# ExaScience/elprep

Hardware: AMD Instinct MI355X
Metric: Mreads/s through sort+markdup+BQSR, 150bp PE (higher is better)
Workload: dtype u8/int32/int64 (integer path; float64 finalize on host)

## Files before the change

### elprep_amd/csrc/common.hpp

```cpp
#pragma once

#include <hip/hip_runtime.h>

#include <sched.h>

#include <cstdarg>
#include <cstdint>
#include <cstdio>
#include <cstring>
#include <map>
#include <mutex>
#include <string>
#include <vector>

#include "../../include/elprep_hip.h"
#include "../../include/elprep_hip_debug.h"

namespace elp {

constexpr int WAVE = 64;

enum : uint16_t {
  F_MULTIPLE = 0x1, F_PROPER = 0x2, F_UNMAPPED = 0x4, F_NEXT_UNMAPPED = 0x8, F_REVERSED = 0x10, F_NEXT_REVERSED = 0x20,
  F_FIRST = 0x40, F_LAST = 0x80, F_SECONDARY = 0x100, F_QCFAILED = 0x200, F_DUPLICATE = 0x400, F_SUPPLEMENTARY = 0x800
};

enum : uint32_t { OP_M = 0, OP_I = 1, OP_D = 2, OP_N = 3, OP_S = 4, OP_H = 5, OP_P = 6, OP_EQ = 7, OP_X = 8 };

__host__ __device__ inline bool op_consumes_read(uint32_t op) { return op == OP_M || op == OP_I || op == OP_S || op == OP_EQ || op == OP_X; }
__host__ __device__ inline bool op_consumes_ref(uint32_t op) { return op == OP_M || op == OP_D || op == OP_N || op == OP_EQ || op == OP_X; }

size_t debug_guard_bytes();
void debug_guard_arm(void *p, size_t payload_bytes);
void debug_guard_release(void *p);
int debug_guard_check_all();

template <class T>
struct DVec {
  T *p = nullptr;
  size_t cap = 0;
  DVec() = default;
  DVec(const DVec &) = delete;
  DVec &operator=(const DVec &) = delete;
  ~DVec() { release(); }
  void release() {
    if (p) { debug_guard_release(p); (void)hipFree(p); }
    p = nullptr;
    cap = 0;
  }
  size_t bytes() const { return cap * sizeof(T); }
};

struct ProfPending {
  int name_id;
  hipEvent_t a, b;
};

}

struct elp_ctx {
  int device = 0;
  int n_cu = 256;
  hipStream_t stream = nullptr;
  std::string err;
  std::mutex stage_mu;

  bool have_header = false;
  int32_t n_ref = 0, n_rg = 0, n_lib = 0, n_cov = 0;
  std::vector<int32_t> h_ref_len;
  std::vector<uint16_t> h_rg_lib, h_rg_cov;
  elp::DVec<int32_t> ref_len;
  elp::DVec<uint16_t> rg_lib, rg_cov;

  static constexpr uint64_t SEQ_FRONT = 16;
  uint64_t n = 0, qname_bytes = 0, cigar_ops = 0, seq_bytes = SEQ_FRONT, qual_bytes = 0;
  uint64_t n_sr = 0;
  uint64_t n_filtered = 0;
  elp::DVec<int32_t> refid, pos, next_refid, pnext, tlen;
  elp::DVec<uint16_t> flag, rgid, split;
  elp::DVec<uint8_t> mapq, has_sr;
  elp::DVec<uint32_t> l_seq;
  elp::DVec<uint64_t> qname_off, cigar_off, seq_off, qual_off;
  elp::DVec<uint8_t> qname, seq4, qual;
  elp::DVec<uint32_t> cigar;
  elp::DVec<uint64_t> stage_tmp;
  uint32_t max_qname_len = 0, max_l_seq = 0;
  uint32_t max_split = 0;
  uint32_t max_pos = 0;
  int key_bits = 64;

  bool adapted = false, sorted = false, marked = false;
  bool sorted_qname = false;
  bool radix_check_pending = false;
  bool adapt_bad_qual = false;
  bool adapt_pending = false;
  elp::DVec<uint32_t> adapt_err;
  bool adapt_sampled = false;
  bool adapt_qmask_valid = false;
  unsigned long long adapt_qmask[2] = {0, 0};
  elp::DVec<uint2> apply_recs;
  bool apply_recs_valid = false;
  int apply_recs_lmax = 0;
  bool have_qual_present = false;
  unsigned long long qual_present[2] = {0, 0};
  elp::DVec<int32_t> upos, score;
  elp::DVec<uint64_t> qbounds;
  elp::DVec<uint64_t> key;
  elp::DVec<uint32_t> perm;
  elp::DVec<uint32_t> err_flag;
  elp::DVec<uint32_t> tile_first;
  void *h_pinned = nullptr;
  size_t h_pinned_cap = 0;
  elp::DVec<unsigned long long> radix_state;
  elp::DVec<uint32_t> radix_ticket;
  elp::DVec<unsigned long long> radix_hist;
  elp::DVec<uint32_t> scan_pool;
  elp::DVec<unsigned long long> xchg_hdr;
  elp::DVec<uint32_t> tie_live;
  elp::DVec<uint32_t> md_ctr;
  static constexpr uint32_t MAX_QNAME = 1000;
  static constexpr uint32_t TIE_LIVE_WORDS = 32;
  uint32_t radix_epoch = 0;
  uint64_t flat_index_n = 0, flat_index_bytes = 0;
  uint32_t uniform_len = 0;
  uint64_t uniform_n = ~0ull, uniform_bytes = ~0ull;

  elp::DVec<uint32_t> mate;
  elp::DVec<uint32_t> pair_win;

  std::vector<uint8_t *> h_ref_seq;
  std::vector<int64_t> h_ref_seq_len;
  std::vector<int32_t *> h_sites;
  std::vector<int64_t> h_n_sites;
  std::vector<uint8_t> ref_flags_dirty;
  std::vector<uint32_t *> h_site_idx;
  elp::DVec<uint8_t *> d_ref_seq;
  elp::DVec<int64_t> d_ref_seq_len;
  elp::DVec<int32_t *> d_sites;
  elp::DVec<uint32_t *> d_site_idx;
  elp::DVec<int64_t> d_n_sites;
  bool bqsr_ptrs_dirty = true;

  static constexpr size_t TABLES_TAIL = 4096;
  elp::DVec<unsigned long long> dev_tables;
  size_t tables_n = 0;
  int tables_max_cycle = 0;
  unsigned long long tables_quals[2] = {0, 0};
  elp::DVec<unsigned long long> tables_pack;
  elp::DVec<uint8_t> lut_rows_dev;
  void *comm = nullptr;
  bool comm_borrowed = false;
  int (*xport)(void *, int64_t *, size_t) = nullptr;
  void *xport_user = nullptr;
  int (*p2p)(void *, int, const void *, size_t, int, void *, size_t) = nullptr;
  void *p2p_user = nullptr;
  int group_rank = 0, group_world = 1;
  elp_ctx *group_owner = nullptr;
  std::vector<elp_ctx *> group_borrowers;

  elp::DVec<uint8_t> raw;
  elp::DVec<uint64_t> raw_off;
  uint64_t raw_n = 0, raw_bytes = 0;
  uint64_t max_raw_rec = 0;
  elp::DVec<uint8_t> rg_ids;
  elp::DVec<uint32_t> rg_ids_off;
  bool have_rg_ids = false;
  hipStream_t copy_stream = nullptr;
  elp::DVec<uint8_t> lut_dev;
  void *lut_pinned = nullptr;
  size_t lut_pinned_cap = 0;
  hipEvent_t lut_ev = nullptr;
  hipEvent_t apply_ev = nullptr;
  int lut_uploaded_cycle = 0;
  elp::DVec<uint32_t> lut_wk;
  bool dict_ready = false;
  bool dict_per_cov = false;
  int dict_qlo = 0, dict_nqi = 0, dict_lmax = 0, dict_cycle = 0, dict_ncov = 0;
  hipEvent_t tables_ev = nullptr;
  void *bounce[2] = {nullptr, nullptr};
  hipEvent_t bounce_ev[2] = {nullptr, nullptr};

  uint32_t *mail = nullptr;
  hipEvent_t mail_ev = nullptr;

  elp_ctx *side[2] = {nullptr, nullptr};
  hipEvent_t side_ev[2] = {nullptr, nullptr};
  hipEvent_t side_done[2] = {nullptr, nullptr};
  bool sort_ahead = false;
  uint64_t adapt_epoch = 0;
  uint64_t presort_epoch = ~0ull, presort_n = 0;
  uint64_t *presort_ks = nullptr;
  int presort_idx_bits = 0;

  elp::DVec<uint16_t> snap_flag;
  elp::DVec<uint8_t> snap_qual;
  uint64_t snap_n = 0, snap_qual_bytes = 0;
  bool have_snapshot = false;

  struct Tuning {
    int count_kernel = 0;
    int apply_kernel = 0;
    int count3_rlog = -1;
    int qual_hint = 0;
    int qual_hint_drop = -1;
    int pair_table_slots = 1 << 20;
    long long bgzf_piece = 1ll << 30;
    int bgzf_weak_guess = 0;
    int score_kernel = 0;
    int mate_path = 0;
    int radix_tile = 0;
    int sort_pairs = 0;
    int tie_rounds = 0;
    int exchange_piece = 0;
    int emit_pass = 0;
    long long bgzf_inflate_piece = 2ll << 30;
    int bgzf_copy_chunk = 0;
    int bgzf_tok_lds = 0;
    int bgzf_first_chunk_div = 4;
    int bgzf_fixed = 0;
    int bgzf_tok_fail_above = 0;
    int bgzf_stored = 0;
    int apply_wgs = 0;
    int presort_tile = 0;
    int side_priority = 0;
  } tune;

  elp::DVec<uint8_t> scratch[8];

  bool profiling = false;
  const char *prof_prefix = nullptr;
  std::vector<std::string> prof_names;
  std::map<std::string, int> prof_index;
  std::vector<uint64_t> prof_launches;
  std::vector<double> prof_ms;
  std::vector<elp::ProfPending> prof_pending;
};

namespace elp {

int set_error(elp_ctx *c, int code, const char *fmt, ...);
int prof_begin(elp_ctx *c, const char *name);
void prof_end(elp_ctx *c, int pending);
int prof_flush(elp_ctx *c);
struct ProfScope {
  elp_ctx *c;
  const char *saved;
  ProfScope(elp_ctx *ctx, const char *prefix) : c(ctx), saved(ctx->prof_prefix) { ctx->prof_prefix = prefix; }
  ~ProfScope() { c->prof_prefix = saved; }
};

#define ELP_HIP(ctx, call)                                                                             \
  do {                                                                                                 \
    hipError_t e__ = (call);                                                                           \
    if (e__ != hipSuccess)                                                                             \
      return elp::set_error((ctx), e__ == hipErrorOutOfMemory ? ELP_ERR_NOMEM : ELP_ERR_HIP, "%s failed: %s (%s:%d)", #call, \
                            hipGetErrorString(e__), __FILE__, __LINE__);                               \
  } while (0)

#define ELP_TRY(expr)            \
  do {                           \
    int rc__ = (expr);           \
    if (rc__ != 0) return rc__;  \
  } while (0)

bool sync_spin();
inline void spin_relax(unsigned &spins) {
  if (++spins < 4096u) {
#if defined(__x86_64__) || defined(__i386__)
    __builtin_ia32_pause();
#elif defined(__aarch64__)
    asm volatile("yield");
#endif
  } else {
    sched_yield();
  }
}
inline hipError_t stream_wait(hipStream_t st) {
  if (!sync_spin()) return hipStreamSynchronize(st);
  hipError_t e;
  unsigned spins = 0;
  while ((e = hipStreamQuery(st)) == hipErrorNotReady) spin_relax(spins);
  return e;
}
inline hipError_t event_wait(hipEvent_t ev) {
  if (!sync_spin()) return hipEventSynchronize(ev);
  hipError_t e;
  unsigned spins = 0;
  while ((e = hipEventQuery(ev)) == hipErrorNotReady) spin_relax(spins);
  return e;
}

int debug_poison();
bool debug_trace();

template <class T>
int ensure(elp_ctx *c, DVec<T> &v, size_t n, bool keep = false, size_t keep_elems = 0) {
  if (n <= v.cap) return 0;
  size_t ncap = keep ? (n + n / 2 + 16) : n;
  T *np = nullptr;
  ELP_HIP(c, hipMalloc((void **)&np, ncap * sizeof(T) + debug_guard_bytes()));
  if (debug_guard_bytes()) debug_guard_arm(np, ncap * sizeof(T));
  if (const int pz = debug_poison(); pz >= 0) {
    ELP_HIP(c, hipMemsetAsync(np, pz, ncap * sizeof(T), c->stream));
    ELP_HIP(c, elp::stream_wait(c->stream));
  }
  if (keep && v.p && keep_elems) {
    hipError_t e = hipMemcpyAsync(np, v.p, keep_elems * sizeof(T), hipMemcpyDeviceToDevice, c->stream);
    if (e == hipSuccess) e = elp::stream_wait(c->stream);
    if (e != hipSuccess) {
      (void)hipFree(np);
      return set_error(c, ELP_ERR_HIP, "device copy failed while growing a column: %s", hipGetErrorString(e));
    }
  }
  if (v.p) {
    (void)elp::stream_wait(c->stream);
    debug_guard_release(v.p);
    if (debug_poison() >= 0) { (void)hipMemsetAsync(v.p, 0xDD, v.cap * sizeof(T), c->stream); (void)elp::stream_wait(c->stream); }
    (void)hipFree(v.p);
  }
  v.p = np;
  v.cap = ncap;
  return 0;
}

template <class T>
int scratch(elp_ctx *c, int slot, size_t n, T **out) {
  ELP_TRY(ensure(c, c->scratch[slot], n * sizeof(T) + 256));
  *out = reinterpret_cast<T *>(c->scratch[slot].p);
  return 0;
}

#define ELP_LAUNCH(ctx, name, kernel, grid, block, shmem, ...)                              \
  do {                                                                                      \
    int pp__ = (ctx)->profiling ? elp::prof_begin((ctx), (name)) : -1;                      \
    if (elp::debug_trace()) fprintf(stderr, "[elp] %s\n", (name));                          \
    hipLaunchKernelGGL(kernel, grid, block, shmem, (ctx)->stream, __VA_ARGS__);             \
    if (pp__ >= 0) elp::prof_end((ctx), pp__);                                              \
    ELP_HIP((ctx), hipGetLastError());                                                      \
    if (elp::debug_trace()) ELP_HIP((ctx), elp::stream_wait((ctx)->stream));            \
  } while (0)

inline unsigned blocks_for(uint64_t n, unsigned per_block) { return (unsigned)((n + per_block - 1) / per_block); }

__device__ __forceinline__ uint64_t mix64(uint64_t x) {
  x ^= x >> 30; x *= 0xbf58476d1ce4e5b9ull; x ^= x >> 27; x *= 0x94d049bb133111ebull; x ^= x >> 31;
  return x;
}

__device__ __forceinline__ uint64_t load8(const uint8_t *__restrict__ p) {
  uint64_t w;
  __builtin_memcpy(&w, p, 8);
  return w;
}
__device__ __forceinline__ uint64_t low_bytes(uint64_t w, uint32_t nbytes) {
  return nbytes >= 8 ? w : (w & ((1ull << (8 * nbytes)) - 1ull));
}
__device__ inline int qname_cmp(const uint8_t *__restrict__ q, const uint64_t *__restrict__ off, uint32_t a, uint32_t b) {
  const uint64_t oa = off[a], ob = off[b];
  const uint32_t la = (uint32_t)(off[a + 1] - oa), lb = (uint32_t)(off[b + 1] - ob);
  const uint32_t m = la < lb ? la : lb;
  for (uint32_t i = 0; i < m; i += 8) {
    const uint32_t nb = m - i;
    const uint64_t wa = low_bytes(load8(q + oa + i), nb), wb = low_bytes(load8(q + ob + i), nb);
    if (wa != wb) {
      const uint64_t ba = __builtin_bswap64(wa), bb = __builtin_bswap64(wb);
      return ba < bb ? -1 : 1;
    }
  }
  return la < lb ? -1 : (la > lb ? 1 : 0);
}
__device__ inline bool qname_eq(const uint8_t *__restrict__ q, const uint64_t *__restrict__ off, uint32_t a, uint32_t b) {
  const uint64_t oa = off[a], ob = off[b];
  const uint32_t la = (uint32_t)(off[a + 1] - oa), lb = (uint32_t)(off[b + 1] - ob);
  if (la != lb) return false;
  uint64_t diff = 0;
  for (uint32_t i = 0; i < la && diff == 0; i += 32) {
    const uint64_t a0 = load8(q + oa + i), a1 = load8(q + oa + i + 8), a2 = load8(q + oa + i + 16), a3 = load8(q + oa + i + 24);
    const uint64_t b0 = load8(q + ob + i), b1 = load8(q + ob + i + 8), b2 = load8(q + ob + i + 16), b3 = load8(q + ob + i + 24);
    const uint32_t nb = la - i;
    diff |= low_bytes(a0 ^ b0, nb);
    diff |= nb > 8 ? low_bytes(a1 ^ b1, nb - 8) : 0ull;
    diff |= nb > 16 ? low_bytes(a2 ^ b2, nb - 16) : 0ull;
    diff |= nb > 24 ? low_bytes(a3 ^ b3, nb - 24) : 0ull;
  }
  return diff == 0;
}

__host__ __device__ inline uint16_t mod_flag(uint16_t flag) {
  if ((flag & F_MULTIPLE) == 0) flag &= (uint16_t) ~(F_NEXT_UNMAPPED | F_NEXT_REVERSED);
  if (flag & F_UNMAPPED) flag &= (uint16_t)~F_REVERSED;
  if (flag & F_NEXT_UNMAPPED) flag &= (uint16_t)~F_NEXT_REVERSED;
  return flag;
}

int radix_sort_pairs(elp_ctx *c, uint64_t *keys, uint32_t *vals, uint64_t *keys_tmp, uint32_t *vals_tmp, uint64_t n,
                     uint64_t **keys_out, uint32_t **vals_out);
int radix_sort_fused(elp_ctx *c, const uint64_t *keycol, uint64_t n, int key_bits, int idx_bits, uint64_t *buf0, uint64_t *buf1, uint64_t **out);
struct RadixBounds {
  uint32_t *start = nullptr, *nend = nullptr;
  uint32_t mask = 0;
  int shift = 0;
};
int radix_sort_pairs_low(elp_ctx *c, uint64_t *keys, uint32_t *vals, uint64_t *keys_tmp, uint32_t *vals_tmp, uint64_t n, int ndigits,
                         uint64_t **keys_out, uint32_t **vals_out, const uint64_t *first_src = nullptr, bool identity_vals = false,
                         const uint32_t *n_dev = nullptr , RadixBounds bnd = RadixBounds{});
int exclusive_scan_u32(elp_ctx *c, const uint32_t *in, uint32_t *out, uint64_t n, uint32_t *total_host );
int ensure_adapted(elp_ctx *c, bool check_quals = true);
int adapt_begin(elp_ctx *c, int *pos_bits);
int adapt_scores(elp_ctx *c);
int mailbox(elp_ctx *c);
int side_lane(elp_ctx *c, int lane, elp_ctx **out);
int side_join(elp_ctx *c, int lane);
int sort_presort(elp_ctx *c);
void prof_merge_side(elp_ctx *c);
constexpr int ADAPT_WORDS = 6;
void adapt_note(elp_ctx *c, const uint32_t *words );
int adapt_quality_error(elp_ctx *c);
int ensure_uniform_len(elp_ctx *c);
int ensure_qual_present(elp_ctx *c, bool exact = false);
int fetch_err(elp_ctx *c, uint32_t *words );
int radix_check(elp_ctx *c);
void group_release(elp_ctx *c);
int group_sendrecv(elp_ctx *c, int send_peer, const void *send_dev, size_t send_bytes, int recv_peer, void *recv_dev, size_t recv_bytes);
int tables_written(elp_ctx *c);
int stage_reserve(elp_ctx *c, uint64_t n, uint64_t qb, uint64_t co, uint64_t sb, uint64_t lb);
int merge_refuses_queryname(elp_ctx *groups, const char *who);
int merge_spread_slots(elp_ctx *groups, elp_ctx *spread, uint64_t **slots_out);
int stage_recode_seq(elp_ctx *c, uint64_t from, uint64_t bytes);
int stage_bam_columns(elp_ctx *c, uint32_t n_rec, uint64_t piece_bytes, uint64_t raw_end, uint64_t max_raw_rec, uint16_t split_id);
uint64_t bgzf_framed_size(uint64_t n_bytes);
int bgzf_frame(elp_ctx *c, const uint8_t *raw, uint64_t n_bytes, uint8_t *out);
int bgzf_deflate(elp_ctx *c, const uint8_t *raw, uint64_t n_bytes, uint8_t *out, uint64_t *out_bytes);

}
```

### elprep_amd/csrc/ctx.hip

```cpp
#include "common.hpp"

namespace elp {

namespace {
constexpr size_t GUARD = 4096;
constexpr uint8_t GUARD_BYTE = 0xC3;
std::mutex guard_mu;
std::map<void *, size_t> guard_of;
int guard_check_one(void *p, size_t payload) {
  uint8_t host[GUARD];
  if (hipDeviceSynchronize() != hipSuccess || hipMemcpy(host, static_cast<uint8_t *>(p) + payload, GUARD, hipMemcpyDeviceToHost) != hipSuccess) return 0;
  for (size_t k = 0; k < GUARD; k++)
    if (host[k] != GUARD_BYTE) {
      fprintf(stderr, "[elp] ELP_DEBUG_GUARD: byte %zu behind the end of a %zu-byte device buffer was overwritten (0x%02x)\n", k, payload, host[k]);
      return 1;
    }
  return 0;
}
}
size_t debug_guard_bytes() {
  static const size_t v = [] { const char *e = getenv("ELP_DEBUG_GUARD"); return (e && *e && *e != '0') ? GUARD : (size_t)0; }();
  return v;
}
void debug_guard_arm(void *p, size_t payload) {
// ... 258 lines not shown
    if (c->bounce[k]) (void)hipHostFree(c->bounce[k]);
    if (c->bounce_ev[k]) (void)hipEventDestroy(c->bounce_ev[k]);
  }
  if (c->copy_stream) (void)hipStreamDestroy(c->copy_stream);
  if (c->tables_ev) (void)hipEventDestroy(c->tables_ev);
  group_release(c);
  (void)hipStreamDestroy(c->stream);
  delete c;
}

const char *elp_last_error(const elp_ctx *c) { return c ? c->err.c_str() : "null context"; }

int elp_sync(elp_ctx *c) {
  if (!c) return ELP_ERR_ARG;
  if (c->radix_check_pending) return radix_check(c);
  ELP_HIP(c, elp::stream_wait(c->stream));
  return 0;
}

void *elp_stream(elp_ctx *c) { return c ? (void *)c->stream : nullptr; }

int elp_set_header(elp_ctx *c, const elp_header *h) {
  if (!c || !h || h->n_ref < 0 || h->n_rg < 0 || (h->n_ref && !h->ref_len) || (h->n_rg && (!h->rg_lib || !h->rg_cov)))
    return set_error(c, ELP_ERR_ARG, "elp_set_header: bad arguments");
  ELP_HIP(c, hipSetDevice(c->device));
  c->n_ref = h->n_ref; c->n_rg = h->n_rg; c->n_lib = h->n_lib; c->n_cov = h->n_cov;
  c->apply_recs_valid = false;
  c->h_ref_len.assign(h->ref_len, h->ref_len + h->n_ref);
  c->h_rg_lib.assign(h->rg_lib, h->rg_lib + h->n_rg);
  c->h_rg_cov.assign(h->rg_cov, h->rg_cov + h->n_rg);
  for (int i = 0; i < h->n_rg; i++) {
    if (c->h_rg_lib[i] != ELP_NIL16 && c->h_rg_lib[i] >= h->n_lib) return set_error(c, ELP_ERR_ARG, "rg_lib[%d] out of range", i);
    if (c->h_rg_cov[i] >= h->n_cov) return set_error(c, ELP_ERR_ARG, "rg_cov[%d] out of range", i);
  }
  ELP_TRY(ensure(c, c->ref_len, (size_t)h->n_ref + 1));
  ELP_TRY(ensure(c, c->rg_lib, (size_t)h->n_rg + 1));
  ELP_TRY(ensure(c, c->rg_cov, (size_t)h->n_rg + 1));
  if (h->n_ref) ELP_HIP(c, hipMemcpyAsync(c->ref_len.p, h->ref_len, h->n_ref * sizeof(int32_t), hipMemcpyHostToDevice, c->stream));
  if (h->n_rg) {
    ELP_HIP(c, hipMemcpyAsync(c->rg_lib.p, h->rg_lib, h->n_rg * sizeof(uint16_t), hipMemcpyHostToDevice, c->stream));
    ELP_HIP(c, hipMemcpyAsync(c->rg_cov.p, h->rg_cov, h->n_rg * sizeof(uint16_t), hipMemcpyHostToDevice, c->stream));
  }
  ELP_HIP(c, elp::stream_wait(c->stream));
  c->h_ref_seq.resize(h->n_ref, nullptr);
  c->h_ref_seq_len.resize(h->n_ref, 0);
  c->h_sites.resize(h->n_ref, nullptr);
  c->h_site_idx.resize(h->n_ref, nullptr);
  c->h_n_sites.resize(h->n_ref, 0);
  c->ref_flags_dirty.assign(h->n_ref, 0);
  c->bqsr_ptrs_dirty = true;
  c->have_header = true;
  return 0;
}

}
namespace elp {
int stage_reserve(elp_ctx *c, uint64_t n, uint64_t qb, uint64_t co, uint64_t sb, uint64_t lb) {
  bool keep = c->n > 0;
  ELP_TRY(ensure(c, c->refid, n, keep, c->n));
  ELP_TRY(ensure(c, c->pos, n, keep, c->n));
  ELP_TRY(ensure(c, c->next_refid, n, keep, c->n));
  ELP_TRY(ensure(c, c->pnext, n, keep, c->n));
  ELP_TRY(ensure(c, c->tlen, n, keep, c->n));
  ELP_TRY(ensure(c, c->flag, n, keep, c->n));
  ELP_TRY(ensure(c, c->rgid, n, keep, c->n));
  ELP_TRY(ensure(c, c->split, n, keep, c->n));
  ELP_TRY(ensure(c, c->mapq, n, keep, c->n));
  ELP_TRY(ensure(c, c->has_sr, n, keep, c->n));
  ELP_TRY(ensure(c, c->l_seq, n, keep, c->n));
  ELP_TRY(ensure(c, c->qname_off, n + 1, keep, c->n + 1));
  ELP_TRY(ensure(c, c->cigar_off, n + 1, keep, c->n + 1));
  ELP_TRY(ensure(c, c->seq_off, n + 1, keep, c->n + 1));
  ELP_TRY(ensure(c, c->qual_off, n + 1, keep, c->n + 1));
  ELP_TRY(ensure(c, c->qname, qb + 64, keep, c->qname_bytes));
  ELP_TRY(ensure(c, c->cigar, co + 4, keep, c->cigar_ops));
  ELP_TRY(ensure(c, c->seq4, sb + 32, keep, c->seq_bytes));
  ELP_TRY(ensure(c, c->qual, lb + 32, keep, c->qual_bytes));
  return 0;
}
}
extern "C" {

int elp_reserve(elp_ctx *c, uint64_t n, uint64_t qb, uint64_t co, uint64_t sb, uint64_t lb) {
  if (!c) return ELP_ERR_ARG;
  std::lock_guard<std::mutex> g(c->stage_mu);
  ELP_HIP(c, hipSetDevice(c->device));
  return stage_reserve(c, n, qb, co, sb + elp_ctx::SEQ_FRONT, lb);
}

int elp_reset(elp_ctx *c) {
  if (!c) return ELP_ERR_ARG;
  std::lock_guard<std::mutex> g(c->stage_mu);
  c->n = c->qname_bytes = c->cigar_ops = c->qual_bytes = 0;
  c->seq_bytes = elp_ctx::SEQ_FRONT;
  c->n_sr = 0;
  c->n_filtered = 0;
  c->raw_n = c->raw_bytes = 0;
  c->max_raw_rec = 0;
  c->max_split = 0;
  c->max_qname_len = c->max_l_seq = 0;
  c->max_pos = 0;
  c->adapted = c->sorted = c->sorted_qname = c->marked = false;
  c->have_qual_present = false;
  c->have_snapshot = false;
  c->flat_index_n = 0;
  c->uniform_n = ~0ull;
  return 0;
}

uint64_t elp_num_records(const elp_ctx *c) { return c ? c->n : 0; }
uint64_t elp_num_sorted(const elp_ctx *c) { return c ? c->n - c->n_sr : 0; }
uint64_t elp_num_qual_bytes(const elp_ctx *c) { return c ? c->qual_bytes : 0; }

int elp_stage(elp_ctx *c, const elp_batch *b) {
  if (!c || !b) return ELP_ERR_ARG;
  std::lock_guard<std::mutex> g(c->stage_mu);
  ELP_HIP(c, hipSetDevice(c->device));
  if (!c->have_header) return set_error(c, ELP_ERR_ARG, "elp_stage: call elp_set_header first");
  uint64_t n = b->n;
  if (n == 0) return 0;
  if (c->n + n > 0xFFFFFFF0ull) return set_error(c, ELP_ERR_UNSUPPORTED, "more than 2^32-16 records per context");
  uint64_t q0 = b->qname_off[0], c0 = b->cigar_off[0], s0 = b->seq_off[0], l0 = b->qual_off[0];
  uint64_t qb = b->qname_off[n] - q0, co = b->cigar_off[n] - c0, sb = b->seq_off[n] - s0, lb = b->qual_off[n] - l0;
  ELP_TRY(stage_reserve(c, c->n + n, c->qname_bytes + qb, c->cigar_ops + co, c->seq_bytes + sb, c->qual_bytes + lb));
  hipStream_t st = c->stream;
  uint64_t at = c->n;
#define H2D(dst, src, cnt, T) ELP_HIP(c, hipMemcpyAsync((dst), (src), (cnt) * sizeof(T), hipMemcpyHostToDevice, st))
  if (lb) H2D(c->qual.p + c->qual_bytes, b->qual + l0, lb, uint8_t);
  if (sb) {
    H2D(c->seq4.p + c->seq_bytes, b->seq4 + s0, sb, uint8_t);
    hipLaunchKernelGGL(k_recode_seq, dim3(blocks_for((sb + 15) / 16, 256)), dim3(256), 0, st, c->seq4.p + c->seq_bytes, sb);
    ELP_HIP(c, hipGetLastError());
  }
  if (qb) H2D(c->qname.p + c->qname_bytes, b->qname + q0, qb, uint8_t);
  if (co) H2D(c->cigar.p + c->cigar_ops, b->cigar + c0, co, uint32_t);
  H2D(c->refid.p + at, b->refid, n, int32_t);
  H2D(c->pos.p + at, b->pos, n, int32_t);
  H2D(c->next_refid.p + at, b->next_refid, n, int32_t);
  H2D(c->pnext.p + at, b->pnext, n, int32_t);
  H2D(c->tlen.p + at, b->tlen, n, int32_t);
  H2D(c->flag.p + at, b->flag, n, uint16_t);
  H2D(c->rgid.p + at, b->rgid, n, uint16_t);
  if (b->split) H2D(c->split.p + at, b->split, n, uint16_t);
  else ELP_HIP(c, hipMemsetAsync(c->split.p + at, 0, n * sizeof(uint16_t), st));
  H2D(c->mapq.p + at, b->mapq, n, uint8_t);
  H2D(c->l_seq.p + at, b->l_seq, n, uint32_t);
  if (b->has_sr) H2D(c->has_sr.p + at, b->has_sr, n, uint8_t);
  else ELP_HIP(c, hipMemsetAsync(c->has_sr.p + at, 0, n, st));
  ELP_TRY(ensure(c, c->stage_tmp, 4 * (n + 1)));
  unsigned blk = 256, grd = blocks_for(n + 1, blk);
  struct { const uint64_t *src; uint64_t *dst; uint64_t base; } offs[4] = {
      {b->qname_off, c->qname_off.p + at, c->qname_bytes}, {b->cigar_off, c->cigar_off.p + at, c->cigar_ops},
      {b->seq_off, c->seq_off.p + at, c->seq_bytes}, {b->qual_off, c->qual_off.p + at, c->qual_bytes}};
  for (int k = 0; k < 4; k++) H2D(c->stage_tmp.p + (size_t)k * (n + 1), offs[k].src, n + 1, uint64_t);
  for (int k = 0; k < 4; k++) {
    hipLaunchKernelGGL(k_rebase_offsets, dim3(grd), dim3(blk), 0, st, (const uint64_t *)(c->stage_tmp.p + (size_t)k * (n + 1)), offs[k].dst, n + 1, offs[k].base,
                       offs[k].src[0]);
    ELP_HIP(c, hipGetLastError());
  }
#undef H2D
  uint64_t n_sr = 0;
  uint32_t max_split = c->max_split;
  uint32_t max_qname_len = c->max_qname_len, max_l_seq = c->max_l_seq, max_pos = c->max_pos;
  int scan_rc = 0;
  for (uint64_t i = 0; i < n && !scan_rc; i++) {
    uint64_t ql = b->qname_off[i + 1] - b->qname_off[i];
    if (ql > elp_ctx::MAX_QNAME) scan_rc = set_error(c, ELP_ERR_UNSUPPORTED, "record %llu: QNAME of %llu bytes (limit %u)", (unsigned long long)i, (unsigned long long)ql, elp_ctx::MAX_QNAME);
    if (b->has_sr && b->has_sr[i]) n_sr++;
    if (b->split && b->split[i] > max_split) max_split = b->split[i];
    if (ql > max_qname_len) max_qname_len = (uint32_t)ql;
    if (b->l_seq[i] > max_l_seq) max_l_seq = b->l_seq[i];
    if ((uint32_t)b->pos[i] > max_pos) max_pos = (uint32_t)b->pos[i];
    if (b->qual_off[i + 1] - b->qual_off[i] > 0x3FFFFFull || b->l_seq[i] > 0x3FFFFFu)
      scan_rc = set_error(c, ELP_ERR_UNSUPPORTED, "record %llu: more than 4194303 bases", (unsigned long long)i);
    if (b->rgid[i] != ELP_NIL16 && b->rgid[i] >= c->n_rg) scan_rc = set_error(c, ELP_ERR_ARG, "record %llu: rgid %u not in header", (unsigned long long)i, b->rgid[i]);
    if (b->refid[i] >= c->n_ref) scan_rc = set_error(c, ELP_ERR_ARG, "record %llu: refid %d not in header", (unsigned long long)i, b->refid[i]);
  }
  if (scan_rc) { (void)elp::stream_wait(st); return scan_rc; }
  ELP_HIP(c, elp::stream_wait(st));
  c->n += n; c->qname_bytes += qb; c->cigar_ops += co; c->seq_bytes += sb; c->qual_bytes += lb;
  c->n_sr += n_sr;
  c->max_split = max_split;
  c->max_qname_len = max_qname_len; c->max_l_seq = max_l_seq; c->max_pos = max_pos;
  c->adapted = c->sorted = c->sorted_qname = c->marked = false;
  c->have_qual_present = false;
  c->have_snapshot = false;
  c->flat_index_n = 0;
  c->uniform_n = ~0ull;
  return 0;
}

int elp_stage_columns(elp_ctx *c, uint64_t n, const int32_t *refid, const int32_t *pos, const int32_t *next_refid, const int32_t *pnext, const int32_t *tlen,
                      const uint16_t *flag, const uint8_t *mapq, const uint16_t *rgid, const uint8_t *has_sr, const uint32_t *l_seq,
                      const uint64_t *qname_off, const uint8_t *qname, const uint64_t *cigar_off, const uint32_t *cigar, const uint64_t *seq_off,
                      const uint8_t *seq4, const uint64_t *qual_off, const uint8_t *qual, const uint16_t *split) {
  if (!c) return ELP_ERR_ARG;
  if (n && (!refid || !pos || !next_refid || !pnext || !tlen || !flag || !mapq || !rgid || !l_seq || !qname_off || !cigar_off || !seq_off || !qual_off))
    return set_error(c, ELP_ERR_ARG, "elp_stage_columns: a required column is NULL");
  elp_batch b;
  b.n = n; b.refid = refid; b.pos = pos; b.next_refid = next_refid; b.pnext = pnext; b.tlen = tlen; b.flag = flag; b.mapq = mapq; b.rgid = rgid;
  b.has_sr = has_sr; b.l_seq = l_seq; b.qname_off = qname_off; b.qname = qname; b.cigar_off = cigar_off; b.cigar = cigar; b.seq_off = seq_off;
  b.seq4 = seq4; b.qual_off = qual_off; b.qual = qual; b.split = split;
  return elp_stage(c, &b);
}

int elp_set_header_columns(elp_ctx *c, int32_t n_ref, const int32_t *ref_len, int32_t n_rg, const uint16_t *rg_lib, const uint16_t *rg_cov, int32_t n_lib,
                           int32_t n_cov) {
  elp_header h;
  h.n_ref = n_ref; h.ref_len = ref_len; h.n_rg = n_rg; h.rg_lib = rg_lib; h.rg_cov = rg_cov; h.n_lib = n_lib; h.n_cov = n_cov;
  return elp_set_header(c, &h);
}

static int d2h(elp_ctx *c, void *dst, const void *src, size_t bytes) {
  if (!bytes) return 0;
  ELP_HIP(c, hipSetDevice(c->device));
  ELP_HIP(c, hipMemcpyAsync(dst, src, bytes, hipMemcpyDeviceToHost, c->stream));
  ELP_HIP(c, elp::stream_wait(c->stream));
  return 0;
}

int elp_get_permutation(elp_ctx *c, uint32_t *out) {
  if (!c || (!out && c->n)) return ELP_ERR_ARG;
  if (!c->sorted) return set_error(c, ELP_ERR_ARG, "elp_get_permutation: call elp_sort_coordinate or elp_sort_queryname first");
  ELP_TRY(radix_check(c));
  return d2h(c, out, c->perm.p, c->n * sizeof(uint32_t));
}
int elp_get_flags(elp_ctx *c, uint16_t *out) {
  if (!c || (!out && c->n)) return ELP_ERR_ARG;
  ELP_TRY(radix_check(c));
  return d2h(c, out, c->flag.p, c->n * sizeof(uint16_t));
}
int elp_get_adapted(elp_ctx *c, int32_t *upos, int32_t *score) {
  if (!c) return ELP_ERR_ARG;
  ELP_TRY(ensure_adapted(c));
  if (upos) ELP_TRY(d2h(c, upos, c->upos.p, c->n * sizeof(int32_t)));
  if (score) ELP_TRY(d2h(c, score, c->score.p, c->n * sizeof(int32_t)));
  return 0;
}
int elp_get_qual(elp_ctx *c, uint8_t *out) {
  if (!c || (!out && c->qual_bytes)) return ELP_ERR_ARG;
  return d2h(c, out, c->qual.p, c->qual_bytes);
}

int elp_snapshot(elp_ctx *c) {
  if (!c) return ELP_ERR_ARG;
  ELP_HIP(c, hipSetDevice(c->device));
  ELP_TRY(ensure(c, c->snap_flag, c->n + 1));
  ELP_TRY(ensure(c, c->snap_qual, c->qual_bytes + 16));
  if (c->n) ELP_HIP(c, hipMemcpyAsync(c->snap_flag.p, c->flag.p, c->n * sizeof(uint16_t), hipMemcpyDeviceToDevice, c->stream));
  if (c->qual_bytes) ELP_HIP(c, hipMemcpyAsync(c->snap_qual.p, c->qual.p, c->qual_bytes, hipMemcpyDeviceToDevice, c->stream));
  c->snap_n = c->n;
  c->snap_qual_bytes = c->qual_bytes;
  c->have_snapshot = true;
  return 0;
}
int elp_rollback(elp_ctx *c) {
  if (!c) return ELP_ERR_ARG;
  if (!c->have_snapshot || c->snap_n != c->n || c->snap_qual_bytes != c->qual_bytes)
    return set_error(c, ELP_ERR_ARG, "elp_rollback: no snapshot of the current record set");
  ELP_HIP(c, hipSetDevice(c->device));
  if (c->n) ELP_HIP(c, hipMemcpyAsync(c->flag.p, c->snap_flag.p, c->n * sizeof(uint16_t), hipMemcpyDeviceToDevice, c->stream));
  if (c->qual_bytes) ELP_HIP(c, hipMemcpyAsync(c->qual.p, c->snap_qual.p, c->qual_bytes, hipMemcpyDeviceToDevice, c->stream));
  c->adapted = c->sorted = c->sorted_qname = c->marked = false;
  c->have_qual_present = false;
  return 0;
}

int elp_set_tuning(elp_ctx *c, const char *key, int64_t value) {
  if (!c || !key) return ELP_ERR_ARG;
  const std::string k(key);
  const int v = (int)value;
  if (k == "count_kernel") c->tune.count_kernel = v;
  else if (k == "apply_kernel") c->tune.apply_kernel = v;
  else if (k == "bgzf_piece") { if (value < 1) return set_error(c, ELP_ERR_ARG, "elp_set_tuning: bgzf_piece must be positive"); c->tune.bgzf_piece = value; }
  else if (k == "bgzf_weak_guess") c->tune.bgzf_weak_guess = v;
  else if (k == "score_kernel") { c->tune.score_kernel = v; c->adapted = false; }
  else if (k == "count3_rlog") c->tune.count3_rlog = v;
  else if (k == "qual_hint") { c->tune.qual_hint = v; c->have_qual_present = false; }
  else if (k == "qual_hint_drop") { c->tune.qual_hint_drop = v; c->have_qual_present = false; }
  else if (k == "pair_table_slots") {
    if (v == 0) { c->tune.pair_table_slots = 1 << 20; return 0; }
    if (v < 2 || v > (1 << 20) || (v & (v - 1))) return set_error(c, ELP_ERR_ARG, "elp_set_tuning: pair_table_slots must be a power of two >= 2");
    c->tune.pair_table_slots = v;
  } else if (k == "mate_path") {
    if (value != 0 && value != 2) return set_error(c, ELP_ERR_ARG, "elp_set_tuning: mate_path is 0 (the library decides) or 2 (every candidate through the table)");
    c->tune.mate_path = v;
  } else if (k == "tie_rounds") c->tune.tie_rounds = v;
  else if (k == "radix_tile") c->tune.radix_tile = v;
  else if (k == "sort_pairs") c->tune.sort_pairs = v;
  else if (k == "exchange_piece") c->tune.exchange_piece = v;
  else if (k == "emit_pass") c->tune.emit_pass = v;
  else if (k == "bgzf_stored") c->tune.bgzf_stored = v;
  else if (k == "bgzf_tok_fail_above") c->tune.bgzf_tok_fail_above = v;
  else if (k == "bgzf_fixed") c->tune.bgzf_fixed = v;
  else if (k == "bgzf_first_chunk_div") c->tune.bgzf_first_chunk_div = v;
  else if (k == "bgzf_tok_lds") c->tune.bgzf_tok_lds = v;
  else if (k == "bgzf_copy_chunk") c->tune.bgzf_copy_chunk = v;
  else if (k == "bgzf_inflate_piece") { if (value < 1) return set_error(c, ELP_ERR_ARG, "elp_set_tuning: bgzf_inflate_piece must be positive"); c->tune.bgzf_inflate_piece = value; }
  else if (k == "md_fused" || k == "bgzf_inflate") {
    if (value != 0) return set_error(c, ELP_ERR_ARG, "elp_set_tuning: key '%s' is retired (only 0 is accepted)", key);
  } else if (k == "apply_wgs") c->tune.apply_wgs = v;
  else if (k == "presort_tile") c->tune.presort_tile = v;
  else if (k == "side_priority") c->tune.side_priority = v;
  else return set_error(c, ELP_ERR_ARG, "elp_set_tuning: unknown key '%s'", key);
  return 0;
}

int elp_profile_enable(elp_ctx *c, int on) {
  if (!c) return ELP_ERR_ARG;
  if (!on) { ELP_TRY(prof_flush(c)); prof_merge_side(c); }
  c->profiling = on != 0;
  for (int lane = 0; lane < 2; lane++)
    if (c->side[lane]) c->side[lane]->profiling = c->profiling;
  return 0;
}
int elp_profile_reset(elp_ctx *c) {
  if (!c) return ELP_ERR_ARG;
  ELP_TRY(prof_flush(c));
  prof_merge_side(c);
  for (auto &v : c->prof_launches) v = 0;
  for (auto &v : c->prof_ms) v = 0.0;
  return 0;
}
int elp_profile_count(elp_ctx *c) {
  if (!c) return ELP_ERR_ARG;
  if (prof_flush(c) != 0) return ELP_ERR_HIP;
  prof_merge_side(c);
  return (int)c->prof_names.size();
}
int elp_profile_get(elp_ctx *c, int index, const char **name, uint64_t *launches, double *total_ms) {
  if (!c || index < 0 || index >= (int)c->prof_names.size()) return ELP_ERR_ARG;
  if (name) *name = c->prof_names[index].c_str();
  if (launches) *launches = c->prof_launches[index];
  if (total_ms) *total_ms = c->prof_ms[index];
  return 0;
}

}
```

### elprep_amd/csrc/metrics.hip

```cpp
#include "common.hpp"

namespace elp {

constexpr uint32_t EMPTY = 0xFFFFFFFFu;

struct MxCols {
  uint64_t n;
  const int32_t *refid;
  const uint16_t *flag;
  const uint16_t *rgid;
  const uint16_t *rg_lib;
  const int32_t *upos;
  const uint64_t *qname_off;
  const uint8_t *qname;
  const uint32_t *mate, *pair_win;
  int32_t n_lib;
  const uint8_t *has_sr;
  const uint16_t *split;
  int32_t n_split;
};
constexpr uint32_t OPT_SMALL = 32;
constexpr uint32_t OPT_LIST_CAP = 300000;

__device__ __forceinline__ uint32_t lib_row(const MxCols &m, uint32_t i) {
  const uint16_t rg = m.rgid[i];
  const uint16_t lb = rg == ELP_NIL16 ? (uint16_t)ELP_NIL16 : m.rg_lib[rg];
  return lb == ELP_NIL16 ? (uint32_t)m.n_lib : (uint32_t)lb;
}
__device__ __forceinline__ bool true_pair(uint16_t f) { return (f & (F_MULTIPLE | F_NEXT_UNMAPPED)) == F_MULTIPLE; }

__device__ __forceinline__ void order_ends(const MxCols &m, uint32_t second, uint32_t first, uint32_t &a1, uint32_t &a2) {
  a1 = second; a2 = first;
  const int32_t r1 = m.refid[a1], r2 = m.refid[a2];
  const int32_t p1 = m.upos[a1], p2 = m.upos[a2];
  const bool v1 = m.flag[a1] & F_REVERSED, v2 = m.flag[a2] & F_REVERSED;
  if (r1 > r2 || (r1 == r2 && (p1 > p2 || (p1 == p2 && v1 && !v2)))) { uint32_t t = a1; a1 = a2; a2 = t; }
}
__device__ __forceinline__ uint32_t listed_read(const MxCols &m, uint32_t owner) {
  uint32_t a1, a2;
  order_ends(m, owner, m.mate[owner], a1, a2);
  return (m.flag[a1] & F_FIRST) ? a1 : a2;
}

constexpr int DC_CAP = 2048, DC_STEP = 1024;
__device__ __forceinline__ void wave_count(unsigned int *lds, int cell) {
  unsigned long long todo = __ballot(cell >= 0);
  while (todo) {
    const int leader = __ffsll((long long)todo) - 1;
    const int c0 = __builtin_amdgcn_readlane(cell, leader);
    const unsigned long long peers = __ballot(cell == c0);
    if ((int)(threadIdx.x & 63) == leader) atomicAdd(&lds[c0], (unsigned int)__popcll(peers));
    todo &= ~peers;
  }
}
__global__ __launch_bounds__(256) void k_dup_counters(MxCols m, unsigned long long *__restrict__ ctr, unsigned long long *__restrict__ pair_reads,
                                                      uint64_t chunk, uint64_t *__restrict__ lkeys, uint32_t *__restrict__ lvals, uint32_t *list_n) {
  extern __shared__ unsigned int lds_ctr[];
  __shared__ uint2 lq[DC_CAP];
  __shared__ uint32_t lcount, gbase;
  const int nrow = (m.n_lib + 1) * ELP_NCTR, ncell = nrow + m.n_split * (m.n_lib + 1);
  for (int k = threadIdx.x; k < ncell; k += blockDim.x) lds_ctr[k] = 0;
  if (threadIdx.x == 0) lcount = 0;
  __syncthreads();
  const uint64_t lo = (uint64_t)blockIdx.x * chunk, hi = lo + chunk < m.n ? lo + chunk : m.n;
  for (uint64_t base = lo; base < hi; base += DC_STEP) {
    constexpr int R = DC_STEP / 256;
    uint8_t sr[R];
    uint16_t fl[R], rg[R], sp[R];
    uint32_t pw[R], mt[R];
#pragma unroll
    for (int t = 0; t < R; t++) {
      const uint64_t i = base + (uint64_t)t * 256 + threadIdx.x;
      const bool in = i < hi;
      sr[t] = in ? m.has_sr[i] : (uint8_t)1;
      fl[t] = in ? m.flag[i] : (uint16_t)0;
      rg[t] = in ? m.rgid[i] : (uint16_t)ELP_NIL16;
      sp[t] = in ? m.split[i] : (uint16_t)0;
      pw[t] = in ? m.pair_win[i] : EMPTY;
      mt[t] = in ? m.mate[i] : EMPTY;
    }
    uint16_t lb[R], fm[R];
    uint8_t srm[R];
#pragma unroll
    for (int t = 0; t < R; t++) {
      lb[t] = rg[t] == ELP_NIL16 ? (uint16_t)ELP_NIL16 : m.rg_lib[rg[t]];
      const bool need = mt[t] != EMPTY && ((fl[t] & F_DUPLICATE) || pw[t] != EMPTY);
      srm[t] = need ? m.has_sr[mt[t]] : (uint8_t)0;
      fm[t] = need ? m.flag[mt[t]] : (uint16_t)0;
    }
#pragma unroll
    for (int t = 0; t < R; t++) {
      const uint32_t i = (uint32_t)(base + (uint64_t)t * 256 + threadIdx.x);
      bool loser = false;
      int cell1 = -1, cell2 = -1;
      if (!sr[t]) {
        const uint16_t f = fl[t];
        const int lib = lb[t] == ELP_NIL16 ? m.n_lib : (int)lb[t], row = lib * ELP_NCTR;
        if (f & F_UNMAPPED) cell1 = row + 3;
        else if (f & (F_SECONDARY | F_SUPPLEMENTARY)) cell1 = row + 2;
        else {
          const bool tp = true_pair(f);
          cell1 = tp ? nrow + (int)sp[t] * (m.n_lib + 1) + lib : row;
          if (f & F_DUPLICATE) {
            if (!tp) cell2 = row + 4;
            else if (mt[t] != EMPTY && mt[t] < i && (fm[t] & F_DUPLICATE) && !srm[t]) cell2 = row + 5;
          }
        }
        loser = pw[t] != EMPTY && !srm[t];
      }
      wave_count(lds_ctr, cell1);
      wave_count(lds_ctr, cell2);
      const unsigned long long mask = __ballot(loser);
      if (mask) {
        const int lane = threadIdx.x & 63, leader = __ffsll((long long)mask) - 1;
        uint32_t at = 0;
        if (lane == leader) at = atomicAdd(&lcount, (uint32_t)__popcll(mask));
        at = __shfl(at, leader, 64);
        if (loser) lq[at + (uint32_t)__popcll(mask & ((1ull << lane) - 1ull))] = make_uint2(i, pw[t]);
      }
    }
    __syncthreads();
    const uint32_t have = lcount;
    if (have > DC_CAP - DC_STEP || base + DC_STEP >= hi) {
      if (threadIdx.x == 0) gbase = have ? atomicAdd(list_n, have) : 0u;
      __syncthreads();
      for (uint32_t k = threadIdx.x; k < have; k += 256) {
        const uint2 e = lq[k];
        lkeys[gbase + k] = (uint64_t)e.y;
        lvals[gbase + k] = e.x;
      }
      __syncthreads();
      if (threadIdx.x == 0) lcount = 0;
      __syncthreads();
    }
  }
  for (int k = threadIdx.x; k < nrow; k += blockDim.x)
    if (lds_ctr[k]) atomicAdd(&ctr[k], (unsigned long long)lds_ctr[k]);
  for (int k = threadIdx.x + nrow; k < ncell; k += blockDim.x)
    if (lds_ctr[k]) atomicAdd(&pair_reads[k - nrow], (unsigned long long)lds_ctr[k]);
}

__global__ __launch_bounds__(256) void k_opt_heads(uint32_t L, const uint64_t *__restrict__ ks, uint32_t *__restrict__ head) {
  const uint32_t j = blockIdx.x * blockDim.x + threadIdx.x;
  if (j < L) head[j] = (j == 0 || ks[j] != ks[j - 1]) ? 1u : 0u;
}
__global__ __launch_bounds__(256) void k_opt_starts(uint32_t L, const uint32_t *__restrict__ head, const uint32_t *__restrict__ gidx,
                                                    uint32_t *__restrict__ gstart, uint32_t G) {
  const uint32_t j = blockIdx.x * blockDim.x + threadIdx.x;
  if (j >= L) return;
  if (head[j]) gstart[gidx[j]] = j;
  if (j == L - 1) gstart[G] = L;
}

struct Tile { long long t, x, y; };

template <class W>
__device__ __forceinline__ Tile tile_parse(uint32_t len, bool *bad, W word) {
  long long v2 = 0, v3 = 0, v4 = 0, v5 = 0, v6 = 0;
  uint32_t badmask = 0;
  int col = 0;
  unsigned long long x = 0;
  uint32_t ndig = 0;
  bool neg = false, fbad = false, first = true;
  uint64_t w = 0;
  for (uint32_t i = 0;; i++) {
    const bool end = i == len;
    if (!end && (i & 7u) == 0) w = word(i >> 3);
    const uint32_t ch = end ? (uint32_t)':' : (uint32_t)(w >> (8 * (i & 7u))) & 0xFFu;
    if (ch == ':') {
      const bool fb = fbad || ndig == 0 || x > (neg ? 0x8000000000000000ull : 0x7FFFFFFFFFFFFFFFull);
      const long long val = (long long)(neg ? 0ull - x : x);
      if (col == 2) v2 = val; else if (col == 3) v3 = val; else if (col == 4) v4 = val; else if (col == 5) v5 = val; else if (col == 6) v6 = val;
      if (col >= 2 && col <= 6 && fb) badmask |= 1u << col;
      col++;
      x = 0; ndig = 0; neg = false; fbad = false; first = true;
    } else {
      if (first && (ch == '+' || ch == '-')) {
        neg = ch == '-';
      } else {
        const uint32_t d = ch - (uint32_t)'0';
        if (d > 9) fbad = true;
        else if (x > 922337203685477580ull) fbad = true;
        else x = x * 10 + d;
        ndig++;
      }
      first = false;
    }
    if (end) break;
  }
  int a;
  if (col == 7) a = 4;
  else if (col == 5) a = 2;
  else return Tile{-1, -1, -1};
  if (badmask & (7u << a)) { *bad = true; return Tile{-1, -1, -1}; }
  return a == 4 ? Tile{v4, v5, v6} : Tile{v2, v3, v4};
}
__device__ inline Tile tile_info(const uint8_t *__restrict__ q, uint32_t len, bool *bad) {
  if (len <= 48) {
    const uint64_t w0 = len > 0 ? load8(q) : 0ull, w1 = len > 8 ? load8(q + 8) : 0ull, w2 = len > 16 ? load8(q + 16) : 0ull,
                   w3 = len > 24 ? load8(q + 24) : 0ull, w4 = len > 32 ? load8(q + 32) : 0ull, w5 = len > 40 ? load8(q + 40) : 0ull;
    return tile_parse(len, bad, [&](uint32_t k) { return k == 0 ? w0 : k == 1 ? w1 : k == 2 ? w2 : k == 3 ? w3 : k == 4 ? w4 : w5; });
  }
  return tile_parse(len, bad, [&](uint32_t k) { return load8(q + 8 * k); });
}

struct Member { long long t, x, y; uint32_t rg_rev, bad; };

__device__ inline Member make_member(const MxCols &m, uint32_t read) {
  bool bad = false;
  const uint64_t o = m.qname_off[read];
  Tile tl = tile_info(m.qname + o, (uint32_t)(m.qname_off[read + 1] - o), &bad);
  return Member{tl.t, tl.x, tl.y, ((uint32_t)m.rgid[read] << 1) | ((m.flag[read] & F_REVERSED) ? 1u : 0u), bad ? 1u : 0u};
}

__global__ __launch_bounds__(256) void k_opt_slots(MxCols m, uint32_t L, const uint64_t *__restrict__ ks, const uint32_t *__restrict__ vs,
                                                   const uint32_t *__restrict__ head, const uint32_t *__restrict__ gidx,
                                                   const uint32_t *__restrict__ gstart, uint32_t *__restrict__ mread, uint2 *__restrict__ ginfo,
                                                   uint32_t *__restrict__ mset) {
  const uint32_t j = blockIdx.x * blockDim.x + threadIdx.x;
  if (j >= L) return;
  const bool is_head = head[j] != 0;
  const uint32_t g = gidx[j] - (is_head ? 0u : 1u);
  const uint32_t j0 = gstart[g], oslot = j0 + g;
  const uint32_t slot = j + g + 1;
  mread[slot] = listed_read(m, vs[j]);
  mset[slot] = oslot;
  if (is_head) {
    const uint32_t origin = (uint32_t)ks[j];
    mread[oslot] = listed_read(m, origin);
    mset[oslot] = oslot;
    ginfo[oslot] = make_uint2(gstart[g + 1] - j0 + 1, origin);
  }
}
__global__ __launch_bounds__(256) void k_opt_fill(MxCols m, uint32_t total, const uint32_t *__restrict__ mread, Member *__restrict__ members) {
  const uint32_t s = blockIdx.x * blockDim.x + threadIdx.x;
  if (s >= total) return;
  members[s] = make_member(m, mread[s]);
}

__device__ inline uint32_t uf_find(uint32_t *p, uint32_t x) {
  uint32_t r = x;
  while (p[r] != r) r = p[r];
  while (p[x] != r) { uint32_t nx = p[x]; p[x] = r; x = nx; }
  return r;
}
__device__ __forceinline__ long long go_abs_diff(long long a, long long b) {
  const unsigned long long d = (unsigned long long)a - (unsigned long long)b;
  return (long long)((long long)d < 0 ? 0ull - d : d);
}
__device__ __forceinline__ bool optical_close(const Member &a, const Member &b, long long dist) {
  if (a.t == -1 || b.rg_rev != a.rg_rev || b.t != a.t) return false;
  return go_abs_diff(a.x, b.x) <= dist && go_abs_diff(a.y, b.y) <= dist;
}

__global__ __launch_bounds__(128) void k_opt_eval(MxCols m, uint32_t total, const uint2 *__restrict__ ginfo, const Member *__restrict__ members,
                                                  uint32_t *__restrict__ parent, long long dist, unsigned long long *__restrict__ ctr,
                                                  uint32_t *err, unsigned long long *__restrict__ hist, int hist_len, int lds_bins,
                                                  uint32_t *__restrict__ linfo, uint32_t *__restrict__ lcount, uint32_t *n_large) {
  extern __shared__ unsigned int lds_opt[];
  unsigned int *lds_h = lds_opt + (m.n_lib + 1);
  const int n_h = hist ? (m.n_lib + 1) * 3 * lds_bins : 0;
  for (int k = threadIdx.x; k <= m.n_lib + n_h; k += blockDim.x) lds_opt[k] = 0;
  __syncthreads();
  for (uint32_t b = blockIdx.x * blockDim.x + threadIdx.x; b < total; b += gridDim.x * blockDim.x) {
  const uint2 gi = ginfo[b];
  const uint32_t cnt = gi.x;
  uint32_t optical = 0;
  bool large = false;
  if (cnt > OPT_SMALL) {
    const Member *g = members + b;
    uint32_t nr = 0, bad_f = 0, bad_r = 0;
    for (uint32_t k = 0; k < cnt; k++) {
      const uint32_t rev = g[k].rg_rev & 1u;
      nr += rev;
      bad_r |= g[k].bad & rev;
      bad_f |= g[k].bad & (rev ^ 1u);
    }
    const uint32_t nf = cnt - nr;
    if ((bad_f && nf >= 2 && nf <= OPT_LIST_CAP) || (bad_r && nr >= 2 && nr <= OPT_LIST_CAP)) atomicOr(&err[2], 1u);
    linfo[b] = 1u | (nf > OPT_LIST_CAP ? 2u : 0u) | (nr > OPT_LIST_CAP ? 4u : 0u);
    lcount[b] = (nf > OPT_LIST_CAP ? OPT_LIST_CAP + 1 : nf) + (nr > OPT_LIST_CAP ? OPT_LIST_CAP + 1 : nr);
    atomicAdd(n_large, cnt);
    large = true;
  } else if (cnt >= 2) {
  const Member *g = members + b;
  {
    uint32_t nr = 0, bad_f = 0, bad_r = 0;
    for (uint32_t k = 0; k < cnt; k++) {
      const uint32_t rev = g[k].rg_rev & 1u, bad = g[k].bad;
      nr += rev;
      bad_r |= bad & rev;
      bad_f |= bad & (rev ^ 1u);
    }
    if ((bad_f && cnt - nr >= 2) || (bad_r && nr >= 2)) atomicOr(&err[2], 1u);
  }
  if (cnt == 2) {
    optical = optical_close(g[0], g[1], dist) ? 1u : 0u;
  } else if (cnt == 3) {
    const Member m0 = g[0], m1 = g[1], m2 = g[2];
    const uint32_t e01 = optical_close(m0, m1, dist), e02 = optical_close(m0, m2, dist), e12 = optical_close(m1, m2, dist);
    const uint32_t edges = e01 + e02 + e12;
    optical = edges >= 2 ? 2u : edges;
  } else {
    uint32_t *p = parent + b;
    for (uint32_t k = 0; k < cnt; k++) p[k] = k;
    uint32_t comps = cnt;
    for (uint32_t a = 0; a < cnt; a++) {
      const Member ma = g[a];
      if (ma.t == -1) continue;
      for (uint32_t c2 = a + 1; c2 < cnt; c2++) {
        if (optical_close(ma, g[c2], dist)) {
          const uint32_t ra = uf_find(p, a), rb = uf_find(p, c2);
          if (ra != rb) { p[rb] = ra; comps--; }
        }
      }
    }
    optical = cnt - comps;
  }
  }
  if (!large && (optical || (hist && cnt >= 2))) {
    const uint32_t owner = gi.y;
    uint32_t a1, a2;
    order_ends(m, owner, m.mate[owner], a1, a2);
    const uint32_t lib = lib_row(m, a1);
    if (optical) atomicAdd(&lds_opt[lib], optical);
    if (hist && cnt >= 2) {
      const int idx[3] = {(int)cnt, (int)(cnt - optical), optical ? (int)optical + 1 : 0};
#pragma unroll
      for (int k = 0; k < 3; k++) {
        if (idx[k] <= 0) continue;
        const int bin = idx[k] < hist_len ? idx[k] : hist_len - 1;
        if (bin < lds_bins) atomicAdd(&lds_h[((int)lib * 3 + k) * lds_bins + bin], 1u);
        else atomicAdd(&hist[((size_t)lib * 3 + k) * hist_len + bin], 1ull);
      }
    }
  }
  }
  __syncthreads();
  for (int k = threadIdx.x; k <= m.n_lib; k += blockDim.x)
    if (lds_opt[k]) atomicAdd(&ctr[k * ELP_NCTR + 6], (unsigned long long)lds_opt[k]);
  for (int k = threadIdx.x; k < n_h; k += blockDim.x)
    if (lds_h[k]) atomicAdd(&hist[(size_t)(k / lds_bins) * hist_len + (k % lds_bins)], (unsigned long long)lds_h[k]);
}

__global__ __launch_bounds__(256) void k_large_list(uint32_t total, const uint32_t *__restrict__ mset, const uint32_t *__restrict__ linfo,
                                                    const Member *__restrict__ members, uint64_t *__restrict__ keys, uint32_t *__restrict__ vals,
                                                    uint32_t *count) {
  const uint32_t s = blockIdx.x * blockDim.x + threadIdx.x;
  if (s >= total) return;
  const uint32_t b = mset[s], li = linfo[b];
  if (!(li & 1u)) return;
  const Member mem = members[s];
  if (mem.t == -1 || (li & ((mem.rg_rev & 1u) ? 4u : 2u))) return;
  const uint32_t at = atomicAdd(count, 1u);
  keys[at] = mix64(mix64(((uint64_t)b << 32) | mem.rg_rev) ^ (uint64_t)mem.t);
  vals[at] = s;
}
__device__ __forceinline__ uint32_t puf_find(uint32_t *parent, uint32_t x) {
  for (;;) {
    const uint32_t p = __hip_atomic_load(&parent[x], __ATOMIC_RELAXED, __HIP_MEMORY_SCOPE_AGENT);
    if (p == x) return x;
    x = p;
  }
}
__device__ inline void puf_union(uint32_t *parent, uint32_t a, uint32_t b) {
  for (;;) {
    a = puf_find(parent, a);
    b = puf_find(parent, b);
    if (a == b) return;
    const uint32_t hi = a > b ? a : b, lo = a > b ? b : a;
    if (atomicCAS(&parent[hi], hi, lo) == hi) return;
  }
}
__global__ __launch_bounds__(256) void k_large_union(uint32_t cnt, const uint64_t *__restrict__ keys, const uint32_t *__restrict__ vals,
                                                     const uint32_t *__restrict__ mset, const Member *__restrict__ members, long long dist,
                                                     uint32_t *parent) {
  const uint32_t j = blockIdx.x * blockDim.x + threadIdx.x;
  if (j >= cnt) return;
  const uint64_t kj = keys[j];
  const uint32_t sj = vals[j], bj = mset[sj];
  const Member mj = members[sj];
  for (uint32_t k = j + 1; k < cnt && keys[k] == kj; k++) {
    const uint32_t sk = vals[k];
    if (mset[sk] == bj && optical_close(mj, members[sk], dist)) puf_union(parent, j, k);
  }
}
__global__ __launch_bounds__(256) void k_large_roots(uint32_t cnt, const uint32_t *__restrict__ vals, const uint32_t *__restrict__ mset,
                                                     const uint32_t *__restrict__ parent, unsigned long long *setcnt) {
  const uint32_t j = blockIdx.x * blockDim.x + threadIdx.x;
  if (j >= cnt) return;
  atomicAdd(&setcnt[mset[vals[j]]], 1ull | (parent[j] == j ? (1ull << 32) : 0ull));
}
__global__ __launch_bounds__(256) void k_large_final(MxCols m, uint32_t total, const uint2 *__restrict__ ginfo, const uint32_t *__restrict__ linfo,
                                                     const uint32_t *__restrict__ lcount, const unsigned long long *__restrict__ setcnt,
                                                     unsigned long long *__restrict__ ctr, unsigned long long *__restrict__ hist, int hist_len) {
  const uint32_t b = blockIdx.x * blockDim.x + threadIdx.x;
  if (b >= total || !(linfo[b] & 1u) || ginfo[b].x == 0) return;
  const unsigned long long sc = setcnt[b];
  const uint32_t optical = (uint32_t)sc - (uint32_t)(sc >> 32);
  const uint32_t owner = ginfo[b].y;
  uint32_t a1, a2;
  order_ends(m, owner, m.mate[owner], a1, a2);
  const uint32_t lib = lib_row(m, a1);
  if (optical) atomicAdd(&ctr[lib * ELP_NCTR + 6], (unsigned long long)optical);
  if (hist) {
    const uint32_t cnt = lcount[b];
    const int idx[3] = {(int)cnt, (int)(cnt - optical), optical ? (int)optical + 1 : 0};
    for (int k = 0; k < 3; k++) {
      if (idx[k] <= 0) continue;
      const int bin = idx[k] < hist_len ? idx[k] : hist_len - 1;
      atomicAdd(&hist[((size_t)lib * 3 + k) * hist_len + bin], 1ull);
    }
  }
}
__global__ __launch_bounds__(256) void k_iota32(uint32_t *v, uint32_t n) {
  const uint32_t i = blockIdx.x * blockDim.x + threadIdx.x;
  if (i < n) v[i] = i;
}

__global__ __launch_bounds__(256) void k_origin_count(MxCols m, unsigned long long *__restrict__ origins) {
  extern __shared__ unsigned int lds_org[];
  for (int k = threadIdx.x; k <= m.n_lib; k += blockDim.x) lds_org[k] = 0;
  __syncthreads();
  for (uint64_t i = (uint64_t)blockIdx.x * blockDim.x + threadIdx.x; i < m.n; i += (uint64_t)gridDim.x * blockDim.x) {
    const uint32_t mt = m.mate[i];
    if (mt == EMPTY || mt > (uint32_t)i || m.pair_win[i] != EMPTY) continue;
    uint32_t a1, a2;
    order_ends(m, (uint32_t)i, mt, a1, a2);
    atomicAdd(&lds_org[lib_row(m, a1)], 1u);
  }
  __syncthreads();
  for (int k = threadIdx.x; k <= m.n_lib; k += blockDim.x)
    if (lds_org[k]) atomicAdd(&origins[k], (unsigned long long)lds_org[k]);
}

static int metrics_impl(elp_ctx *c, int dist, int64_t *counters_host, int64_t *hist_host, int hist_len) {
  const uint64_t n = c->n;
  const int ncell = (c->n_lib + 1) * ELP_NCTR;
  if (!c->marked) return set_error(c, ELP_ERR_ARG, "elp_dup_metrics: call elp_mark_duplicates first");
  const size_t nhist = hist_host ? (size_t)(c->n_lib + 1) * 3 * (size_t)hist_len : 0, norg = hist_host ? (size_t)(c->n_lib + 1) : 0;
  const int n_split = (int)c->max_split + 1;
  const size_t npr = (size_t)n_split * (size_t)(c->n_lib + 1);
  if (((size_t)ncell + npr) * sizeof(unsigned int) > 46000)
    return set_error(c, ELP_ERR_UNSUPPORTED, "elp_dup_metrics: %d split ids x %d libraries in one context", n_split, c->n_lib + 1);
  unsigned long long *ctr;
  ELP_TRY(scratch(c, 0, (size_t)ncell + norg + nhist + npr + 8, &ctr));
  unsigned long long *origins = ctr + ncell, *hist = hist_host ? origins + norg : nullptr, *pair_reads = ctr + ncell + norg + nhist;
  hipStream_t st = c->stream;
  ELP_HIP(c, hipMemsetAsync(ctr, 0, ((size_t)ncell + norg + nhist + npr) * sizeof(unsigned long long), st));
  int lds_bins = hist_host ? std::min(hist_len, 32) : 0;
  if ((size_t)(c->n_lib + 1) * (1 + 3 * (size_t)lds_bins) * sizeof(unsigned int) > 32768) lds_bins = 0;
  if (n) {
    MxCols m{n, c->refid.p, c->flag.p, c->rgid.p, c->rg_lib.p, c->upos.p, c->qname_off.p, c->qname.p, c->mate.p, c->pair_win.p, c->n_lib,
             c->has_sr.p, c->split.p, n_split};
    const unsigned grid = blocks_for(n, 256);
    const size_t lcap = n / 2 + 8;
    uint32_t *gs;
    ELP_TRY(scratch(c, 1, 6 * lcap + 16, &gs));
    uint64_t *pk = reinterpret_cast<uint64_t *>(gs);
    uint32_t *pv = gs + 4 * lcap;
    uint32_t *mailbox = c->err_flag.p + 3;
    ELP_HIP(c, hipMemsetAsync(mailbox, 0, 4, st));
    const unsigned cgrid = (unsigned)std::min<uint64_t>(2048, (n + DC_STEP - 1) / DC_STEP);
    const uint64_t chunk = (((n + cgrid - 1) / cgrid) + DC_STEP - 1) / DC_STEP * DC_STEP;
    ELP_LAUNCH(c, "mx_counters", k_dup_counters, dim3(cgrid), dim3(256), ((size_t)ncell + npr) * sizeof(unsigned int), m, ctr, pair_reads, chunk, pk, pv,
               mailbox);
    uint32_t L = 0;
    ELP_HIP(c, hipMemcpyAsync(&L, mailbox, 4, hipMemcpyDeviceToHost, st));
    ELP_HIP(c, elp::stream_wait(st));
    ELP_HIP(c, hipMemsetAsync(mailbox, 0, 4, st));
    if ((size_t)L > lcap) return set_error(c, ELP_ERR_HIP, "elp_dup_metrics: more losing pairs than pairs");
    uint32_t total = 0, G = 0;
    uint64_t *ks = pk;
    uint32_t *vs = pv, *head = nullptr, *gidx = nullptr, *gstart = nullptr;
    if (L) {
      int ndig = 1;
      while (ndig < 4 && (n >> (8 * ndig)) != 0) ndig++;
      {
        ProfScope ps(c, "mx_");
        ELP_TRY(radix_sort_pairs_low(c, pk, pv, pk + lcap, pv + lcap, L, ndig, &ks, &vs));
      }
      head = reinterpret_cast<uint32_t *>(ks == pk ? pk + lcap : pk);
      gidx = head + lcap;
      gstart = vs == pv ? pv + lcap : pv;
      ELP_LAUNCH(c, "mx_opt_heads", k_opt_heads, dim3(blocks_for(L, 256)), dim3(256), 0, L, (const uint64_t *)ks, head);
      {
        ProfScope ps(c, "mx_");
        ELP_TRY(exclusive_scan_u32(c, head, gidx, L, &G));
      }
      ELP_LAUNCH(c, "mx_opt_starts", k_opt_starts, dim3(blocks_for(L, 256)), dim3(256), 0, L, (const uint32_t *)head, (const uint32_t *)gidx, gstart, G);
      total = L + G;
    }
    if (total) {
      Member *members;
      uint32_t *wk, *mread;
      uint2 *ginfo;
      const size_t tp = ((size_t)total + 7) & ~(size_t)7;
      ELP_TRY(scratch(c, 2, (size_t)total + 4, &members));
      ELP_TRY(scratch(c, 3, 12 * tp + 16, &wk));
      ELP_TRY(scratch(c, 4, (size_t)total + 4, &mread));
      ELP_TRY(scratch(c, 5, (size_t)total + 4, &ginfo));
      uint32_t *parent = wk, *mset = wk + tp, *linfo = wk + 2 * tp, *lcount = wk + 3 * tp, *lvals = wk + 6 * tp;
      unsigned long long *setcnt = reinterpret_cast<unsigned long long *>(wk + 4 * tp);
      uint64_t *lkeys = reinterpret_cast<uint64_t *>(wk + 8 * tp);
      ELP_HIP(c, hipMemsetAsync(ginfo, 0, (size_t)total * sizeof(uint2), st));
      ELP_HIP(c, hipMemsetAsync(linfo, 0, 4 * tp * sizeof(uint32_t), st));
      ELP_LAUNCH(c, "mx_opt_slots", k_opt_slots, dim3(blocks_for(L, 256)), dim3(256), 0, m, L, (const uint64_t *)ks, (const uint32_t *)vs,
                 (const uint32_t *)head, (const uint32_t *)gidx, (const uint32_t *)gstart, mread, ginfo, mset);
      ELP_LAUNCH(c, "mx_opt_fill", k_opt_fill, dim3(blocks_for(total, 256)), dim3(256), 0, m, total, (const uint32_t *)mread, members);
      ELP_LAUNCH(c, "mx_opt_eval", k_opt_eval, dim3(std::min(blocks_for(total, 128), 2048u)), dim3(128),
                 (size_t)(c->n_lib + 1) * (1 + (hist ? 3 * (size_t)lds_bins : 0)) * sizeof(unsigned int), m, total, (const uint2 *)ginfo,
                 (const Member *)members, parent, (long long)dist, ctr, c->err_flag.p, hist, hist_len, lds_bins, linfo, lcount, mailbox);
      uint32_t n_large = 0;
      ELP_HIP(c, hipMemcpyAsync(&n_large, mailbox, 4, hipMemcpyDeviceToHost, st));
      ELP_HIP(c, elp::stream_wait(st));
      ELP_HIP(c, hipMemsetAsync(mailbox, 0, 4, st));
      if (n_large) {
        ELP_LAUNCH(c, "mx_large_list", k_large_list, dim3(blocks_for(total, 256)), dim3(256), 0, total, (const uint32_t *)mset, (const uint32_t *)linfo,
                   (const Member *)members, lkeys, lvals, mailbox);
        uint32_t cl = 0;
        ELP_HIP(c, hipMemcpyAsync(&cl, mailbox, 4, hipMemcpyDeviceToHost, st));
        ELP_HIP(c, elp::stream_wait(st));
        ELP_HIP(c, hipMemsetAsync(mailbox, 0, 4, st));
        if (cl) {
          uint64_t *ks;
          uint32_t *vs;
          ProfScope ps(c, "mx_large_");
          ELP_TRY(radix_sort_pairs(c, lkeys, lvals, lkeys + tp, lvals + tp, cl, &ks, &vs));
          ELP_LAUNCH(c, "mx_large_iota", k_iota32, dim3(blocks_for(cl, 256)), dim3(256), 0, parent, cl);
          ELP_LAUNCH(c, "mx_large_union", k_large_union, dim3(blocks_for(cl, 256)), dim3(256), 0, cl, (const uint64_t *)ks, (const uint32_t *)vs,
                     (const uint32_t *)mset, (const Member *)members, (long long)dist, parent);
          ELP_LAUNCH(c, "mx_large_roots", k_large_roots, dim3(blocks_for(cl, 256)), dim3(256), 0, cl, (const uint32_t *)vs, (const uint32_t *)mset,
                     (const uint32_t *)parent, setcnt);
        }
        ELP_LAUNCH(c, "mx_large_final", k_large_final, dim3(blocks_for(total, 256)), dim3(256), 0, m, total, (const uint2 *)ginfo, (const uint32_t *)linfo,
                   (const uint32_t *)lcount, (const unsigned long long *)setcnt, ctr, hist, hist_len);
      }
    }
    if (hist)
      ELP_LAUNCH(c, "mx_origin_count", k_origin_count, dim3(std::min(grid, 2048u)), dim3(256), (c->n_lib + 1) * sizeof(unsigned int), m, origins);
  }
  std::vector<unsigned long long> h((size_t)ncell + norg + nhist + npr);
  ELP_HIP(c, hipMemcpyAsync(h.data(), ctr, h.size() * sizeof(unsigned long long), hipMemcpyDeviceToHost, st));
  uint32_t e[4];
  ELP_TRY(fetch_err(c, e));
  if (e[2]) {
    ELP_HIP(c, hipMemsetAsync(c->err_flag.p + 2, 0, 4, st));
    return set_error(c, ELP_ERR_DATA, "QNAME tile/x/y field is not an integer (reference: internal.ParseInt panics, filters/mark-optical-duplicates.go:55-61)");
  }
  for (int l = 0; l <= c->n_lib; l++)
    for (int k = 0; k < ELP_NCTR; k++) counters_host[l * ELP_NCTR + k] = (int64_t)h[l * ELP_NCTR + k];
  for (int l = 0; l <= c->n_lib; l++) {
    int64_t pairs = 0;
    for (int sp = 0; sp < n_split; sp++) pairs += (int64_t)(h[(size_t)ncell + norg + nhist + (size_t)sp * (c->n_lib + 1) + l] / 2);
    counters_host[l * ELP_NCTR + 1] = pairs;
  }
  if (hist_host) {
    const unsigned long long *ho = h.data() + ncell, *hh = ho + norg;
    for (int l = 0; l <= c->n_lib; l++) {
      int64_t *out = hist_host + (size_t)l * 3 * hist_len;
      unsigned long long with_dups = 0;
      for (size_t k = 0; k < (size_t)3 * hist_len; k++) out[k] = (int64_t)hh[(size_t)l * 3 * hist_len + k];
      for (int b = 0; b < hist_len; b++) with_dups += hh[(size_t)l * 3 * hist_len + b];
      const int64_t alone = (int64_t)(ho[l] - with_dups);
      const int one = 1 < hist_len ? 1 : hist_len - 1;
      out[one] += alone;
      out[hist_len + one] += alone;
    }
  }
  return 0;
}

}

namespace elp {
static int metrics_on_side(elp_ctx *c, int dist, int64_t *counters_host, int64_t *hist_host, int hist_len) {
  if (!c->marked) return set_error(c, ELP_ERR_ARG, "elp_dup_metrics: call elp_mark_duplicates first");
  elp_ctx *s = nullptr;
  ELP_TRY(side_lane(c, 0, &s));
  s->n = c->n; s->n_lib = c->n_lib; s->n_rg = c->n_rg; s->n_ref = c->n_ref; s->max_split = c->max_split; s->marked = c->marked;
  s->n_sr = c->n_sr; s->n_filtered = c->n_filtered;
  s->flag.p = c->flag.p; s->rgid.p = c->rgid.p; s->rg_lib.p = c->rg_lib.p; s->refid.p = c->refid.p; s->qname_off.p = c->qname_off.p; s->qname.p = c->qname.p;
  s->pair_win.p = c->pair_win.p; s->mate.p = c->mate.p; s->has_sr.p = c->has_sr.p; s->upos.p = c->upos.p; s->split.p = c->split.p;
  const int rc = metrics_impl(s, dist, counters_host, hist_host, hist_len);
  s->flag.p = nullptr; s->rgid.p = nullptr; s->rg_lib.p = nullptr; s->refid.p = nullptr; s->qname_off.p = nullptr; s->qname.p = nullptr;
  s->pair_win.p = nullptr; s->mate.p = nullptr; s->has_sr.p = nullptr; s->upos.p = nullptr; s->split.p = nullptr;
  if (rc != 0) {
    (void)elp::stream_wait(s->stream);
    c->err = s->err;
  }
  return rc;
}
}

extern "C" int elp_dup_metrics(elp_ctx *c, int optical_pixel_distance, int64_t *counters) {
  if (!c || !counters) return ELP_ERR_ARG;
  ELP_HIP(c, hipSetDevice(c->device));
  return elp::metrics_on_side(c, optical_pixel_distance, counters, nullptr, 0);
}

extern "C" int elp_dup_metrics_hist(elp_ctx *c, int optical_pixel_distance, int64_t *counters, int64_t *hist, int hist_len) {
  if (!c || !counters || !hist || hist_len < 2) return elp::set_error(c, ELP_ERR_ARG, "elp_dup_metrics_hist: bad arguments (hist_len >= 2)");
  ELP_HIP(c, hipSetDevice(c->device));
  return elp::metrics_on_side(c, optical_pixel_distance, counters, hist, hist_len);
}
```

### elprep_amd/csrc/radix.hip

```cpp
#include "common.hpp"

namespace elp {

__device__ __forceinline__ uint32_t wave_incl_scan(uint32_t v) {
  const int lane = threadIdx.x & 63;
#pragma unroll
  for (int d = 1; d < 64; d <<= 1) {
    uint32_t t = __shfl_up(v, d, 64);
    if (lane >= d) v += t;
  }
  return v;
}

__device__ __forceinline__ uint32_t block_excl_scan_256(uint32_t v, uint32_t *total, uint32_t *lds ) {
  const int lane = threadIdx.x & 63, w = threadIdx.x >> 6;
  uint32_t inc = wave_incl_scan(v);
  if (lane == 63) lds[w] = inc;
  __syncthreads();
  uint32_t base = 0, tot = 0;
#pragma unroll
  for (int i = 0; i < 4; i++) {
    uint32_t s = lds[i];
    if (i < w) base += s;
    tot += s;
  }
  __syncthreads();
  *total = tot;
  return base + inc - v;
}

constexpr int SCAN_ITEMS = 8;
constexpr int SCAN_TILE = 256 * SCAN_ITEMS;

__global__ __launch_bounds__(256) void k_scan_reduce(const uint32_t *__restrict__ in, uint32_t *__restrict__ sums, uint64_t n) {
  __shared__ uint32_t lds[8];
  uint64_t base = (uint64_t)blockIdx.x * SCAN_TILE + (uint64_t)threadIdx.x * SCAN_ITEMS;
  uint32_t s = 0;
#pragma unroll
  for (int i = 0; i < SCAN_ITEMS; i++)
    if (base + i < n) s += in[base + i];
  uint32_t tot;
  (void)block_excl_scan_256(s, &tot, lds);
  if (threadIdx.x == 0) sums[blockIdx.x] = tot;
}

__global__ __launch_bounds__(256) void k_scan_down(const uint32_t *__restrict__ in, uint32_t *__restrict__ out,
                                                   const uint32_t *__restrict__ block_base, uint64_t n) {
  __shared__ uint32_t lds[8];
  uint64_t base = (uint64_t)blockIdx.x * SCAN_TILE + (uint64_t)threadIdx.x * SCAN_ITEMS;
  uint32_t v[SCAN_ITEMS];
  uint32_t s = 0;
#pragma unroll
  for (int i = 0; i < SCAN_ITEMS; i++) {
    v[i] = (base + i < n) ? in[base + i] : 0u;
    s += v[i];
  }
  uint32_t tot;
  uint32_t ex = block_excl_scan_256(s, &tot, lds) + (block_base ? block_base[blockIdx.x] : 0u);
#pragma unroll
  for (int i = 0; i < SCAN_ITEMS; i++) {
    if (base + i < n) out[base + i] = ex;
    ex += v[i];
  }
}

static int scan_levels(elp_ctx *c, const uint32_t *in, uint32_t *out, uint64_t n, uint32_t *total_dev) {
  if (n == 0) {
    if (total_dev) ELP_HIP(c, hipMemsetAsync(total_dev, 0, 4, c->stream));
    return 0;
  }
  std::vector<uint64_t> cnt;
  cnt.push_back(n);
  while (true) {
    uint64_t nb = (cnt.back() + SCAN_TILE - 1) / SCAN_TILE;
    cnt.push_back(nb);
    if (nb <= 1) break;
  }
  size_t need = 0;
  for (size_t k = 1; k < cnt.size(); k++) need += cnt[k] + 4;
  uint32_t *pool;
  ELP_TRY(ensure(c, c->scan_pool, need + 16));
  pool = c->scan_pool.p;
  std::vector<uint32_t *> sums(cnt.size(), nullptr);
  size_t off = 0;
  for (size_t k = 1; k < cnt.size(); k++) { sums[k] = pool + off; off += cnt[k] + 4; }
  const uint32_t *src = in;
  for (size_t k = 0; k + 1 < cnt.size(); k++) {
    ELP_LAUNCH(c, "scan_reduce", k_scan_reduce, dim3((unsigned)cnt[k + 1]), dim3(256), 0, src, sums[k + 1], cnt[k]);
    src = sums[k + 1];
  }
  size_t top = cnt.size() - 1;
  if (total_dev) ELP_HIP(c, hipMemcpyAsync(total_dev, sums[top], 4, hipMemcpyDeviceToDevice, c->stream));
  ELP_HIP(c, hipMemsetAsync(sums[top], 0, 4, c->stream));
  for (size_t k = top - 1; k >= 1; k--) {
    ELP_LAUNCH(c, "scan_down", k_scan_down, dim3((unsigned)cnt[k + 1]), dim3(256), 0, (const uint32_t *)sums[k], sums[k],
               (const uint32_t *)sums[k + 1], cnt[k]);
  }
  ELP_LAUNCH(c, "scan_down", k_scan_down, dim3((unsigned)cnt[1]), dim3(256), 0, in, out, (const uint32_t *)sums[1], n);
  return 0;
}

int exclusive_scan_u32(elp_ctx *c, const uint32_t *in, uint32_t *out, uint64_t n, uint32_t *total_host) {
  uint32_t *tot_dev = nullptr;
  if (total_host) tot_dev = c->err_flag.p + 3;
  ELP_TRY(scan_levels(c, in, out, n, tot_dev));
  if (total_host) {
    ELP_HIP(c, hipMemcpyAsync(total_host, tot_dev, 4, hipMemcpyDeviceToHost, c->stream));
    ELP_HIP(c, elp::stream_wait(c->stream));
    ELP_HIP(c, hipMemsetAsync(tot_dev, 0, 4, c->stream));
  }
  return 0;
}

constexpr int RS_THREADS = 256;
constexpr int RS_ITEMS = 16;
constexpr int RS_TILE = RS_THREADS * RS_ITEMS;

template <int ND>
__global__ __launch_bounds__(256) void k_radix_hist_all(const uint64_t *__restrict__ keys, uint64_t n, unsigned long long *__restrict__ ghist ,
                                                        const uint32_t *__restrict__ n_dev) {
  __shared__ uint32_t h[8][256];
  if (n_dev) n = *n_dev;
  for (int i = threadIdx.x; i < 8 * 256; i += 256) (&h[0][0])[i] = 0;
  __syncthreads();
  for (uint64_t i = (uint64_t)blockIdx.x * 256 + threadIdx.x; i < n; i += (uint64_t)gridDim.x * 256) {
    uint64_t k = keys[i];
    const unsigned long long act = __ballot(1);
    const int first = __ffsll((long long)act) - 1;
#pragma unroll
    for (int d = 0; d < ND; d++) {
      uint32_t dg = (uint32_t)(k >> (8 * d)) & 0xFF;
      uint32_t d0 = __shfl(dg, first, 64);
      if (__all(dg == d0)) {
        if ((int)(threadIdx.x & 63) == first) atomicAdd(&h[d][d0], (uint32_t)__popcll(act));
      } else {
        atomicAdd(&h[d][dg], 1u);
      }
    }
  }
  __syncthreads();
  for (int i = threadIdx.x; i < ND * 256; i += 256) {
    uint32_t v = (&h[0][0])[i];
    if (v) atomicAdd(&ghist[i], (unsigned long long)v);
  }
}

constexpr unsigned long long RS_AGG = 1ull << 32, RS_INCL = 2ull << 32;

template <int THREADS, bool PAIRS>
__global__ __launch_bounds__(THREADS, THREADS >= 512 ? 4 : 1) void k_radix_scatter_t(const uint64_t *__restrict__ keys, const uint32_t *__restrict__ vals,
                                                              uint64_t *__restrict__ keys_out, uint32_t *__restrict__ vals_out, uint64_t n,
                                                              int shift, const unsigned long long *__restrict__ ghist ,
                                                              unsigned long long *state, uint32_t epoch, uint32_t *ticket,
                                                              uint32_t *err, const uint32_t *__restrict__ n_dev, int fuse, RadixBounds bnd) {
  constexpr int WAVES = THREADS / 64, TILE = THREADS * RS_ITEMS;
  __shared__ uint32_t cnt[WAVES][256];
  __shared__ uint32_t gbase[256];
  __shared__ uint32_t scan_lds[16];
  extern __shared__ __attribute__((aligned(16))) uint64_t sbuf_dyn[];
  __shared__ uint64_t sbuf_static[THREADS == 256 ? RS_TILE : 1];
  uint64_t *const sbuf = THREADS == 256 ? sbuf_static : sbuf_dyn;
  __shared__ uint32_t my_tile;
  const int lane = threadIdx.x & 63, w = threadIdx.x >> 6;
  if (threadIdx.x == 0) my_tile = atomicAdd(ticket, 1u);
  for (int i = threadIdx.x; i < WAVES * 256; i += THREADS) (&cnt[0][0])[i] = 0;
  __syncthreads();
  const uint32_t tile = my_tile;
  const uint64_t tbase = (uint64_t)tile * TILE;
  if (n_dev) {
    n = *n_dev;
    if (tbase >= n) return;
  }
  const uint64_t wbase = tbase + (uint64_t)w * (64 * RS_ITEMS);
  const uint32_t tile_n = (uint32_t)((n - tbase) < (uint64_t)TILE ? (n - tbase) : (uint64_t)TILE);
  uint64_t k[RS_ITEMS];
  uint32_t v[PAIRS ? RS_ITEMS : 1];
  uint32_t pos[RS_ITEMS];
  const unsigned long long lt_mask = (1ull << lane) - 1ull;
#pragma unroll
  for (int r = 0; r < RS_ITEMS; r++) {
    uint64_t i = wbase + (uint64_t)r * 64 + lane;
    bool valid = i < n;
    k[r] = valid ? keys[i] : ~0ull;
    if (!PAIRS && fuse && valid) k[r] = (k[r] << fuse) | i;
    if (PAIRS) v[r] = valid ? (vals ? vals[i] : (uint32_t)i) : 0u;
    uint32_t d = (uint32_t)(k[r] >> shift) & 0xFF;
    unsigned long long peers = __ballot(valid);
    peers = valid ? peers : ~peers;
#pragma unroll
    for (int b = 0; b < 8; b++) {
      unsigned long long m = __ballot((d >> b) & 1);
      peers &= ((d >> b) & 1) ? m : ~m;
    }
    uint32_t before = (uint32_t)__popcll(peers & lt_mask);
    int leader = __ffsll((long long)peers) - 1;
    uint32_t old = 0;
    if (valid && lane == leader) {
      old = cnt[w][d];
      cnt[w][d] = old + (uint32_t)__popcll(peers);
    }
    old = __shfl(old, leader, 64);
    pos[r] = old + before;
  }
  __syncthreads();
  uint32_t tot = 0, tstart;
  const unsigned long long tag = (unsigned long long)epoch << 34;
  const bool owner = THREADS == 256 || threadIdx.x < 256;
  const uint32_t dg = THREADS == 256 ? threadIdx.x : (threadIdx.x & 255u);
  unsigned long long *mine = state + (size_t)tile * 256 + dg;
  {
    if (owner) {
#pragma unroll
      for (int i = 0; i < WAVES; i++) tot += cnt[i][dg];
      __hip_atomic_store(mine, tag | (tile == 0 ? RS_INCL : RS_AGG) | tot, __ATOMIC_RELAXED, __HIP_MEMORY_SCOPE_AGENT);
    }
    uint32_t all;
    tstart = block_excl_scan_256(tot, &all, scan_lds);
    if (owner) {
      uint32_t run = tstart;
#pragma unroll
      for (int i = 0; i < WAVES; i++) {
        uint32_t t = cnt[i][dg];
        cnt[i][dg] = run;
        run += t;
      }
    }
  }
  __syncthreads();
#pragma unroll
  for (int r = 0; r < RS_ITEMS; r++) {
    uint64_t i = wbase + (uint64_t)r * 64 + lane;
    if (i < n) {
      uint32_t d = (uint32_t)(k[r] >> shift) & 0xFF;
      pos[r] += cnt[w][d];
      sbuf[pos[r]] = k[r];
    }
  }
  {
    uint32_t dall;
    const uint32_t dbase = block_excl_scan_256(owner ? (uint32_t)ghist[dg] : 0u, &dall, scan_lds);
    uint32_t prefix = 0;
    if (tile != 0 && owner) {
      constexpr int LB = 8;
      uint32_t back = 1, spins = 0;
      bool done = false;
      while (!done) {
        unsigned long long v[LB];
#pragma unroll
        for (int i = 0; i < LB; i++) {
          const uint32_t b = back + (uint32_t)i;
          v[i] = b <= tile ? __hip_atomic_load(mine - (size_t)b * 256, __ATOMIC_RELAXED, __HIP_MEMORY_SCOPE_AGENT) : (tag | RS_INCL);
        }
#pragma unroll
        for (int i = 0; i < LB; i++) {
          if (done || (v[i] >> 34) != epoch) break;
          prefix += (uint32_t)v[i];
          back++;
          done = (v[i] & RS_INCL) != 0;
        }
        if (!done) {
          __builtin_amdgcn_s_sleep(1);
          if (++spins == (1u << 22)) { atomicOr(err, 256u); break; }
        }
      }
      __hip_atomic_store(mine, tag | RS_INCL | (prefix + tot), __ATOMIC_RELAXED, __HIP_MEMORY_SCOPE_AGENT);
    }
    if (owner) gbase[dg] = dbase + prefix - tstart;
  }
  __syncthreads();
  uint32_t dst[RS_ITEMS];
#pragma unroll
  for (int r = 0; r < RS_ITEMS; r++) {
    const uint32_t j = (uint32_t)r * THREADS + threadIdx.x;
    if (j < tile_n) {
      const uint64_t key = sbuf[j];
      dst[r] = gbase[(uint32_t)(key >> shift) & 0xFF] + j;
      keys_out[dst[r]] = key;
      if (PAIRS && bnd.start) {
        const uint32_t b = ((uint32_t)key & bnd.mask) >> bnd.shift;
        const bool first = j == 0 || (((uint32_t)sbuf[j - 1] & bnd.mask) >> bnd.shift) != b;
        const bool last = j + 1 == tile_n || (((uint32_t)sbuf[j + 1] & bnd.mask) >> bnd.shift) != b;
        if (first) atomicMin(&bnd.start[b], dst[r]);
        if (last) atomicMin(&bnd.nend[b], ~(dst[r] + 1u));
      }
    }
  }
  if (!PAIRS) return;
  __syncthreads();
  uint32_t *sval = reinterpret_cast<uint32_t *>(sbuf);
#pragma unroll
  for (int r = 0; r < RS_ITEMS; r++) {
    uint64_t i = wbase + (uint64_t)r * 64 + lane;
    if (i < n) sval[pos[r]] = v[PAIRS ? r : 0];
  }
  __syncthreads();
#pragma unroll
  for (int r = 0; r < RS_ITEMS; r++) {
    const uint32_t j = (uint32_t)r * THREADS + threadIdx.x;
    if (j < tile_n) vals_out[dst[r]] = sval[j];
  }
}

static int radix_pass_setup(elp_ctx *c, uint32_t ntiles) {
  if ((size_t)ntiles * 256 > c->radix_state.cap) {
    ELP_TRY(ensure(c, c->radix_state, (size_t)ntiles * 256));
    ELP_HIP(c, hipMemsetAsync(c->radix_state.p, 0, c->radix_state.cap * sizeof(unsigned long long), c->stream));
    c->radix_epoch = 0;
  }
  return 0;
}
static int radix_next_epoch(elp_ctx *c) {
  if (++c->radix_epoch >= (1u << 30)) {
    ELP_HIP(c, hipMemsetAsync(c->radix_state.p, 0, c->radix_state.cap * sizeof(unsigned long long), c->stream));
    c->radix_epoch = 1;
  }
  return 0;
}

static int radix_tile_shift(const elp_ctx *c, uint64_t n) {
  if (c->tune.radix_tile >= 1 && c->tune.radix_tile <= 3) return c->tune.radix_tile - 1;
  return n >= (16ull << 20) ? 2 : n >= (4ull << 20) ? 1 : 0;
}
static bool radix_big_tiles(const elp_ctx *c, uint64_t n) { return radix_tile_shift(c, n) == 1; }
static uint32_t radix_tiles(const elp_ctx *c, uint64_t n) {
  const uint64_t tile = (uint64_t)RS_TILE << radix_tile_shift(c, n);
  return (uint32_t)((n + tile - 1) / tile);
}
template <bool PAIRS>
static int radix_scatter_launch_t(elp_ctx *c, uint64_t n, const uint64_t *kin, const uint32_t *vin, uint64_t *kdst, uint32_t *vdst, int shift,
                                  const unsigned long long *ghist, uint32_t *ticket, const uint32_t *n_dev, int fuse, RadixBounds bnd = RadixBounds{}) {
  const uint32_t ntiles = radix_tiles(c, n);
  const int ts = radix_tile_shift(c, n);
  if (ts == 2) {
    const size_t dyn = (size_t)4 * RS_TILE * sizeof(uint64_t);
    ELP_HIP(c, hipFuncSetAttribute(reinterpret_cast<const void *>(&k_radix_scatter_t<1024, PAIRS>), hipFuncAttributeMaxDynamicSharedMemorySize, (int)dyn));
    ELP_LAUNCH(c, "radix_scatter", (k_radix_scatter_t<1024, PAIRS>), dim3(ntiles), dim3(1024), dyn, kin, vin, kdst, vdst, n, shift, ghist, c->radix_state.p,
               c->radix_epoch, ticket, c->err_flag.p, n_dev, fuse, bnd);
  } else if (ts == 1) {
    const size_t dyn = (size_t)2 * RS_TILE * sizeof(uint64_t);
    ELP_HIP(c, hipFuncSetAttribute(reinterpret_cast<const void *>(&k_radix_scatter_t<512, PAIRS>), hipFuncAttributeMaxDynamicSharedMemorySize, (int)dyn));
    ELP_LAUNCH(c, "radix_scatter", (k_radix_scatter_t<512, PAIRS>), dim3(ntiles), dim3(512), dyn, kin, vin, kdst, vdst, n, shift, ghist, c->radix_state.p,
               c->radix_epoch, ticket, c->err_flag.p, n_dev, fuse, bnd);
  } else {
    ELP_LAUNCH(c, "radix_scatter", (k_radix_scatter_t<256, PAIRS>), dim3(ntiles), dim3(256), 0, kin, vin, kdst, vdst, n, shift, ghist, c->radix_state.p,
               c->radix_epoch, ticket, c->err_flag.p, n_dev, fuse, bnd);
  }
  return 0;
}
static int radix_scatter_launch(elp_ctx *c, uint64_t n, const uint64_t *kin, const uint32_t *vin, uint64_t *kdst, uint32_t *vdst, int shift,
                                const unsigned long long *ghist, uint32_t *ticket, const uint32_t *n_dev, RadixBounds bnd = RadixBounds{}) {
  return radix_scatter_launch_t<true>(c, n, kin, vin, kdst, vdst, shift, ghist, ticket, n_dev, 0, bnd);
}

int radix_sort_fused(elp_ctx *c, const uint64_t *keycol, uint64_t n, int key_bits, int idx_bits, uint64_t *buf0, uint64_t *buf1, uint64_t **out) {
  if (n >= 0xFFFFFFFFull || key_bits + idx_bits > 64 || key_bits < 1 || idx_bits < 1) return set_error(c, ELP_ERR_UNSUPPORTED, "radix sort: bad size");
  const int ndigits = (key_bits + 7) / 8;
  unsigned long long *ghist;
  ELP_TRY(ensure(c, c->radix_hist, 8 * 256 + 4));
  ghist = c->radix_hist.p;
  ELP_HIP(c, hipMemsetAsync(ghist, 0, (8 * 256 + 4) * sizeof(unsigned long long), c->stream));
  uint32_t *ticket = reinterpret_cast<uint32_t *>(ghist + 8 * 256);
  const unsigned hb = (unsigned)std::min<uint64_t>((n + 255) / 256, 2048);
  if (ndigits <= 2) ELP_LAUNCH(c, "radix_hist_all", k_radix_hist_all<2>, dim3(hb), dim3(256), 0, keycol, n, ghist, (const uint32_t *)nullptr);
  else if (ndigits <= 4) ELP_LAUNCH(c, "radix_hist_all", k_radix_hist_all<4>, dim3(hb), dim3(256), 0, keycol, n, ghist, (const uint32_t *)nullptr);
  else ELP_LAUNCH(c, "radix_hist_all", k_radix_hist_all<8>, dim3(hb), dim3(256), 0, keycol, n, ghist, (const uint32_t *)nullptr);
  ELP_TRY(radix_pass_setup(c, radix_tiles(c, n)));
  uint64_t *src = buf1, *dst = buf0;
  for (int d = 0; d < ndigits; d++) {
    ELP_TRY(radix_next_epoch(c));
    ELP_TRY(radix_scatter_launch_t<false>(c, n, d == 0 ? keycol : src, nullptr, dst, nullptr, idx_bits + 8 * d, (const unsigned long long *)(ghist + d * 256),
                                          ticket + d, nullptr, d == 0 ? idx_bits : 0));
    std::swap(src, dst);
  }
  *out = src;
  return 0;
}

int radix_sort_pairs_low(elp_ctx *c, uint64_t *keys, uint32_t *vals, uint64_t *keys_tmp, uint32_t *vals_tmp, uint64_t n, int ndigits,
                         uint64_t **keys_out, uint32_t **vals_out, const uint64_t *first_src, bool identity_vals, const uint32_t *n_dev, RadixBounds bnd) {
  *keys_out = keys;
  *vals_out = vals;
  if ((ndigits <= 0 || (n < 2 && !n_dev)) && !first_src && !identity_vals) return 0;
  if (ndigits <= 0) ndigits = 1;
  if (n >= 0xFFFFFFFFull || ndigits > 8) return set_error(c, ELP_ERR_UNSUPPORTED, "radix sort: bad size");
  unsigned long long *ghist;
  ELP_TRY(ensure(c, c->radix_hist, 8 * 256 + 4));
  ghist = c->radix_hist.p;
  ELP_HIP(c, hipMemsetAsync(ghist, 0, (8 * 256 + 4) * sizeof(unsigned long long), c->stream));
  uint32_t *ticket = reinterpret_cast<uint32_t *>(ghist + 8 * 256);
  const unsigned hb = (unsigned)std::min<uint64_t>((n + 255) / 256, 2048);
  if (ndigits <= 2) ELP_LAUNCH(c, "radix_hist_all", k_radix_hist_all<2>, dim3(hb), dim3(256), 0, (const uint64_t *)(first_src ? first_src : keys), n, ghist, n_dev);
  else if (ndigits <= 4) ELP_LAUNCH(c, "radix_hist_all", k_radix_hist_all<4>, dim3(hb), dim3(256), 0, (const uint64_t *)(first_src ? first_src : keys), n, ghist, n_dev);
  else ELP_LAUNCH(c, "radix_hist_all", k_radix_hist_all<8>, dim3(hb), dim3(256), 0, (const uint64_t *)(first_src ? first_src : keys), n, ghist, n_dev);
  ELP_TRY(radix_pass_setup(c, radix_tiles(c, n)));
  uint64_t *ksrc = keys, *kdst = keys_tmp;
  uint32_t *vsrc = vals, *vdst = vals_tmp;
  for (int d = 0; d < ndigits; d++) {
    ELP_TRY(radix_next_epoch(c));
    const uint64_t *kin = (d == 0 && first_src) ? first_src : ksrc;
    const uint32_t *vin = (d == 0 && identity_vals) ? nullptr : vsrc;
    ELP_TRY(radix_scatter_launch(c, n, kin, vin, kdst, vdst, 8 * d, (const unsigned long long *)(ghist + d * 256), ticket + d, n_dev,
                                 d == ndigits - 1 ? bnd : RadixBounds{}));
    std::swap(ksrc, kdst);
    std::swap(vsrc, vdst);
  }
  *keys_out = ksrc;
  *vals_out = vsrc;
  return 0;
}

int radix_sort_pairs(elp_ctx *c, uint64_t *keys, uint32_t *vals, uint64_t *keys_tmp, uint32_t *vals_tmp, uint64_t n, uint64_t **keys_out,
                     uint32_t **vals_out) {
  *keys_out = keys;
  *vals_out = vals;
  if (n < 2) return 0;
  if (n >= 0xFFFFFFFFull) return set_error(c, ELP_ERR_UNSUPPORTED, "radix sort: more than 2^32-1 elements");
  unsigned long long *ghist;
  ELP_TRY(ensure(c, c->radix_hist, 8 * 256 + 4));
  ghist = c->radix_hist.p;
  ELP_HIP(c, hipMemsetAsync(ghist, 0, (8 * 256 + 4) * sizeof(unsigned long long), c->stream));
  uint32_t *ticket = reinterpret_cast<uint32_t *>(ghist + 8 * 256);
  unsigned hb = (unsigned)std::min<uint64_t>((n + 255) / 256, 2048);
  ELP_LAUNCH(c, "radix_hist_all", k_radix_hist_all<8>, dim3(hb), dim3(256), 0, (const uint64_t *)keys, n, ghist, (const uint32_t *)nullptr);
  unsigned long long hh[8 * 256];
  ELP_HIP(c, hipMemcpyAsync(hh, ghist, sizeof hh, hipMemcpyDeviceToHost, c->stream));
  ELP_HIP(c, elp::stream_wait(c->stream));
  ELP_TRY(radix_pass_setup(c, radix_tiles(c, n)));
  uint64_t *ksrc = keys, *kdst = keys_tmp;
  uint32_t *vsrc = vals, *vdst = vals_tmp;
  for (int d = 0; d < 8; d++) {
    bool live = true;
    for (int b = 0; b < 256; b++)
      if (hh[d * 256 + b] == n) { live = false; break; }
    if (!live) continue;
    ELP_TRY(radix_next_epoch(c));
    ELP_TRY(radix_scatter_launch(c, n, ksrc, vsrc, kdst, vdst, 8 * d, (const unsigned long long *)(ghist + d * 256), ticket + d, nullptr));
    std::swap(ksrc, kdst);
    std::swap(vsrc, vdst);
  }
  *keys_out = ksrc;
  *vals_out = vsrc;
  return 0;
}

}
```

### elprep_amd/csrc/sort.hip

```cpp
#include <cstdlib>

#include "apply_rec.hpp"
#include "common.hpp"
#include "flat.hpp"

namespace elp {

constexpr int TIE_SMALL = 48;

__global__ __launch_bounds__(256) void k_adapt_fixed(uint64_t n, const int32_t *__restrict__ pos, const int32_t *__restrict__ refid,
                                                     const uint16_t *__restrict__ flag, const uint64_t *__restrict__ cigar_off,
                                                     const uint32_t *__restrict__ cigar, int32_t *__restrict__ upos, int32_t *__restrict__ score,
                                                     uint64_t *__restrict__ key, uint32_t n_ref, int pos_bits,
                                                     const uint8_t *__restrict__ has_sr) {
  uint64_t i = (uint64_t)blockIdx.x * blockDim.x + threadIdx.x;
  if (i >= n) return;
  const uint16_t f = flag[i];
  const int32_t p = pos[i];
  const int32_t r = refid[i];
  const uint64_t ru = has_sr[i] ? (uint64_t)n_ref + 1 : (r < 0 ? (uint64_t)n_ref : (uint64_t)(uint32_t)r);
  key[i] = (ru << (pos_bits + 1)) | ((uint64_t)(uint32_t)p << 1) | ((f & F_REVERSED) ? 1ull : 0ull);
  int32_t up = 0;
  if ((f & (F_UNMAPPED | F_SECONDARY | F_SUPPLEMENTARY)) == 0) {
    const uint64_t c0 = cigar_off[i], c1 = cigar_off[i + 1];
// ... 277 lines not shown
      }
    }
  }
  for (int d = 32; d >= 1; d >>= 1) {
    m[0] |= __shfl_xor(m[0], d, 64);
    m[1] |= __shfl_xor(m[1], d, 64);
    m[2] |= __shfl_xor(m[2], d, 64);
  }
  if ((threadIdx.x & 63) == 0) {
    const unsigned long long lo = (unsigned long long)m[0] | ((unsigned long long)m[1] << 32);
    if (lo) atomicOr(&qmask[0], lo);
    if (m[2]) atomicOr(&qmask[1], (unsigned long long)m[2]);
  }
}

__global__ __launch_bounds__(256) void k_flat_index(const uint64_t *__restrict__ qual_off, uint64_t n_reads, uint64_t ntiles,
                                                    uint32_t *__restrict__ tile_first) {
  const uint64_t t = (uint64_t)blockIdx.x * blockDim.x + threadIdx.x;
  if (t > ntiles) return;
  if (t == ntiles) { tile_first[t] = (uint32_t)n_reads; return; }
  const uint64_t x = t * FL_TILE;
  uint64_t lo = 0, hi = n_reads;
  while (lo < hi) {
    const uint64_t mid = lo + (hi - lo) / 2;
    if (qual_off[mid] >= x) hi = mid; else lo = mid + 1;
  }
  tile_first[t] = (uint32_t)lo;
}

int ensure_flat_index(elp_ctx *c) {
  if (c->flat_index_n == c->n && c->flat_index_bytes == c->qual_bytes && c->n) return 0;
  const uint64_t ntiles = (c->qual_bytes + FL_TILE - 1) / FL_TILE;
  ELP_TRY(ensure(c, c->tile_first, ntiles + 2));
  if (c->n)
    ELP_LAUNCH(c, "flat_index", k_flat_index, dim3(blocks_for(ntiles + 1, 256)), dim3(256), 0, (const uint64_t *)c->qual_off.p, c->n, ntiles,
               c->tile_first.p);
  c->flat_index_n = c->n;
  c->flat_index_bytes = c->qual_bytes;
  return 0;
}

__global__ __launch_bounds__(256) void k_uniform_check(uint64_t n, const uint64_t *__restrict__ qual_off, const uint64_t *__restrict__ seq_off,
                                                       const uint32_t *__restrict__ l_seq, uint64_t len, uint64_t sb, uint64_t seq_front, uint32_t *bad) {
  const uint64_t i = (uint64_t)blockIdx.x * blockDim.x + threadIdx.x;
  bool b = false;
  if (i < n) b = qual_off[i] != i * len || seq_off[i] != seq_front + i * sb || (uint64_t)l_seq[i] != len;
  if (i == n) b = qual_off[n] != n * len || seq_off[n] != seq_front + n * sb;
  if (__any(b) && (threadIdx.x & 63) == 0) atomicOr(bad, 1u);
}
int ensure_uniform_len(elp_ctx *c) {
  if (c->uniform_n == c->n && c->uniform_bytes == c->qual_bytes && c->n) return 0;
  c->uniform_len = 0;
  c->uniform_n = c->n;
  c->uniform_bytes = c->qual_bytes;
  if (!c->n || c->qual_bytes % c->n) return 0;
  const uint64_t len = c->qual_bytes / c->n;
  if (len == 0 || len > 0x3FFFFFull) return 0;
  uint32_t *bad = c->err_flag.p + 2;
  ELP_HIP(c, hipMemsetAsync(bad, 0, 4, c->stream));
  ELP_LAUNCH(c, "uniform_check", k_uniform_check, dim3(blocks_for(c->n + 1, 256)), dim3(256), 0, c->n, (const uint64_t *)c->qual_off.p,
             (const uint64_t *)c->seq_off.p, (const uint32_t *)c->l_seq.p, len, (len + 1) / 2, (uint64_t)elp_ctx::SEQ_FRONT, bad);
  uint32_t hb = 0;
  ELP_HIP(c, hipMemcpyAsync(&hb, bad, 4, hipMemcpyDeviceToHost, c->stream));
  ELP_HIP(c, elp::stream_wait(c->stream));
  ELP_HIP(c, hipMemsetAsync(bad, 0, 4, c->stream));
  if (!hb) c->uniform_len = (uint32_t)len;
  return 0;
}

int adapt_quality_error(elp_ctx *c) {
  return set_error(c, ELP_ERR_DATA, "Invalid QUAL character (phred > 93) in a duplicate-marking candidate (reference: log.Panic, filters/mark-duplicates.go:64-66)");
}

static int adapt_resolve(elp_ctx *c) {
  if (!c->adapt_pending) return 0;
  uint32_t w[ADAPT_WORDS];
  ELP_HIP(c, hipMemcpyAsync(w, c->adapt_err.p, sizeof w, hipMemcpyDeviceToHost, c->stream));
  ELP_HIP(c, elp::stream_wait(c->stream));
  adapt_note(c, w);
  return 0;
}
void adapt_note(elp_ctx *c, const uint32_t *words) {
  c->adapt_pending = false;
  if (words[0] & 1u) c->adapt_bad_qual = true;
  if (c->adapt_sampled) {
    c->adapt_qmask[0] = (unsigned long long)words[2] | ((unsigned long long)words[3] << 32);
    c->adapt_qmask[1] = (unsigned long long)words[4] | ((unsigned long long)words[5] << 32);
    c->adapt_qmask_valid = true;
  }
}
int adapt_begin(elp_ctx *c, int *pos_bits_out) {
  ELP_HIP(c, hipSetDevice(c->device));
  const uint64_t n = c->n;
  ELP_TRY(ensure_flat_index(c));
  ELP_TRY(ensure(c, c->upos, n + 1));
  ELP_TRY(ensure(c, c->score, n + 1));
  ELP_TRY(ensure(c, c->key, n + 1));
  ELP_TRY(ensure(c, c->qbounds, n + 1));
  ELP_TRY(ensure(c, c->adapt_err, ADAPT_WORDS + 2));
  ELP_HIP(c, hipMemsetAsync(c->adapt_err.p, 0, ADAPT_WORDS * sizeof(uint32_t), c->stream));
  c->adapt_bad_qual = false;
  c->adapt_pending = false;
  c->adapt_sampled = c->adapt_qmask_valid = false;
  c->apply_recs_valid = false;
  c->adapt_epoch++;
  int pos_bits = 1;
  while (pos_bits < 32 && (c->max_pos >> pos_bits) != 0) pos_bits++;
  int ref_bits = 1;
  while (ref_bits < 32 && (((uint32_t)c->n_ref + 1u) >> ref_bits) != 0) ref_bits++;
  c->key_bits = ref_bits + pos_bits + 1;
  *pos_bits_out = pos_bits;
  return 0;
}
int adapt_scores(elp_ctx *c) {
  const uint64_t n = c->n;
  if (!n) return 0;
  if (!c->qual_bytes) {
    ELP_HIP(c, hipMemsetAsync(c->qbounds.p, 0, n * sizeof(uint64_t), c->stream));
    ELP_HIP(c, hipMemsetAsync(c->score.p, 0, n * sizeof(int32_t), c->stream));
    return 0;
  }
  ELP_TRY(ensure_uniform_len(c));
  if (c->uniform_len && score_uniform_ok(c->uniform_len) && c->tune.score_kernel != 1) {
    ELP_TRY(score_uniform(c));
  } else {
    ELP_HIP(c, hipMemsetAsync(c->score.p, 0, n * sizeof(int32_t), c->stream));
    const unsigned grid = (unsigned)std::min<uint64_t>(flat_steps<ScoreBody>(c->qual_bytes), (uint64_t)c->n_cu * 4);
    ELP_LAUNCH(c, "adapt_score_flat", k_score_flat, dim3(grid), dim3(FL_THREADS), 0, n, (const uint64_t *)c->qual_off.p, (const uint8_t *)c->qual.p,
               c->qual_bytes, (const uint32_t *)c->tile_first.p, (const uint16_t *)c->flag.p, c->score.p, c->qbounds.p, c->adapt_err.p);
  }
  c->adapt_pending = true;
  return 0;
}
int ensure_adapted(elp_ctx *c, bool check_quals) {
  if (c->adapted) {
    if (check_quals) ELP_TRY(adapt_resolve(c));
    return (check_quals && c->adapt_bad_qual) ? adapt_quality_error(c) : 0;
  }
  int pos_bits = 1;
  ELP_TRY(adapt_begin(c, &pos_bits));
  const uint64_t n = c->n;
  if (n) {
    ELP_LAUNCH(c, "adapt_fixed", k_adapt_fixed, dim3(blocks_for(n, 256)), dim3(256), 0, n, (const int32_t *)c->pos.p, (const int32_t *)c->refid.p,
               (const uint16_t *)c->flag.p, (const uint64_t *)c->cigar_off.p, (const uint32_t *)c->cigar.p, c->upos.p, c->score.p, c->key.p,
               (uint32_t)c->n_ref, pos_bits, (const uint8_t *)c->has_sr.p);
    ELP_TRY(adapt_scores(c));
  }
  c->adapted = true;
  if (check_quals) ELP_TRY(adapt_resolve(c));
  return (check_quals && c->adapt_bad_qual) ? adapt_quality_error(c) : 0;
}

int ensure_qual_present(elp_ctx *c, bool exact) {
  if (c->have_qual_present) return 0;
  c->qual_present[0] = c->qual_present[1] = 0;
  if (!exact && c->tune.qual_hint != 1 && c->adapted && c->adapt_sampled) {
    ELP_TRY(adapt_resolve(c));
    c->qual_present[0] = c->adapt_qmask[0];
    c->qual_present[1] = c->adapt_qmask[1];
  } else if (c->qual_bytes && (exact || c->tune.qual_hint != 1)) {
    unsigned long long *qm;
    ELP_TRY(scratch(c, 6, 4, &qm));
    ELP_HIP(c, hipMemsetAsync(qm, 0, 16, c->stream));
    const uint64_t ntiles = (c->qual_bytes + FL_TILE - 1) / FL_TILE;
    const uint64_t stride = exact ? 1 : std::min<uint64_t>(16, std::max<uint64_t>(1, ntiles / 2048));
    const unsigned grid = (unsigned)std::min<uint64_t>((ntiles + stride - 1) / stride, 2048);
    ELP_LAUNCH(c, "qual_present_sample", k_qual_present_sample, dim3(grid), dim3(256), 0, (const uint8_t *)c->qual.p, c->qual_bytes, stride,
               (exact || stride == 1) ? FL_TILE : (uint64_t)4096, qm);
    ELP_HIP(c, hipMemcpyAsync(c->qual_present, qm, 16, hipMemcpyDeviceToHost, c->stream));
    ELP_HIP(c, elp::stream_wait(c->stream));
  }
  if (!exact && c->tune.qual_hint_drop >= 0) {
    const int q = c->tune.qual_hint_drop;
    if (q < 64) c->qual_present[0] &= ~(1ull << q);
    else if (q < 128) c->qual_present[1] &= ~(1ull << (q - 64));
  }
  c->have_qual_present = true;
  return 0;
}

struct TieCols {
  const uint64_t *qname_off;
  const uint8_t *qname;
  const uint16_t *flag;
  const uint8_t *mapq;
  const int32_t *next_refid, *pnext, *tlen;
  const uint8_t *rows = nullptr;
  uint32_t rw = 0;
};

__device__ inline bool tie_less(const TieCols &t, uint32_t a, uint32_t b) {
  const uint32_t la = (uint32_t)(t.qname_off[a + 1] - t.qname_off[a]), lb = (uint32_t)(t.qname_off[b + 1] - t.qname_off[b]);
  if (la != 0 && lb != 0) {
    int c = qname_cmp(t.qname, t.qname_off, a, b);
    if (c < 0) return true;
    if (c > 0) return false;
  }
  const uint16_t fa = mod_flag(t.flag[a]), fb = mod_flag(t.flag[b]);
  if (fa < fb) return true;
  if (fa > fb) return false;
  const uint8_t ma = t.mapq[a], mb = t.mapq[b];
  if (ma < mb) return true;
  if (ma > mb) return false;
  if ((t.flag[a] & F_MULTIPLE) && (t.flag[b] & F_MULTIPLE)) {
    const int32_t na = t.next_refid[a], nb = t.next_refid[b];
    if (na < nb) return true;
    if (na > nb) return false;
    const int32_t pa = t.pnext[a], pb = t.pnext[b];
    if (pa < pb) return true;
    if (pa > pb) return false;
  }
  return t.tlen[a] < t.tlen[b];
}

__global__ __launch_bounds__(256) void k_iota(uint32_t *v, uint64_t n) {
  uint64_t i = (uint64_t)blockIdx.x * blockDim.x + threadIdx.x;
  if (i < n) v[i] = (uint32_t)i;
}

struct SortedView {
  const uint64_t *__restrict__ keys;
  const uint32_t *__restrict__ vals;
  uint32_t idx_bits;
  __device__ __forceinline__ uint64_t key(uint64_t i) const { return idx_bits ? keys[i] >> idx_bits : keys[i]; }
  __device__ __forceinline__ uint32_t val(uint64_t i) const { return idx_bits ? (uint32_t)(keys[i] & ((1ull << idx_bits) - 1ull)) : vals[i]; }
};

constexpr int TS_TILES = 32;
__global__ __launch_bounds__(256) void k_tie_scan(uint64_t n, SortedView sv, uint32_t *__restrict__ perm_out, uint32_t *__restrict__ list, uint32_t *list_n,
                                                  uint32_t *__restrict__ bounds) {
  if (blockIdx.x == 0 && threadIdx.x < 4) bounds[threadIdx.x] = 0;
  __shared__ uint32_t lq[TS_TILES * 256];
  __shared__ uint32_t lcount, gbase;
  if (threadIdx.x == 0) lcount = 0;
  __syncthreads();
#pragma unroll 1
  for (int tile = 0; tile < TS_TILES; tile++) {
    const uint64_t i = ((uint64_t)blockIdx.x * TS_TILES + (uint64_t)tile) * 256 + threadIdx.x;
    bool in_run = false;
    if (i < n) {
      const uint64_t w = sv.keys[i], wp = i > 0 ? sv.keys[i - 1] : 0ull, wn = i + 1 < n ? sv.keys[i + 1] : 0ull;
      const uint64_t k = w >> sv.idx_bits, kp = i > 0 ? wp >> sv.idx_bits : ~k, kn = i + 1 < n ? wn >> sv.idx_bits : ~k;
      const uint32_t me = sv.idx_bits ? (uint32_t)(w & ((1ull << sv.idx_bits) - 1ull)) : sv.vals[i];
      in_run = kp == k || kn == k;
      if (!in_run) perm_out[i] = me;
    }
    const unsigned long long mask = __ballot(in_run);
    if (mask) {
      const int lane = threadIdx.x & 63, leader = __ffsll((long long)mask) - 1;
      uint32_t base = 0;
      if (lane == leader) base = atomicAdd(&lcount, (uint32_t)__popcll(mask));
      base = __shfl(base, leader, 64);
      if (in_run) lq[base + (uint32_t)__popcll(mask & ((1ull << lane) - 1ull))] = (uint32_t)i;
    }
  }
  __syncthreads();
  if (threadIdx.x == 0) gbase = lcount ? atomicAdd(list_n, lcount) : 0u;
  __syncthreads();
  for (uint32_t k = threadIdx.x; k < lcount; k += 256) list[gbase + k] = lq[k];
}
__global__ __launch_bounds__(256) void k_tie_small(uint64_t n, SortedView sv, uint32_t *__restrict__ perm_out, uint32_t *__restrict__ bounds ,
                                                   uint32_t bounds_cap, const uint32_t *__restrict__ list, const uint32_t *__restrict__ list_n, TieCols t) {
  const uint64_t j0 = (uint64_t)blockIdx.x * blockDim.x + threadIdx.x;
  if (j0 >= (uint64_t)*list_n) return;
  const uint64_t i = list[j0];
  const uint64_t k = sv.key(i);
  const uint32_t me = sv.val(i);
  uint64_t s = i, e = i + 1;
  bool large = false;
  while (s > 0 && sv.key(s - 1) == k) {
    s--;
    if (i - s >= (uint64_t)TIE_SMALL) { large = true; break; }
  }
  if (!large) {
    while (e < n && sv.key(e) == k) {
      e++;
      if (e - s > (uint64_t)TIE_SMALL) { large = true; break; }
    }
  }
  if (large) {
    perm_out[i] = me;
    if (i == 0 || sv.key(i - 1) != k) { const uint32_t at = atomicAdd(&bounds[0], 1u); if (at < bounds_cap) bounds[4 + at] = (uint32_t)i; }
    if (i + 1 == n || sv.key(i + 1) != k) { const uint32_t at = atomicAdd(&bounds[1], 1u); if (at < bounds_cap) bounds[4 + bounds_cap + at] = (uint32_t)i; }
    return;
  }
  if (e - s == 2) {
    if (i != s) return;
    const uint32_t other = sv.val(s + 1);
    const bool swap = tie_less(t, other, me);
    perm_out[s] = swap ? other : me;
    perm_out[s + 1] = swap ? me : other;
    return;
  }
  uint32_t rank = 0;
  for (uint64_t j = s; j < e; j++) {
    if (j == i) continue;
    const uint32_t other = sv.val(j);
    if (tie_less(t, other, me)) rank++;
    else if (j < i && !tie_less(t, me, other)) rank++;
  }
  perm_out[s + rank] = me;
}

__global__ __launch_bounds__(256) void k_large_fill(uint32_t nu, uint32_t nr, const uint32_t *__restrict__ start, const uint32_t *__restrict__ first,
                                                    SortedView sv, uint32_t *__restrict__ u_pos, uint32_t *__restrict__ u_read,
                                                    uint32_t *__restrict__ u_seg) {
  const uint32_t j = blockIdx.x * blockDim.x + threadIdx.x;
  if (j >= nu) return;
  uint32_t lo = 0, hi = nr;
  while (hi - lo > 1) {
    const uint32_t mid = (lo + hi) >> 1;
    if (first[mid] <= j) lo = mid; else hi = mid;
  }
  const uint32_t pos = start[lo] + (j - first[lo]);
  u_pos[j] = pos;
  u_read[j] = sv.val(pos);
  u_seg[j] = lo + 1u;
}

__device__ inline uint32_t material_byte(const TieCols &t, uint32_t r, uint32_t j, uint32_t maxq, uint32_t m = 0) {
  if (t.rows) return t.rows[(size_t)m * t.rw + j];
  if (j < maxq) {
    const uint64_t o = t.qname_off[r];
    const uint32_t l = (uint32_t)(t.qname_off[r + 1] - o);
    return j < l ? t.qname[o + j] : 0u;
  }
  const uint32_t f = j - maxq;
  const uint16_t fl = t.flag[r];
  if (f < 2) { const uint16_t m = mod_flag(fl); return f == 0 ? (m >> 8) : (m & 0xFF); }
  if (f == 2) return t.mapq[r];
  if (f < 11) {
    if (!(fl & F_MULTIPLE)) return 0u;
    const uint32_t v = (f < 7 ? (uint32_t)t.next_refid[r] : (uint32_t)t.pnext[r]) ^ 0x80000000u;
    const uint32_t b = (f < 7) ? (f - 3) : (f - 7);
    return (v >> (8 * (3 - b))) & 0xFF;
  }
  if (f < 15) {
    const uint32_t v = (uint32_t)t.tlen[r] ^ 0x80000000u;
    return (v >> (8 * (3 - (f - 11)))) & 0xFF;
  }
  return 0u;
}

__global__ __launch_bounds__(256) void k_material_rows(uint32_t nu, const uint32_t *__restrict__ u_read, uint32_t maxq, uint32_t nbytes, uint32_t rw,
                                                       uint8_t *__restrict__ rows, TieCols t ) {
  const uint64_t g = (uint64_t)blockIdx.x * blockDim.x + threadIdx.x;
  const uint32_t per = rw >> 3;
  const uint64_t m = g / per;
  if (m >= nu) return;
  const uint32_t k = (uint32_t)(g - m * per) * 8u, r = u_read[m];
  uint64_t v = 0;
  for (uint32_t i = 0; i < 8; i++)
    if (k + i < nbytes) v |= (uint64_t)material_byte(t, r, k + i, maxq) << (8 * i);
  reinterpret_cast<uint64_t *>(rows + m * rw)[k >> 3] = v;
}

__global__ __launch_bounds__(256) void k_material_live(uint32_t nu, const uint32_t *__restrict__ u_read, uint32_t maxq, uint32_t nbytes,
                                                       uint32_t *live, TieCols t) {
  __shared__ uint32_t acc[elp_ctx::TIE_LIVE_WORDS];
  if (threadIdx.x < elp_ctx::TIE_LIVE_WORDS) acc[threadIdx.x] = 0;
  __syncthreads();
  const uint32_t m = blockIdx.x * blockDim.x + threadIdx.x;
  if (m < nu && t.rows) {
    const uint64_t *a8 = reinterpret_cast<const uint64_t *>(t.rows + (size_t)m * t.rw), *b8 = reinterpret_cast<const uint64_t *>(t.rows);
    for (uint32_t k = 0; k < nbytes; k += 8) {
      uint64_t x = a8[k >> 3] ^ b8[k >> 3];
      if (x) {
        x |= x >> 4; x |= x >> 2; x |= x >> 1;
        x &= 0x0101010101010101ull;
        const uint32_t bits = (uint32_t)((x * 0x0102040810204080ull) >> 56);
        for (uint32_t i = 0; i < 8 && k + i < nbytes; i++)
          if ((bits >> i) & 1u) atomicOr(&acc[(k + i) >> 5], 1u << ((k + i) & 31));
      }
    }
  } else if (m < nu) {
    const uint32_t r = u_read[m], r0 = u_read[0];
    const uint64_t oa = t.qname_off[r], ob = t.qname_off[r0];
    const uint32_t la = (uint32_t)(t.qname_off[r + 1] - oa), lb = (uint32_t)(t.qname_off[r0 + 1] - ob);
    for (uint32_t k = 0; k < maxq; k += 8) {
      const uint64_t a = k < la ? low_bytes(load8(t.qname + oa + k), la - k) : 0ull;
      const uint64_t b = k < lb ? low_bytes(load8(t.qname + ob + k), lb - k) : 0ull;
      uint64_t x = a ^ b;
      if (x) {
        x |= x >> 4; x |= x >> 2; x |= x >> 1;
        x &= 0x0101010101010101ull;
        const uint32_t bits = (uint32_t)((x * 0x0102040810204080ull) >> 56);
        for (uint32_t i = 0; i < 8 && k + i < maxq; i++)
          if ((bits >> i) & 1u) atomicOr(&acc[(k + i) >> 5], 1u << ((k + i) & 31));
      }
    }
    for (uint32_t j = maxq; j < nbytes; j++)
      if (material_byte(t, r, j, maxq) != material_byte(t, r0, j, maxq)) atomicOr(&acc[j >> 5], 1u << (j & 31));
  }
  __syncthreads();
  if (threadIdx.x < elp_ctx::TIE_LIVE_WORDS && acc[threadIdx.x]) atomicOr(&live[threadIdx.x], acc[threadIdx.x]);
}

constexpr int TIE_MAX_PACKED = 96;
struct TiePosList { uint16_t pos[TIE_MAX_PACKED]; uint32_t n; };
__global__ __launch_bounds__(256) void k_material_values(uint32_t nu, const uint32_t *__restrict__ u_read, TiePosList lp, uint32_t maxq,
                                                         uint32_t *vals , TieCols t) {
  __shared__ uint32_t acc[TIE_MAX_PACKED * 8];
  for (uint32_t k = threadIdx.x; k < lp.n * 8; k += blockDim.x) acc[k] = 0;
  __syncthreads();
  for (uint32_t m = blockIdx.x * blockDim.x + threadIdx.x; m < nu; m += gridDim.x * blockDim.x) {
    const uint32_t r = u_read[m];
    for (uint32_t k = 0; k < lp.n; k++) {
      const uint32_t v = material_byte(t, r, lp.pos[k], maxq, m);
      const uint32_t bit = 1u << (v & 31u);
      uint32_t *w = &acc[k * 8 + (v >> 5)];
      if (!(*w & bit)) atomicOr(w, bit);
    }
  }
  __syncthreads();
  for (uint32_t k = threadIdx.x; k < lp.n * 8; k += blockDim.x)
    if (acc[k]) atomicOr(&vals[k], acc[k]);
}
struct TiePacked { uint16_t pos[64]; uint8_t shift[64]; uint8_t slot[64]; uint32_t n; };
__global__ __launch_bounds__(256) void k_material_keys_packed(uint32_t nu, const uint32_t *__restrict__ vals, const uint32_t *__restrict__ u_read,
                                                              TiePacked sel, const uint8_t *__restrict__ lut, uint32_t maxq, uint64_t *__restrict__ keys,
                                                              TieCols t, const uint32_t *__restrict__ u_seg, uint32_t seg_shift) {
  uint32_t j = blockIdx.x * blockDim.x + threadIdx.x;
  if (j >= nu) return;
  const uint32_t mem = vals[j], r = u_read[mem];
  uint64_t k = u_seg ? (uint64_t)u_seg[mem] << seg_shift : 0ull;
  for (uint32_t b = 0; b < sel.n; b++) k |= (uint64_t)lut[(uint32_t)sel.slot[b] * 256u + material_byte(t, r, sel.pos[b], maxq, mem)] << sel.shift[b];
  keys[j] = k;
}

struct TieSel { uint16_t pos[8]; uint32_t n; };
__global__ __launch_bounds__(256) void k_material_keys_sel(uint32_t nu, const uint32_t *__restrict__ vals, const uint32_t *__restrict__ u_read,
                                                           TieSel sel, uint32_t maxq, uint64_t *__restrict__ keys, TieCols t) {
  uint32_t j = blockIdx.x * blockDim.x + threadIdx.x;
  if (j >= nu) return;
  const uint32_t mem = vals[j], r = u_read[mem];
  uint64_t k = 0;
  for (uint32_t b = 0; b < sel.n; b++) k = (k << 8) | material_byte(t, r, sel.pos[b], maxq, mem);
  keys[j] = k;
}

__global__ __launch_bounds__(256) void k_seg_keys(uint32_t nu, const uint32_t *__restrict__ vals, const uint32_t *__restrict__ u_seg_incl,
                                                  uint64_t *__restrict__ keys) {
  uint32_t j = blockIdx.x * blockDim.x + threadIdx.x;
  if (j < nu) keys[j] = (uint64_t)u_seg_incl[vals[j]];
}


__device__ inline int material_cmp(const TieCols &t, uint32_t ma, uint32_t ra, uint32_t mb, uint32_t rb, uint32_t nbytes, uint32_t maxq) {
  if (t.rows) {
    const uint64_t *a8 = reinterpret_cast<const uint64_t *>(t.rows + (size_t)ma * t.rw), *b8 = reinterpret_cast<const uint64_t *>(t.rows + (size_t)mb * t.rw);
    for (uint32_t k = 0; k < nbytes; k += 8) {
      const uint64_t x = a8[k >> 3], y = b8[k >> 3];
      if (x != y) return __builtin_bswap64(x) < __builtin_bswap64(y) ? -1 : 1;
    }
    return 0;
  }
  for (uint32_t j = 0; j < nbytes; j++) {
    const uint32_t x = material_byte(t, ra, j, maxq), y = material_byte(t, rb, j, maxq);
    if (x != y) return x < y ? -1 : 1;
  }
  return 0;
}
constexpr uint32_t LT_CAP = 1024;
__global__ __launch_bounds__(256) void k_large_ties(uint32_t nu, const uint64_t *__restrict__ keys, const uint32_t *__restrict__ vals,
                                                    uint32_t *__restrict__ vals_out, const uint32_t *__restrict__ u_read, uint32_t nbytes, uint32_t maxq,
                                                    uint32_t *over, TieCols t) {
  const uint32_t j = blockIdx.x * blockDim.x + threadIdx.x;
  if (j >= nu) return;
  const uint64_t k = keys[j];
  const uint32_t me = vals[j];
  const bool eq_prev = j > 0 && keys[j - 1] == k, eq_next = j + 1 < nu && keys[j + 1] == k;
  if (!eq_prev && !eq_next) { vals_out[j] = me; return; }
  uint32_t s = j, e = j + 1;
  bool large = false;
  while (s > 0 && keys[s - 1] == k) {
    s--;
    if (j - s >= LT_CAP) { large = true; break; }
  }
  while (!large && e < nu && keys[e] == k) {
    e++;
    if (e - s > LT_CAP) large = true;
  }
  if (large) {
    vals_out[j] = me;
    if (!eq_prev) atomicOr(over, 1u);
    return;
  }
  const uint32_t rme = u_read[me];
  uint32_t rank = 0;
  for (uint32_t i = s; i < e; i++) {
    if (i == j) continue;
    const uint32_t other = vals[i];
    const int c = material_cmp(t, other, u_read[other], me, rme, nbytes, maxq);
    if (c < 0 || (c == 0 && other < me)) rank++;
  }
  vals_out[s + rank] = me;
}

__global__ __launch_bounds__(256) void k_large_scatter(uint32_t nu, const uint32_t *__restrict__ vals_sorted, const uint32_t *__restrict__ u_pos,
                                                       const uint32_t *__restrict__ u_read, uint32_t *__restrict__ perm_out) {
  uint32_t j = blockIdx.x * blockDim.x + threadIdx.x;
  if (j < nu) perm_out[u_pos[j]] = u_read[vals_sorted[j]];
}

static int sort_impl(elp_ctx *c, uint64_t *presorted = nullptr ) {
  const uint64_t n = c->n;
  ELP_TRY(ensure_adapted(c, false));
  ELP_TRY(ensure(c, c->perm, n + 1));
  if (n == 0) { c->sorted = true; return 0; }
  uint64_t *kbuf;
  uint32_t *vbuf, *flags;
  ELP_TRY(scratch(c, 0, 2 * n + 8, &kbuf));
  ELP_TRY(scratch(c, 1, 2 * n + 8, &vbuf));
  ELP_TRY(scratch(c, 2, 2 * n + 8, &flags));
  uint64_t *k0 = kbuf, *k1 = kbuf + n;
  uint32_t *v0 = vbuf, *v1 = vbuf + n;
  uint64_t *ks;
  uint32_t *vs = nullptr;
  int idx_bits = 1;
  while (idx_bits < 32 && (n >> idx_bits) != 0) idx_bits++;
  const bool words = c->tune.sort_pairs != 1 && c->key_bits >= 1 && c->key_bits + idx_bits <= 64;
  if (words && presorted) ks = presorted;
  else if (words) ELP_TRY(radix_sort_fused(c, c->key.p, n, c->key_bits, idx_bits, k0, k1, &ks));
  else {
    ProfScope ps(c, "sort_pairs_");
    ELP_TRY(radix_sort_pairs_low(c, k0, v0, k1, v1, n, (c->key_bits + 7) / 8, &ks, &vs, c->key.p, true));
  }
  const SortedView sv{ks, vs, words ? (uint32_t)idx_bits : 0u};
  TieCols t{c->qname_off.p, c->qname.p, c->flag.p, c->mapq.p, c->next_refid.p, c->pnext.p, c->tlen.p};
  const uint32_t bounds_cap = (uint32_t)std::min<uint64_t>(n / TIE_SMALL + 16, (2 * n + 8 - 4) / 2);
  uint32_t *bounds = flags;
  {
    uint32_t *list = (vs == v0) ? v1 : v0, *list_n = c->err_flag.p + 3;
    ELP_HIP(c, hipMemsetAsync(list_n, 0, 4, c->stream));
    ELP_LAUNCH(c, "tie_scan", k_tie_scan, dim3(blocks_for(n, 256 * TS_TILES)), dim3(256), 0, n, sv, c->perm.p, list, list_n, bounds);
    ELP_LAUNCH(c, "tie_small", k_tie_small, dim3(blocks_for(n, 256)), dim3(256), 0, n, sv, c->perm.p, bounds, bounds_cap, (const uint32_t *)list, (const uint32_t *)list_n, t);
    ELP_HIP(c, hipMemsetAsync(list_n, 0, 4, c->stream));
  }
  constexpr uint32_t TIE_HEAD = 256;
  std::vector<uint32_t> hb(4 + 2 * (size_t)TIE_HEAD), starts, ends;
  {
    const uint32_t head = std::min<uint32_t>(TIE_HEAD, bounds_cap);
    ELP_HIP(c, hipMemcpyAsync(hb.data(), bounds, (4 + (size_t)head) * 4, hipMemcpyDeviceToHost, c->stream));
    ELP_HIP(c, hipMemcpyAsync(hb.data() + 4 + TIE_HEAD, bounds + 4 + bounds_cap, (size_t)head * 4, hipMemcpyDeviceToHost, c->stream));
    ELP_HIP(c, elp::stream_wait(c->stream));
  }
  const uint32_t nr = hb[0];
  if (nr != hb[1] || nr > bounds_cap) return set_error(c, ELP_ERR_HIP, "coordinate sort: %u starts and %u ends of long runs (internal)", hb[0], hb[1]);
  uint32_t nu = 0;
  if (nr > 0) {
    starts.resize(nr); ends.resize(nr);
    if (nr <= TIE_HEAD) {
      std::copy(hb.begin() + 4, hb.begin() + 4 + nr, starts.begin());
      std::copy(hb.begin() + 4 + TIE_HEAD, hb.begin() + 4 + TIE_HEAD + nr, ends.begin());
    } else {
      ELP_HIP(c, hipMemcpyAsync(starts.data(), bounds + 4, (size_t)nr * 4, hipMemcpyDeviceToHost, c->stream));
      ELP_HIP(c, hipMemcpyAsync(ends.data(), bounds + 4 + bounds_cap, (size_t)nr * 4, hipMemcpyDeviceToHost, c->stream));
      ELP_HIP(c, elp::stream_wait(c->stream));
    }
    std::sort(starts.begin(), starts.end());
    std::sort(ends.begin(), ends.end());
    std::vector<uint32_t> first(nr + 1);
    uint64_t total = 0;
    for (uint32_t r = 0; r < nr; r++) {
      if (ends[r] < starts[r] || (r + 1 < nr && starts[r + 1] <= ends[r])) return set_error(c, ELP_ERR_HIP, "coordinate sort: long runs overlap (internal)");
      first[r] = (uint32_t)total;
      total += (uint64_t)ends[r] - starts[r] + 1;
    }
    first[nr] = (uint32_t)total;
    nu = (uint32_t)total;
    const uint32_t rw = (c->max_qname_len + 15u + 15u) & ~15u;
    const bool use_rows = (uint64_t)nu * rw <= (512ull << 20);
    const size_t u_words = ((size_t)5 * nu + 2 * (size_t)nr + 64 + 3) & ~(size_t)3;
    uint32_t *u;
    ELP_TRY(scratch(c, 3, u_words + (use_rows ? ((size_t)nu * rw + 64) / 4 : 0), &u));
    uint32_t *u_pos = u, *u_read = u + nu, *u_seg = u + 2 * (size_t)nu, *uv0 = u + 3 * (size_t)nu, *uv1 = u + 4 * (size_t)nu, *d_start = u + 5 * (size_t)nu,
             *d_first = d_start + nr;
    uint64_t *uk;
    ELP_TRY(scratch(c, 4, (size_t)2 * nu + 16, &uk));
    uint64_t *uk0 = uk, *uk1 = uk + nu;
    ELP_HIP(c, hipMemcpyAsync(d_start, starts.data(), (size_t)nr * 4, hipMemcpyHostToDevice, c->stream));
    ELP_HIP(c, hipMemcpyAsync(d_first, first.data(), ((size_t)nr + 1) * 4, hipMemcpyHostToDevice, c->stream));
    ELP_LAUNCH(c, "large_fill", k_large_fill, dim3(blocks_for(nu, 256)), dim3(256), 0, nu, nr, (const uint32_t *)d_start, (const uint32_t *)d_first, sv, u_pos, u_read, u_seg);
    ELP_LAUNCH(c, "iota", k_iota, dim3(blocks_for(nu, 256)), dim3(256), 0, uv0, (uint64_t)nu);
    const uint32_t maxq = c->max_qname_len;
    const uint32_t m_bytes = maxq + 15;
    static_assert(elp_ctx::MAX_QNAME + 15 <= 32 * elp_ctx::TIE_LIVE_WORDS, "live-position bitmap too small");
    ELP_TRY(ensure(c, c->tie_live, elp_ctx::TIE_LIVE_WORDS));
    ELP_HIP(c, hipMemsetAsync(c->tie_live.p, 0, elp_ctx::TIE_LIVE_WORDS * sizeof(uint32_t), c->stream));
    if (use_rows) {
      uint8_t *rows = reinterpret_cast<uint8_t *>(u + u_words);
      ELP_LAUNCH(c, "material_rows", k_material_rows, dim3(blocks_for((uint64_t)nu * (rw >> 3), 256)), dim3(256), 0, nu, (const uint32_t *)u_read, maxq, m_bytes, rw,
                 rows, t);
      t.rows = rows;
      t.rw = rw;
    }
    ELP_LAUNCH(c, "material_live", k_material_live, dim3(blocks_for(nu, 256)), dim3(256), 0, nu, (const uint32_t *)u_read, maxq, m_bytes,
               c->tie_live.p, t);
    uint32_t live[elp_ctx::TIE_LIVE_WORDS];
    ELP_HIP(c, hipMemcpyAsync(live, c->tie_live.p, sizeof live, hipMemcpyDeviceToHost, c->stream));
    ELP_HIP(c, elp::stream_wait(c->stream));
    std::vector<uint16_t> lp;
    for (uint32_t j = 0; j < m_bytes; j++)
      if ((live[j >> 5] >> (j & 31)) & 1u) lp.push_back((uint16_t)j);
    uint32_t *vcur = uv0, *vtmp = uv1;
    bool packed_done = false;
    if (!lp.empty() && lp.size() <= (size_t)TIE_MAX_PACKED) {
      TiePosList pl;
      pl.n = (uint32_t)lp.size();
      for (size_t k = 0; k < lp.size(); k++) pl.pos[k] = lp[k];
      uint32_t *d_vals;
      ELP_TRY(scratch(c, 5, (size_t)TIE_MAX_PACKED * 8 + (size_t)TIE_MAX_PACKED * 64 + 64, &d_vals));
      uint8_t *d_lut = reinterpret_cast<uint8_t *>(d_vals + TIE_MAX_PACKED * 8);
      ELP_HIP(c, hipMemsetAsync(d_vals, 0, (size_t)pl.n * 8 * 4, c->stream));
      ELP_LAUNCH(c, "material_values", k_material_values, dim3(std::min(blocks_for(nu, 256), 1024u)), dim3(256), 0, nu, (const uint32_t *)u_read, pl, maxq, d_vals, t);
      std::vector<uint32_t> hv((size_t)pl.n * 8);
      ELP_HIP(c, hipMemcpyAsync(hv.data(), d_vals, hv.size() * 4, hipMemcpyDeviceToHost, c->stream));
      ELP_HIP(c, elp::stream_wait(c->stream));
      std::vector<uint8_t> lut((size_t)pl.n * 256, 0);
      std::vector<int> bits(pl.n);
      for (uint32_t k = 0; k < pl.n; k++) {
        int rank = 0;
        for (int v = 0; v < 256; v++)
          if ((hv[(size_t)k * 8 + (v >> 5)] >> (v & 31)) & 1u) lut[(size_t)k * 256 + v] = (uint8_t)rank++;
        int b = 1;
        while ((1 << b) < rank) b++;
        bits[k] = b;
      }
      ELP_HIP(c, hipMemcpyAsync(d_lut, lut.data(), lut.size(), hipMemcpyHostToDevice, c->stream));
      int segbits = 0;
      while (nr > 1 && (1u << segbits) <= nr) segbits++;
      if (c->tune.tie_rounds != 1 && segbits + bits[0] <= 64) {
        TiePacked sel;
        memset(&sel, 0, sizeof sel);
        int total = 0, hi = 0;
        while (hi < (int)pl.n && hi < 64 && segbits + total + bits[hi] <= 64) total += bits[hi++];
        int sh = total;
        for (int k = 0; k < hi; k++) {
          sh -= bits[k];
          sel.pos[sel.n] = pl.pos[k]; sel.shift[sel.n] = (uint8_t)sh; sel.slot[sel.n] = (uint8_t)k;
          sel.n++;
        }
        ELP_LAUNCH(c, "material_keys", k_material_keys_packed, dim3(blocks_for(nu, 256)), dim3(256), 0, nu, (const uint32_t *)vcur, (const uint32_t *)u_read,
                   sel, (const uint8_t *)d_lut, maxq, uk0, t, (const uint32_t *)(nr > 1 ? u_seg : nullptr), (uint32_t)total);
        uint64_t *ko;
        uint32_t *vo;
        ELP_TRY(radix_sort_pairs_low(c, uk0, vcur, uk1, vtmp, nu, (segbits + total + 7) / 8, &ko, &vo));
        if (vo != vcur) { vtmp = vcur; vcur = vo; }
        bool settled = hi == (int)pl.n;
        if (!settled) {
          uint32_t *over = c->err_flag.p + 3;
          ELP_LAUNCH(c, "large_ties", k_large_ties, dim3(blocks_for(nu, 256)), dim3(256), 0, nu, (const uint64_t *)ko, (const uint32_t *)vcur, vtmp,
                     (const uint32_t *)u_read, m_bytes, maxq, over, t);
          std::swap(vcur, vtmp);
          ELP_LAUNCH(c, "large_scatter", k_large_scatter, dim3(blocks_for(nu, 256)), dim3(256), 0, nu, (const uint32_t *)vcur, (const uint32_t *)u_pos,
                     (const uint32_t *)u_read, c->perm.p);
          uint32_t h_over = 0;
          ELP_HIP(c, hipMemcpyAsync(&h_over, over, 4, hipMemcpyDeviceToHost, c->stream));
          ELP_HIP(c, elp::stream_wait(c->stream));
          settled = h_over == 0;
          if (!settled) {
            ELP_HIP(c, hipMemsetAsync(over, 0, 4, c->stream));
            ELP_LAUNCH(c, "iota", k_iota, dim3(blocks_for(nu, 256)), dim3(256), 0, uv0, (uint64_t)nu);
            vcur = uv0; vtmp = uv1;
          }
        } else {
          ELP_LAUNCH(c, "large_scatter", k_large_scatter, dim3(blocks_for(nu, 256)), dim3(256), 0, nu, (const uint32_t *)vcur, (const uint32_t *)u_pos,
                     (const uint32_t *)u_read, c->perm.p);
        }
        if (settled) {
          c->radix_check_pending = true;
          c->sorted = true;
          return 0;
        }
      }
      for (int hi = (int)pl.n; hi > 0;) {
        TiePacked sel;
        memset(&sel, 0, sizeof sel);
        int total = 0, lo = hi;
        while (lo > 0 && total + bits[lo - 1] <= 64 && hi - lo < 64) { lo--; total += bits[lo]; }
        int sh = total;
        for (int k = lo; k < hi; k++) {
          sh -= bits[k];
          sel.pos[sel.n] = pl.pos[k]; sel.shift[sel.n] = (uint8_t)sh; sel.slot[sel.n] = (uint8_t)k;
          sel.n++;
        }
        ELP_LAUNCH(c, "material_keys", k_material_keys_packed, dim3(blocks_for(nu, 256)), dim3(256), 0, nu, (const uint32_t *)vcur, (const uint32_t *)u_read,
                   sel, (const uint8_t *)d_lut, maxq, uk0, t, (const uint32_t *)nullptr, 0u);
        uint64_t *ko;
        uint32_t *vo;
        ELP_TRY(radix_sort_pairs_low(c, uk0, vcur, uk1, vtmp, nu, (total + 7) / 8, &ko, &vo));
        if (vo != vcur) { vtmp = vcur; vcur = vo; }
        hi = lo;
      }
      packed_done = true;
    }
    for (size_t hi = packed_done ? 0 : lp.size(); hi > 0;) {
      const size_t lo = hi >= 8 ? hi - 8 : 0;
      TieSel sel;
      sel.n = (uint32_t)(hi - lo);
      for (size_t b = 0; b < 8; b++) sel.pos[b] = b < sel.n ? lp[lo + b] : 0;
      ELP_LAUNCH(c, "material_keys", k_material_keys_sel, dim3(blocks_for(nu, 256)), dim3(256), 0, nu, (const uint32_t *)vcur,
                 (const uint32_t *)u_read, sel, maxq, uk0, t);
      uint64_t *ko;
      uint32_t *vo;
      ELP_TRY(radix_sort_pairs_low(c, uk0, vcur, uk1, vtmp, nu, (int)sel.n, &ko, &vo));
      if (vo != vcur) { vtmp = vcur; vcur = vo; }
      hi = lo;
    }
    if (nr > 1) ELP_LAUNCH(c, "seg_keys", k_seg_keys, dim3(blocks_for(nu, 256)), dim3(256), 0, nu, (const uint32_t *)vcur, (const uint32_t *)u_seg, uk0);
    if (nr > 1) {
      uint64_t *ko;
      uint32_t *vo;
      ELP_TRY(radix_sort_pairs(c, uk0, vcur, uk1, vtmp, nu, &ko, &vo));
      if (vo != vcur) { vtmp = vcur; vcur = vo; }
    }
    ELP_LAUNCH(c, "large_scatter", k_large_scatter, dim3(blocks_for(nu, 256)), dim3(256), 0, nu, (const uint32_t *)vcur, (const uint32_t *)u_pos,
               (const uint32_t *)u_read, c->perm.p);
  }
  c->radix_check_pending = true;
  c->sorted = true;
  return 0;
}

}

namespace elp {
static int sort_on_side(elp_ctx *c) {
  ELP_TRY(ensure_adapted(c, false));
  ELP_TRY(ensure(c, c->perm, c->n + 1));
  elp_ctx *s = nullptr;
  ELP_TRY(side_lane(c, 1, &s));
  s->n = c->n; s->n_sr = c->n_sr; s->n_filtered = c->n_filtered; s->key_bits = c->key_bits; s->max_qname_len = c->max_qname_len; s->max_pos = c->max_pos;
  s->n_ref = c->n_ref; s->adapted = true; s->adapt_pending = false; s->sorted = false;
  s->key.p = c->key.p; s->flag.p = c->flag.p; s->mapq.p = c->mapq.p; s->next_refid.p = c->next_refid.p; s->pnext.p = c->pnext.p; s->tlen.p = c->tlen.p;
  s->qname_off.p = c->qname_off.p; s->qname.p = c->qname.p; s->has_sr.p = c->has_sr.p;
  s->perm.p = c->perm.p; s->perm.cap = c->perm.cap;
  int ib = 1;
  while (ib < 32 && (c->n >> ib) != 0) ib++;
  uint64_t *pre = (c->presort_ks && c->presort_epoch == c->adapt_epoch && c->presort_n == c->n && c->presort_idx_bits == ib && c->tune.sort_pairs != 1) ? c->presort_ks : nullptr;
  c->presort_epoch = ~0ull;
  int rc = sort_impl(s, pre);
  s->key.p = nullptr; s->flag.p = nullptr; s->mapq.p = nullptr; s->next_refid.p = nullptr; s->pnext.p = nullptr; s->tlen.p = nullptr;
  s->qname_off.p = nullptr; s->qname.p = nullptr; s->has_sr.p = nullptr;
  s->perm.p = nullptr; s->perm.cap = 0;
  if (rc == 0) rc = radix_check(s);
  if (rc != 0) {
    (void)elp::stream_wait(s->stream);
    c->err = s->err;
    return rc;
  }
  ELP_TRY(side_join(c, 1));
  c->sorted = s->sorted;
  return 0;
}
}

namespace elp {
int sort_presort(elp_ctx *c) {
  const uint64_t n = c->n;
  c->presort_epoch = ~0ull;
  if (!c->sort_ahead || n < 2 || !c->adapted || c->tune.sort_pairs == 1) return 0;
  int idx_bits = 1;
  while (idx_bits < 32 && (n >> idx_bits) != 0) idx_bits++;
  if (c->key_bits < 1 || c->key_bits + idx_bits > 64) return 0;
  elp_ctx *s = nullptr;
  ELP_TRY(side_lane(c, 1, &s));
  s->n = n; s->key_bits = c->key_bits;
  const int tile_saved = s->tune.radix_tile;
  if (!s->tune.radix_tile) s->tune.radix_tile = c->tune.presort_tile >= 1 && c->tune.presort_tile <= 3 ? c->tune.presort_tile : 2;
  uint64_t *kbuf, *ks = nullptr;
  int rc = scratch(s, 0, 2 * n + 8, &kbuf);
  if (rc == 0) rc = radix_sort_fused(s, c->key.p, n, c->key_bits, idx_bits, kbuf, kbuf + n, &ks);
  s->tune.radix_tile = tile_saved;
  if (rc != 0) { c->err = s->err; return rc; }
  c->presort_ks = ks; c->presort_n = n; c->presort_idx_bits = idx_bits; c->presort_epoch = c->adapt_epoch;
  return 0;
}
}

extern "C" int elp_sort_ahead(elp_ctx *c, int on) {
  if (!c) return ELP_ERR_ARG;
  c->sort_ahead = on != 0;
  if (!on) c->presort_epoch = ~0ull;
  return 0;
}

extern "C" int elp_sort_coordinate(elp_ctx *c) {
  if (!c) return ELP_ERR_ARG;
  ELP_HIP(c, hipSetDevice(c->device));
  c->sorted = c->sorted_qname = false;
  return elp::sort_on_side(c);
}
```

Measured before the change: 2351.

## Drive duplicate-metrics and tie-sort sizes from device plans to skip host syncs

The optical-duplicate metrics path and the coordinate-sort tie-breaking path now remember capacity bounds learnt on an earlier call. On later calls they run with device-side counts: small plan kernels clamp sizes, and scan and radix kernels read n from device memory, so the host no longer copies back counts and waits mid-pipeline. An overflow or large-set flag is checked once at the end, and the call re-runs on the old synchronous path if the learnt bounds were too small. The cost is extra kernel launches sized to capacity caps rather than exact counts, larger scratch reservations, and a possible full re-execution when a guess is exceeded.

```diff
diff --git a/elprep_amd/csrc/common.hpp b/elprep_amd/csrc/common.hpp
--- a/elprep_amd/csrc/common.hpp
+++ b/elprep_amd/csrc/common.hpp
@@ -128,6 +128,13 @@
   elp::DVec<uint32_t> mate;
   elp::DVec<uint32_t> pair_win;
 
+  bool mx_learnt = false, mx_large_seen = false;
+  uint64_t mx_cap_list = 0, mx_cap_members = 0;
+
+  bool tie_learnt = false, tie_had_runs = false;
+  uint64_t tie_cap_u = 0;
+  uint32_t tie_cap_r = 0;
+
   std::vector<uint8_t *> h_ref_seq;
   std::vector<int64_t> h_ref_seq_len;
   std::vector<int32_t *> h_sites;
@@ -222,6 +229,8 @@
     int bgzf_stored = 0;
     int apply_wgs = 0;
     int presort_tile = 0;
+    int tie_plan = 0;
+    int mx_plan = 0;
     int side_priority = 0;
   } tune;
 
@@ -405,6 +414,8 @@
                          uint64_t **keys_out, uint32_t **vals_out, const uint64_t *first_src = nullptr, bool identity_vals = false,
                          const uint32_t *n_dev = nullptr , RadixBounds bnd = RadixBounds{});
 int exclusive_scan_u32(elp_ctx *c, const uint32_t *in, uint32_t *out, uint64_t n, uint32_t *total_host );
+int exclusive_scan_u32_dev(elp_ctx *c, const uint32_t *in, uint32_t *out, uint64_t n_bound, const uint32_t *n_dev, uint32_t *total_dev);
+int radix_reserve(elp_ctx *c, uint64_t n_bound);
 int ensure_adapted(elp_ctx *c, bool check_quals = true);
 int adapt_begin(elp_ctx *c, int *pos_bits);
 int adapt_scores(elp_ctx *c);
diff --git a/elprep_amd/csrc/ctx.hip b/elprep_amd/csrc/ctx.hip
--- a/elprep_amd/csrc/ctx.hip
+++ b/elprep_amd/csrc/ctx.hip
@@ -584,6 +584,8 @@
   } else if (k == "apply_wgs") c->tune.apply_wgs = v;
   else if (k == "presort_tile") c->tune.presort_tile = v;
   else if (k == "side_priority") c->tune.side_priority = v;
+  else if (k == "mx_plan") c->tune.mx_plan = v;
+  else if (k == "tie_plan") c->tune.tie_plan = v;
   else return set_error(c, ELP_ERR_ARG, "elp_set_tuning: unknown key '%s'", key);
   return 0;
 }
diff --git a/elprep_amd/csrc/metrics.hip b/elprep_amd/csrc/metrics.hip
--- a/elprep_amd/csrc/metrics.hip
+++ b/elprep_amd/csrc/metrics.hip
@@ -140,12 +140,26 @@
     if (lds_ctr[k]) atomicAdd(&pair_reads[k - nrow], (unsigned long long)lds_ctr[k]);
 }
 
-__global__ __launch_bounds__(256) void k_opt_heads(uint32_t L, const uint64_t *__restrict__ ks, uint32_t *__restrict__ head) {
+enum MxPlan { MXP_LIST_RAW = 0, MXP_LIST = 1, MXP_GROUPS = 2, MXP_MEMBERS = 3, MXP_LARGE = 4, MXP_OVER = 5, MXP_WORDS = 8 };
+__global__ void k_mx_plan(uint32_t *plan, int stage, uint32_t cap) {
+  if (stage == 0) {
+    const uint32_t L = plan[MXP_LIST_RAW];
+    if (L > cap) plan[MXP_OVER] = 1u;
+    plan[MXP_LIST] = L > cap ? 0u : L;
+  } else {
+    const uint32_t total = plan[MXP_LIST] + plan[MXP_GROUPS];
+    if (total > cap) { plan[MXP_OVER] |= 2u; plan[MXP_LIST] = 0; }
+    plan[MXP_MEMBERS] = total > cap ? 0u : total;
+  }
+}
+__global__ __launch_bounds__(256) void k_opt_heads(uint32_t L, const uint64_t *__restrict__ ks, uint32_t *__restrict__ head, const uint32_t *__restrict__ plan) {
+  if (plan) L = plan[MXP_LIST];
   const uint32_t j = blockIdx.x * blockDim.x + threadIdx.x;
   if (j < L) head[j] = (j == 0 || ks[j] != ks[j - 1]) ? 1u : 0u;
 }
 __global__ __launch_bounds__(256) void k_opt_starts(uint32_t L, const uint32_t *__restrict__ head, const uint32_t *__restrict__ gidx,
-                                                    uint32_t *__restrict__ gstart, uint32_t G) {
+                                                    uint32_t *__restrict__ gstart, uint32_t G, const uint32_t *__restrict__ plan) {
+  if (plan) { L = plan[MXP_LIST]; G = plan[MXP_GROUPS]; }
   const uint32_t j = blockIdx.x * blockDim.x + threadIdx.x;
   if (j >= L) return;
   if (head[j]) gstart[gidx[j]] = j;
@@ -216,7 +230,8 @@
 __global__ __launch_bounds__(256) void k_opt_slots(MxCols m, uint32_t L, const uint64_t *__restrict__ ks, const uint32_t *__restrict__ vs,
                                                    const uint32_t *__restrict__ head, const uint32_t *__restrict__ gidx,
                                                    const uint32_t *__restrict__ gstart, uint32_t *__restrict__ mread, uint2 *__restrict__ ginfo,
-                                                   uint32_t *__restrict__ mset) {
+                                                   uint32_t *__restrict__ mset, const uint32_t *__restrict__ plan) {
+  if (plan) L = plan[MXP_LIST];
   const uint32_t j = blockIdx.x * blockDim.x + threadIdx.x;
   if (j >= L) return;
   const bool is_head = head[j] != 0;
@@ -232,7 +247,9 @@
     ginfo[oslot] = make_uint2(gstart[g + 1] - j0 + 1, origin);
   }
 }
-__global__ __launch_bounds__(256) void k_opt_fill(MxCols m, uint32_t total, const uint32_t *__restrict__ mread, Member *__restrict__ members) {
+__global__ __launch_bounds__(256) void k_opt_fill(MxCols m, uint32_t total, const uint32_t *__restrict__ mread, Member *__restrict__ members,
+                                                  const uint32_t *__restrict__ plan) {
+  if (plan) total = plan[MXP_MEMBERS];
   const uint32_t s = blockIdx.x * blockDim.x + threadIdx.x;
   if (s >= total) return;
   members[s] = make_member(m, mread[s]);
@@ -256,7 +273,9 @@
 __global__ __launch_bounds__(128) void k_opt_eval(MxCols m, uint32_t total, const uint2 *__restrict__ ginfo, const Member *__restrict__ members,
                                                   uint32_t *__restrict__ parent, long long dist, unsigned long long *__restrict__ ctr,
                                                   uint32_t *err, unsigned long long *__restrict__ hist, int hist_len, int lds_bins,
-                                                  uint32_t *__restrict__ linfo, uint32_t *__restrict__ lcount, uint32_t *n_large) {
+                                                  uint32_t *__restrict__ linfo, uint32_t *__restrict__ lcount, uint32_t *n_large,
+                                                  const uint32_t *plan ) {
+  if (plan) total = plan[MXP_MEMBERS];
   extern __shared__ unsigned int lds_opt[];
   unsigned int *lds_h = lds_opt + (m.n_lib + 1);
   const int n_h = hist ? (m.n_lib + 1) * 3 * lds_bins : 0;
@@ -443,13 +462,20 @@
   const size_t npr = (size_t)n_split * (size_t)(c->n_lib + 1);
   if (((size_t)ncell + npr) * sizeof(unsigned int) > 46000)
     return set_error(c, ELP_ERR_UNSUPPORTED, "elp_dup_metrics: %d split ids x %d libraries in one context", n_split, c->n_lib + 1);
+  constexpr size_t plan_ull = MXP_WORDS * sizeof(uint32_t) / sizeof(unsigned long long);
+  const size_t nctr = (size_t)ncell + norg + nhist + npr;
   unsigned long long *ctr;
-  ELP_TRY(scratch(c, 0, (size_t)ncell + norg + nhist + npr + 8, &ctr));
+  ELP_TRY(scratch(c, 0, nctr + plan_ull + 8, &ctr));
   unsigned long long *origins = ctr + ncell, *hist = hist_host ? origins + norg : nullptr, *pair_reads = ctr + ncell + norg + nhist;
+  uint32_t *plan = reinterpret_cast<uint32_t *>(ctr + nctr);
   hipStream_t st = c->stream;
-  ELP_HIP(c, hipMemsetAsync(ctr, 0, ((size_t)ncell + norg + nhist + npr) * sizeof(unsigned long long), st));
   int lds_bins = hist_host ? std::min(hist_len, 32) : 0;
   if ((size_t)(c->n_lib + 1) * (1 + 3 * (size_t)lds_bins) * sizeof(unsigned int) > 32768) lds_bins = 0;
+  std::vector<unsigned long long> h(nctr + plan_ull);
+  uint32_t e[4];
+  bool dev = n > 0 && c->tune.mx_plan != 1 && c->mx_learnt && !c->mx_large_seen;
+  for (;; dev = false) {
+  ELP_HIP(c, hipMemsetAsync(ctr, 0, (nctr + plan_ull) * sizeof(unsigned long long), st));
   if (n) {
     MxCols m{n, c->refid.p, c->flag.p, c->rgid.p, c->rg_lib.p, c->upos.p, c->qname_off.p, c->qname.p, c->mate.p, c->pair_win.p, c->n_lib,
              c->has_sr.p, c->split.p, n_split};
@@ -460,16 +486,22 @@
     uint64_t *pk = reinterpret_cast<uint64_t *>(gs);
     uint32_t *pv = gs + 4 * lcap;
     uint32_t *mailbox = c->err_flag.p + 3;
-    ELP_HIP(c, hipMemsetAsync(mailbox, 0, 4, st));
+    const uint32_t *dplan = dev ? plan : nullptr;
+    if (!dev) ELP_HIP(c, hipMemsetAsync(mailbox, 0, 4, st));
     const unsigned cgrid = (unsigned)std::min<uint64_t>(2048, (n + DC_STEP - 1) / DC_STEP);
     const uint64_t chunk = (((n + cgrid - 1) / cgrid) + DC_STEP - 1) / DC_STEP * DC_STEP;
     ELP_LAUNCH(c, "mx_counters", k_dup_counters, dim3(cgrid), dim3(256), ((size_t)ncell + npr) * sizeof(unsigned int), m, ctr, pair_reads, chunk, pk, pv,
-               mailbox);
+               dev ? plan + MXP_LIST_RAW : mailbox);
     uint32_t L = 0;
-    ELP_HIP(c, hipMemcpyAsync(&L, mailbox, 4, hipMemcpyDeviceToHost, st));
-    ELP_HIP(c, elp::stream_wait(st));
-    ELP_HIP(c, hipMemsetAsync(mailbox, 0, 4, st));
-    if ((size_t)L > lcap) return set_error(c, ELP_ERR_HIP, "elp_dup_metrics: more losing pairs than pairs");
+    if (dev) {
+      L = (uint32_t)std::min<uint64_t>(c->mx_cap_list, lcap);
+      ELP_LAUNCH(c, "mx_plan", k_mx_plan, dim3(1), dim3(1), 0, plan, 0, L);
+    } else {
+      ELP_HIP(c, hipMemcpyAsync(&L, mailbox, 4, hipMemcpyDeviceToHost, st));
+      ELP_HIP(c, elp::stream_wait(st));
+      ELP_HIP(c, hipMemsetAsync(mailbox, 0, 4, st));
+      if ((size_t)L > lcap) return set_error(c, ELP_ERR_HIP, "elp_dup_metrics: more losing pairs than pairs");
+    }
     uint32_t total = 0, G = 0;
     uint64_t *ks = pk;
     uint32_t *vs = pv, *head = nullptr, *gidx = nullptr, *gstart = nullptr;
@@ -478,43 +510,56 @@
       while (ndig < 4 && (n >> (8 * ndig)) != 0) ndig++;
       {
         ProfScope ps(c, "mx_");
-        ELP_TRY(radix_sort_pairs_low(c, pk, pv, pk + lcap, pv + lcap, L, ndig, &ks, &vs));
+        ELP_TRY(radix_sort_pairs_low(c, pk, pv, pk + lcap, pv + lcap, L, ndig, &ks, &vs, nullptr, false, dev ? plan + MXP_LIST : nullptr));
       }
       head = reinterpret_cast<uint32_t *>(ks == pk ? pk + lcap : pk);
       gidx = head + lcap;
       gstart = vs == pv ? pv + lcap : pv;
-      ELP_LAUNCH(c, "mx_opt_heads", k_opt_heads, dim3(blocks_for(L, 256)), dim3(256), 0, L, (const uint64_t *)ks, head);
+      ELP_LAUNCH(c, "mx_opt_heads", k_opt_heads, dim3(blocks_for(L, 256)), dim3(256), 0, L, (const uint64_t *)ks, head, dplan);
       {
         ProfScope ps(c, "mx_");
-        ELP_TRY(exclusive_scan_u32(c, head, gidx, L, &G));
-      }
-      ELP_LAUNCH(c, "mx_opt_starts", k_opt_starts, dim3(blocks_for(L, 256)), dim3(256), 0, L, (const uint32_t *)head, (const uint32_t *)gidx, gstart, G);
-      total = L + G;
-    }
+        if (dev) ELP_TRY(exclusive_scan_u32_dev(c, head, gidx, L, plan + MXP_LIST, plan + MXP_GROUPS));
+        else ELP_TRY(exclusive_scan_u32(c, head, gidx, L, &G));
+      }
+      if (dev) {
+        total = (uint32_t)std::min<uint64_t>(c->mx_cap_members, 2 * lcap);
+        ELP_LAUNCH(c, "mx_plan", k_mx_plan, dim3(1), dim3(1), 0, plan, 1, total);
+      } else {
+        total = L + G;
+        c->mx_cap_list = std::max<uint64_t>(c->mx_cap_list, (uint64_t)L + L / 8 + 4096);
+        c->mx_cap_members = std::max<uint64_t>(c->mx_cap_members, (uint64_t)total + total / 8 + 8192);
+        ELP_TRY(radix_reserve(c, std::min<uint64_t>(c->mx_cap_list, lcap)));
+      }
+      ELP_LAUNCH(c, "mx_opt_starts", k_opt_starts, dim3(blocks_for(L, 256)), dim3(256), 0, L, (const uint32_t *)head, (const uint32_t *)gidx, gstart, G, dplan);
+    }
+    uint32_t n_large = 0;
     if (total) {
       Member *members;
       uint32_t *wk, *mread;
       uint2 *ginfo;
       const size_t tp = ((size_t)total + 7) & ~(size_t)7;
-      ELP_TRY(scratch(c, 2, (size_t)total + 4, &members));
-      ELP_TRY(scratch(c, 3, 12 * tp + 16, &wk));
-      ELP_TRY(scratch(c, 4, (size_t)total + 4, &mread));
-      ELP_TRY(scratch(c, 5, (size_t)total + 4, &ginfo));
+      const size_t ta = std::max<size_t>(total, (size_t)std::min<uint64_t>(c->mx_cap_members, 2 * lcap)), tpa = (ta + 7) & ~(size_t)7;
+      ELP_TRY(scratch(c, 2, ta + 4, &members));
+      ELP_TRY(scratch(c, 3, 12 * tpa + 16, &wk));
+      ELP_TRY(scratch(c, 4, ta + 4, &mread));
+      ELP_TRY(scratch(c, 5, ta + 4, &ginfo));
       uint32_t *parent = wk, *mset = wk + tp, *linfo = wk + 2 * tp, *lcount = wk + 3 * tp, *lvals = wk + 6 * tp;
       unsigned long long *setcnt = reinterpret_cast<unsigned long long *>(wk + 4 * tp);
       uint64_t *lkeys = reinterpret_cast<uint64_t *>(wk + 8 * tp);
       ELP_HIP(c, hipMemsetAsync(ginfo, 0, (size_t)total * sizeof(uint2), st));
       ELP_HIP(c, hipMemsetAsync(linfo, 0, 4 * tp * sizeof(uint32_t), st));
       ELP_LAUNCH(c, "mx_opt_slots", k_opt_slots, dim3(blocks_for(L, 256)), dim3(256), 0, m, L, (const uint64_t *)ks, (const uint32_t *)vs,
-                 (const uint32_t *)head, (const uint32_t *)gidx, (const uint32_t *)gstart, mread, ginfo, mset);
-      ELP_LAUNCH(c, "mx_opt_fill", k_opt_fill, dim3(blocks_for(total, 256)), dim3(256), 0, m, total, (const uint32_t *)mread, members);
+                 (const uint32_t *)head, (const uint32_t *)gidx, (const uint32_t *)gstart, mread, ginfo, mset, dplan);
+      ELP_LAUNCH(c, "mx_opt_fill", k_opt_fill, dim3(blocks_for(total, 256)), dim3(256), 0, m, total, (const uint32_t *)mread, members, dplan);
       ELP_LAUNCH(c, "mx_opt_eval", k_opt_eval, dim3(std::min(blocks_for(total, 128), 2048u)), dim3(128),
                  (size_t)(c->n_lib + 1) * (1 + (hist ? 3 * (size_t)lds_bins : 0)) * sizeof(unsigned int), m, total, (const uint2 *)ginfo,
-                 (const Member *)members, parent, (long long)dist, ctr, c->err_flag.p, hist, hist_len, lds_bins, linfo, lcount, mailbox);
-      uint32_t n_large = 0;
+                 (const Member *)members, parent, (long long)dist, ctr, c->err_flag.p, hist, hist_len, lds_bins, linfo, lcount,
+                 dev ? plan + MXP_LARGE : mailbox, dplan);
+      if (!dev) {
       ELP_HIP(c, hipMemcpyAsync(&n_large, mailbox, 4, hipMemcpyDeviceToHost, st));
       ELP_HIP(c, elp::stream_wait(st));
       ELP_HIP(c, hipMemsetAsync(mailbox, 0, 4, st));
+      }
       if (n_large) {
         ELP_LAUNCH(c, "mx_large_list", k_large_list, dim3(blocks_for(total, 256)), dim3(256), 0, total, (const uint32_t *)mset, (const uint32_t *)linfo,
                    (const Member *)members, lkeys, lvals, mailbox);
@@ -537,13 +582,23 @@
                    (const uint32_t *)lcount, (const unsigned long long *)setcnt, ctr, hist, hist_len);
       }
     }
+    if (!dev) {
+      c->mx_learnt = true;
+      c->mx_large_seen = n_large != 0;
+      if (!L) c->mx_cap_list = std::max<uint64_t>(c->mx_cap_list, 4096), c->mx_cap_members = std::max<uint64_t>(c->mx_cap_members, 8192);
+    }
     if (hist)
       ELP_LAUNCH(c, "mx_origin_count", k_origin_count, dim3(std::min(grid, 2048u)), dim3(256), (c->n_lib + 1) * sizeof(unsigned int), m, origins);
   }
-  std::vector<unsigned long long> h((size_t)ncell + norg + nhist + npr);
   ELP_HIP(c, hipMemcpyAsync(h.data(), ctr, h.size() * sizeof(unsigned long long), hipMemcpyDeviceToHost, st));
-  uint32_t e[4];
   ELP_TRY(fetch_err(c, e));
+  if (dev) {
+    uint32_t hp[MXP_WORDS];
+    memcpy(hp, h.data() + nctr, sizeof hp);
+    if (hp[MXP_OVER] || hp[MXP_LARGE]) continue;
+  }
+  break;
+  }
   if (e[2]) {
     ELP_HIP(c, hipMemsetAsync(c->err_flag.p + 2, 0, 4, st));
     return set_error(c, ELP_ERR_DATA, "QNAME tile/x/y field is not an integer (reference: internal.ParseInt panics, filters/mark-optical-duplicates.go:55-61)");
diff --git a/elprep_amd/csrc/radix.hip b/elprep_amd/csrc/radix.hip
--- a/elprep_amd/csrc/radix.hip
+++ b/elprep_amd/csrc/radix.hip
@@ -32,8 +32,10 @@
 constexpr int SCAN_ITEMS = 8;
 constexpr int SCAN_TILE = 256 * SCAN_ITEMS;
 
-__global__ __launch_bounds__(256) void k_scan_reduce(const uint32_t *__restrict__ in, uint32_t *__restrict__ sums, uint64_t n) {
+__global__ __launch_bounds__(256) void k_scan_reduce(const uint32_t *__restrict__ in, uint32_t *__restrict__ sums, uint64_t n,
+                                                     const uint32_t *__restrict__ n_dev) {
   __shared__ uint32_t lds[8];
+  if (n_dev) n = *n_dev;
   uint64_t base = (uint64_t)blockIdx.x * SCAN_TILE + (uint64_t)threadIdx.x * SCAN_ITEMS;
   uint32_t s = 0;
 #pragma unroll
@@ -45,8 +47,9 @@
 }
 
 __global__ __launch_bounds__(256) void k_scan_down(const uint32_t *__restrict__ in, uint32_t *__restrict__ out,
-                                                   const uint32_t *__restrict__ block_base, uint64_t n) {
+                                                   const uint32_t *__restrict__ block_base, uint64_t n, const uint32_t *__restrict__ n_dev) {
   __shared__ uint32_t lds[8];
+  if (n_dev) n = *n_dev;
   uint64_t base = (uint64_t)blockIdx.x * SCAN_TILE + (uint64_t)threadIdx.x * SCAN_ITEMS;
   uint32_t v[SCAN_ITEMS];
   uint32_t s = 0;
@@ -64,7 +67,7 @@
   }
 }
 
-static int scan_levels(elp_ctx *c, const uint32_t *in, uint32_t *out, uint64_t n, uint32_t *total_dev) {
+static int scan_levels(elp_ctx *c, const uint32_t *in, uint32_t *out, uint64_t n, uint32_t *total_dev, const uint32_t *n_dev = nullptr) {
   if (n == 0) {
     if (total_dev) ELP_HIP(c, hipMemsetAsync(total_dev, 0, 4, c->stream));
     return 0;
@@ -86,7 +89,7 @@
   for (size_t k = 1; k < cnt.size(); k++) { sums[k] = pool + off; off += cnt[k] + 4; }
   const uint32_t *src = in;
   for (size_t k = 0; k + 1 < cnt.size(); k++) {
-    ELP_LAUNCH(c, "scan_reduce", k_scan_reduce, dim3((unsigned)cnt[k + 1]), dim3(256), 0, src, sums[k + 1], cnt[k]);
+    ELP_LAUNCH(c, "scan_reduce", k_scan_reduce, dim3((unsigned)cnt[k + 1]), dim3(256), 0, src, sums[k + 1], cnt[k], k == 0 ? n_dev : (const uint32_t *)nullptr);
     src = sums[k + 1];
   }
   size_t top = cnt.size() - 1;
@@ -94,10 +97,14 @@
   ELP_HIP(c, hipMemsetAsync(sums[top], 0, 4, c->stream));
   for (size_t k = top - 1; k >= 1; k--) {
     ELP_LAUNCH(c, "scan_down", k_scan_down, dim3((unsigned)cnt[k + 1]), dim3(256), 0, (const uint32_t *)sums[k], sums[k],
-               (const uint32_t *)sums[k + 1], cnt[k]);
-  }
-  ELP_LAUNCH(c, "scan_down", k_scan_down, dim3((unsigned)cnt[1]), dim3(256), 0, in, out, (const uint32_t *)sums[1], n);
-  return 0;
+               (const uint32_t *)sums[k + 1], cnt[k], (const uint32_t *)nullptr);
+  }
+  ELP_LAUNCH(c, "scan_down", k_scan_down, dim3((unsigned)cnt[1]), dim3(256), 0, in, out, (const uint32_t *)sums[1], n, n_dev);
+  return 0;
+}
+
+int exclusive_scan_u32_dev(elp_ctx *c, const uint32_t *in, uint32_t *out, uint64_t n_bound, const uint32_t *n_dev, uint32_t *total_dev) {
+  return scan_levels(c, in, out, n_bound, total_dev, n_dev);
 }
 
 int exclusive_scan_u32(elp_ctx *c, const uint32_t *in, uint32_t *out, uint64_t n, uint32_t *total_host) {
@@ -325,6 +332,18 @@
 static uint32_t radix_tiles(const elp_ctx *c, uint64_t n) {
   const uint64_t tile = (uint64_t)RS_TILE << radix_tile_shift(c, n);
   return (uint32_t)((n + tile - 1) / tile);
+}
+int radix_reserve(elp_ctx *c, uint64_t n_bound) {
+  if (n_bound == 0 || n_bound >= 0xFFFFFFFFull) return 0;
+  ELP_TRY(ensure(c, c->radix_hist, 8 * 256 + 4));
+  ELP_TRY(radix_pass_setup(c, radix_tiles(c, n_bound)));
+  size_t need = 0;
+  for (uint64_t cnt = n_bound;;) {
+    cnt = (cnt + SCAN_TILE - 1) / SCAN_TILE;
+    need += cnt + 4;
+    if (cnt <= 1) break;
+  }
+  return ensure(c, c->scan_pool, need + 16);
 }
 template <bool PAIRS>
 static int radix_scatter_launch_t(elp_ctx *c, uint64_t n, const uint64_t *kin, const uint32_t *vin, uint64_t *kdst, uint32_t *vdst, int shift,
diff --git a/elprep_amd/csrc/sort.hip b/elprep_amd/csrc/sort.hip
--- a/elprep_amd/csrc/sort.hip
+++ b/elprep_amd/csrc/sort.hip
@@ -603,11 +603,136 @@
   perm_out[s + rank] = me;
 }
 
+constexpr int TIE_MAX_PACKED = 96;
+struct TiePosList { uint16_t pos[TIE_MAX_PACKED]; uint32_t n; };
+struct TiePacked { uint16_t pos[64]; uint8_t shift[64]; uint8_t slot[64]; uint32_t n; };
+constexpr uint32_t TP_MAX_RUNS = 2048;
+enum : uint32_t {
+  TPS_UNSETTLED = 1,
+  TPS_CAPACITY = 2,
+  TPS_INTERNAL = 4,
+  TPS_UNPACKED = 8,
+  TPS_RUNS = 16
+};
+struct TiePlan {
+  uint32_t nr, nu;
+  uint32_t settled;
+  uint32_t seg_shift, use_seg;
+  TiePosList pl;
+  TiePacked sel;
+};
+
+__global__ __launch_bounds__(256) void k_tie_plan_runs(const uint32_t *__restrict__ bounds, uint32_t bounds_cap, uint32_t cap_r, uint32_t cap_u, TiePlan *plan,
+                                                       uint32_t *__restrict__ start, uint32_t *__restrict__ first, uint32_t *status, uint32_t *__restrict__ live,
+                                                       uint32_t *__restrict__ d_vals) {
+  __shared__ uint32_t s_in[TP_MAX_RUNS], e_in[TP_MAX_RUNS], s_out[TP_MAX_RUNS], e_out[TP_MAX_RUNS];
+  for (uint32_t k = threadIdx.x; k < elp_ctx::TIE_LIVE_WORDS; k += blockDim.x) live[k] = 0;
+  for (uint32_t k = threadIdx.x; k < (uint32_t)TIE_MAX_PACKED * 8; k += blockDim.x) d_vals[k] = 0;
+  const uint32_t nr = bounds[0];
+  uint32_t bad = 0;
+  if (nr != bounds[1] || nr > bounds_cap) bad = TPS_INTERNAL;
+  else if (nr > cap_r || nr > TP_MAX_RUNS) bad = TPS_CAPACITY;
+  if (bad || nr == 0) {
+    if (threadIdx.x == 0) {
+      plan->nr = 0; plan->nu = 0; plan->pl.n = 0; plan->sel.n = 0;
+      if (bad) *status = bad;
+    }
+    return;
+  }
+  for (uint32_t k = threadIdx.x; k < nr; k += blockDim.x) {
+    s_in[k] = bounds[4 + k];
+    e_in[k] = bounds[4 + bounds_cap + k];
+    s_out[k] = 0xFFFFFFFFu;
+    e_out[k] = 0;
+  }
+  __syncthreads();
+  for (uint32_t k = threadIdx.x; k < nr; k += blockDim.x) {
+    const uint32_t xs = s_in[k], xe = e_in[k];
+    uint32_t rs = 0, re = 0;
+    for (uint32_t j = 0; j < nr; j++) {
+      rs += s_in[j] < xs ? 1u : 0u;
+      re += e_in[j] < xe ? 1u : 0u;
+    }
+    s_out[rs] = xs;
+    e_out[re] = xe;
+  }
+  __syncthreads();
+  for (uint32_t k = threadIdx.x; k < nr; k += blockDim.x) start[k] = s_out[k];
+  if (threadIdx.x == 0) {
+    unsigned long long total = 0;
+    bool ok = true;
+    for (uint32_t r = 0; r < nr; r++) {
+      if (e_out[r] < s_out[r] || (r + 1 < nr && s_out[r + 1] <= e_out[r])) { ok = false; break; }
+      first[r] = (uint32_t)total;
+      total += (unsigned long long)e_out[r] - s_out[r] + 1ull;
+    }
+    first[nr] = (uint32_t)total;
+    const uint32_t st = !ok ? TPS_INTERNAL : total > (unsigned long long)cap_u ? TPS_CAPACITY : 0u;
+    plan->nr = st ? 0u : nr;
+    plan->nu = st ? 0u : (uint32_t)total;
+    plan->pl.n = 0; plan->sel.n = 0;
+    *status = st ? st : TPS_RUNS;
+  }
+}
+__global__ void k_tie_plan_live(TiePlan *plan, const uint32_t *__restrict__ live, uint32_t m_bytes, uint32_t *status) {
+  if (plan->nu == 0) return;
+  uint32_t nl = 0;
+  for (uint32_t j = 0; j < m_bytes; j++)
+    if ((live[j >> 5] >> (j & 31)) & 1u) {
+      if (nl < (uint32_t)TIE_MAX_PACKED) plan->pl.pos[nl] = (uint16_t)j;
+      nl++;
+    }
+  if (nl == 0 || nl > (uint32_t)TIE_MAX_PACKED) {
+    *status |= TPS_UNPACKED;
+    plan->nu = 0; plan->nr = 0;
+    nl = 0;
+  }
+  plan->pl.n = nl;
+}
+__global__ __launch_bounds__(256) void k_tie_plan_keys(TiePlan *plan, const uint32_t *__restrict__ vals, uint8_t *__restrict__ lut, uint32_t *status) {
+  __shared__ int bits[TIE_MAX_PACKED];
+  if (plan->nu == 0) return;
+  const uint32_t np = plan->pl.n, nr = plan->nr;
+  for (uint32_t k = threadIdx.x; k < np; k += blockDim.x) {
+    int rank = 0;
+    for (int v = 0; v < 256; v++) {
+      const bool there = (vals[(size_t)k * 8 + (v >> 5)] >> (v & 31)) & 1u;
+      lut[(size_t)k * 256 + v] = there ? (uint8_t)rank : (uint8_t)0;
+      rank += there ? 1 : 0;
+    }
+    int b = 1;
+    while ((1 << b) < rank) b++;
+    bits[k] = b;
+  }
+  __syncthreads();
+  if (threadIdx.x != 0) return;
+  int segbits = 0;
+  while (nr > 1 && (1u << segbits) <= nr) segbits++;
+  if (segbits + bits[0] > 64) {
+    *status |= TPS_UNPACKED;
+    plan->nu = 0; plan->nr = 0;
+    return;
+  }
+  int total = 0, hi = 0;
+  while (hi < (int)np && hi < 64 && segbits + total + bits[hi] <= 64) total += bits[hi++];
+  int sh = total;
+  for (int k = 0; k < hi; k++) {
+    sh -= bits[k];
+    plan->sel.pos[k] = plan->pl.pos[k]; plan->sel.shift[k] = (uint8_t)sh; plan->sel.slot[k] = (uint8_t)k;
+  }
+  plan->sel.n = (uint32_t)hi;
+  plan->settled = hi == (int)np ? 1u : 0u;
+  plan->seg_shift = (uint32_t)total;
+  plan->use_seg = nr > 1 ? 1u : 0u;
+}
+
 __global__ __launch_bounds__(256) void k_large_fill(uint32_t nu, uint32_t nr, const uint32_t *__restrict__ start, const uint32_t *__restrict__ first,
                                                     SortedView sv, uint32_t *__restrict__ u_pos, uint32_t *__restrict__ u_read,
-                                                    uint32_t *__restrict__ u_seg) {
+                                                    uint32_t *__restrict__ u_seg, const TiePlan *__restrict__ plan, uint32_t *__restrict__ iota) {
+  if (plan) { nu = plan->nu; nr = plan->nr; }
   const uint32_t j = blockIdx.x * blockDim.x + threadIdx.x;
   if (j >= nu) return;
+  if (iota) iota[j] = j;
   uint32_t lo = 0, hi = nr;
   while (hi - lo > 1) {
     const uint32_t mid = (lo + hi) >> 1;
@@ -644,7 +769,8 @@
 }
 
 __global__ __launch_bounds__(256) void k_material_rows(uint32_t nu, const uint32_t *__restrict__ u_read, uint32_t maxq, uint32_t nbytes, uint32_t rw,
-                                                       uint8_t *__restrict__ rows, TieCols t ) {
+                                                       uint8_t *__restrict__ rows, TieCols t , const TiePlan *__restrict__ plan) {
+  if (plan) nu = plan->nu;
   const uint64_t g = (uint64_t)blockIdx.x * blockDim.x + threadIdx.x;
   const uint32_t per = rw >> 3;
   const uint64_t m = g / per;
@@ -657,8 +783,10 @@
 }
 
 __global__ __launch_bounds__(256) void k_material_live(uint32_t nu, const uint32_t *__restrict__ u_read, uint32_t maxq, uint32_t nbytes,
-                                                       uint32_t *live, TieCols t) {
+                                                       uint32_t *live, TieCols t, const TiePlan *__restrict__ plan) {
   __shared__ uint32_t acc[elp_ctx::TIE_LIVE_WORDS];
+  if (plan) nu = plan->nu;
+  if ((uint64_t)blockIdx.x * blockDim.x >= nu) return;
   if (threadIdx.x < elp_ctx::TIE_LIVE_WORDS) acc[threadIdx.x] = 0;
   __syncthreads();
   const uint32_t m = blockIdx.x * blockDim.x + threadIdx.x;
@@ -697,11 +825,12 @@
   if (threadIdx.x < elp_ctx::TIE_LIVE_WORDS && acc[threadIdx.x]) atomicOr(&live[threadIdx.x], acc[threadIdx.x]);
 }
 
-constexpr int TIE_MAX_PACKED = 96;
-struct TiePosList { uint16_t pos[TIE_MAX_PACKED]; uint32_t n; };
-__global__ __launch_bounds__(256) void k_material_values(uint32_t nu, const uint32_t *__restrict__ u_read, TiePosList lp, uint32_t maxq,
-                                                         uint32_t *vals , TieCols t) {
+__global__ __launch_bounds__(256) void k_material_values(uint32_t nu, const uint32_t *__restrict__ u_read, TiePosList lp_arg, uint32_t maxq,
+                                                         uint32_t *vals , TieCols t, const TiePlan *__restrict__ plan) {
   __shared__ uint32_t acc[TIE_MAX_PACKED * 8];
+  if (plan) nu = plan->nu;
+  if ((uint64_t)blockIdx.x * blockDim.x >= nu) return;
+  const TiePosList &lp = plan ? plan->pl : lp_arg;
   for (uint32_t k = threadIdx.x; k < lp.n * 8; k += blockDim.x) acc[k] = 0;
   __syncthreads();
   for (uint32_t m = blockIdx.x * blockDim.x + threadIdx.x; m < nu; m += gridDim.x * blockDim.x) {
@@ -717,10 +846,14 @@
   for (uint32_t k = threadIdx.x; k < lp.n * 8; k += blockDim.x)
     if (acc[k]) atomicOr(&vals[k], acc[k]);
 }
-struct TiePacked { uint16_t pos[64]; uint8_t shift[64]; uint8_t slot[64]; uint32_t n; };
 __global__ __launch_bounds__(256) void k_material_keys_packed(uint32_t nu, const uint32_t *__restrict__ vals, const uint32_t *__restrict__ u_read,
-                                                              TiePacked sel, const uint8_t *__restrict__ lut, uint32_t maxq, uint64_t *__restrict__ keys,
-                                                              TieCols t, const uint32_t *__restrict__ u_seg, uint32_t seg_shift) {
+                                                              TiePacked sel_arg, const uint8_t *__restrict__ lut, uint32_t maxq, uint64_t *__restrict__ keys,
+                                                              TieCols t, const uint32_t *__restrict__ u_seg, uint32_t seg_shift, const TiePlan *__restrict__ plan) {
+  if (plan) {
+    nu = plan->nu; seg_shift = plan->seg_shift;
+    if (!plan->use_seg) u_seg = nullptr;
+  }
+  const TiePacked &sel = plan ? plan->sel : sel_arg;
   uint32_t j = blockIdx.x * blockDim.x + threadIdx.x;
   if (j >= nu) return;
   const uint32_t mem = vals[j], r = u_read[mem];
@@ -765,11 +898,13 @@
 constexpr uint32_t LT_CAP = 1024;
 __global__ __launch_bounds__(256) void k_large_ties(uint32_t nu, const uint64_t *__restrict__ keys, const uint32_t *__restrict__ vals,
                                                     uint32_t *__restrict__ vals_out, const uint32_t *__restrict__ u_read, uint32_t nbytes, uint32_t maxq,
-                                                    uint32_t *over, TieCols t) {
+                                                    uint32_t *over, TieCols t, const TiePlan *__restrict__ plan) {
+  if (plan) nu = plan->nu;
   const uint32_t j = blockIdx.x * blockDim.x + threadIdx.x;
   if (j >= nu) return;
   const uint64_t k = keys[j];
   const uint32_t me = vals[j];
+  if (plan && plan->settled) { vals_out[j] = me; return; }
   const bool eq_prev = j > 0 && keys[j - 1] == k, eq_next = j + 1 < nu && keys[j + 1] == k;
   if (!eq_prev && !eq_next) { vals_out[j] = me; return; }
   uint32_t s = j, e = j + 1;
@@ -799,10 +934,15 @@
 }
 
 __global__ __launch_bounds__(256) void k_large_scatter(uint32_t nu, const uint32_t *__restrict__ vals_sorted, const uint32_t *__restrict__ u_pos,
-                                                       const uint32_t *__restrict__ u_read, uint32_t *__restrict__ perm_out) {
+                                                       const uint32_t *__restrict__ u_read, uint32_t *__restrict__ perm_out, const TiePlan *__restrict__ plan) {
+  if (plan) nu = plan->nu;
   uint32_t j = blockIdx.x * blockDim.x + threadIdx.x;
   if (j < nu) perm_out[u_pos[j]] = u_read[vals_sorted[j]];
 }
+
+constexpr size_t PLAN_WORDS = (sizeof(TiePlan) + 15) / 16 * 4;
+static size_t tie_plan_u_words(uint32_t cap_u, uint32_t cap_r) { return ((size_t)5 * cap_u + 2 * (size_t)cap_r + 64 + 3) & ~(size_t)3; }
+static size_t tie_plan_words(uint32_t cap_u, uint32_t cap_r, uint32_t rw) { return tie_plan_u_words(cap_u, cap_r) + PLAN_WORDS + ((size_t)cap_u * rw + 64) / 4; }
 
 static int sort_impl(elp_ctx *c, uint64_t *presorted = nullptr ) {
   const uint64_t n = c->n;
@@ -838,6 +978,55 @@
     ELP_LAUNCH(c, "tie_small", k_tie_small, dim3(blocks_for(n, 256)), dim3(256), 0, n, sv, c->perm.p, bounds, bounds_cap, (const uint32_t *)list, (const uint32_t *)list_n, t);
     ELP_HIP(c, hipMemsetAsync(list_n, 0, 4, c->stream));
   }
+  const uint32_t maxq_p = c->max_qname_len, rw_p = (maxq_p + 15u + 15u) & ~15u;
+  if (c->tune.tie_plan != 1 && c->tune.tie_rounds != 1 && c->tie_learnt && c->tie_had_runs && (uint64_t)c->tie_cap_u * rw_p <= (512ull << 20)) {
+    const uint32_t CU = (uint32_t)std::min<uint64_t>(c->tie_cap_u, n), CR = std::min<uint32_t>(std::min<uint32_t>(c->tie_cap_r, TP_MAX_RUNS), bounds_cap);
+    const uint32_t m_bytes = maxq_p + 15;
+    const size_t u_words = tie_plan_u_words(CU, CR);
+    uint32_t *u, *d_vals, *status = c->err_flag.p + 3;
+    uint64_t *uk;
+    ELP_TRY(scratch(c, 3, tie_plan_words(CU, CR, rw_p), &u));
+    ELP_TRY(scratch(c, 4, (size_t)2 * CU + 16, &uk));
+    ELP_TRY(scratch(c, 5, (size_t)TIE_MAX_PACKED * 8 + (size_t)TIE_MAX_PACKED * 64 + 64, &d_vals));
+    ELP_TRY(ensure(c, c->tie_live, elp_ctx::TIE_LIVE_WORDS));
+    uint32_t *u_pos = u, *u_read = u + CU, *u_seg = u + 2 * (size_t)CU, *uv0 = u + 3 * (size_t)CU, *uv1 = u + 4 * (size_t)CU, *d_start = u + 5 * (size_t)CU,
+             *d_first = d_start + CR;
+    TiePlan *plan = reinterpret_cast<TiePlan *>(u + u_words);
+    const TiePlan *cplan = plan;
+    uint8_t *rows = reinterpret_cast<uint8_t *>(u + u_words + PLAN_WORDS), *d_lut = reinterpret_cast<uint8_t *>(d_vals + TIE_MAX_PACKED * 8);
+    uint64_t *uk0 = uk, *uk1 = uk + CU;
+    ELP_LAUNCH(c, "tie_plan", k_tie_plan_runs, dim3(1), dim3(256), 0, (const uint32_t *)bounds, bounds_cap, CR, CU, plan, d_start, d_first, status, c->tie_live.p, d_vals);
+    ELP_LAUNCH(c, "large_fill", k_large_fill, dim3(blocks_for(CU, 256)), dim3(256), 0, CU, CR, (const uint32_t *)d_start, (const uint32_t *)d_first, sv, u_pos, u_read,
+               u_seg, cplan, uv0);
+    ELP_LAUNCH(c, "material_rows", k_material_rows, dim3(blocks_for((uint64_t)CU * (rw_p >> 3), 256)), dim3(256), 0, CU, (const uint32_t *)u_read, maxq_p, m_bytes, rw_p,
+               rows, t, cplan);
+    TieCols tr = t;
+    tr.rows = rows;
+    tr.rw = rw_p;
+    ELP_LAUNCH(c, "material_live", k_material_live, dim3(blocks_for(CU, 256)), dim3(256), 0, CU, (const uint32_t *)u_read, maxq_p, m_bytes, c->tie_live.p, tr, cplan);
+    ELP_LAUNCH(c, "tie_plan", k_tie_plan_live, dim3(1), dim3(1), 0, plan, (const uint32_t *)c->tie_live.p, m_bytes, status);
+    ELP_LAUNCH(c, "material_values", k_material_values, dim3(std::min(blocks_for(CU, 256), 1024u)), dim3(256), 0, CU, (const uint32_t *)u_read, TiePosList{}, maxq_p,
+               d_vals, tr, cplan);
+    ELP_LAUNCH(c, "tie_plan", k_tie_plan_keys, dim3(1), dim3(256), 0, plan, (const uint32_t *)d_vals, d_lut, status);
+    ELP_LAUNCH(c, "material_keys", k_material_keys_packed, dim3(blocks_for(CU, 256)), dim3(256), 0, CU, (const uint32_t *)uv0, (const uint32_t *)u_read, TiePacked{},
+               (const uint8_t *)d_lut, maxq_p, uk0, tr, (const uint32_t *)u_seg, 0u, cplan);
+    uint64_t *ko;
+    uint32_t *vo;
+    ELP_TRY(radix_sort_pairs_low(c, uk0, uv0, uk1, uv1, CU, 8, &ko, &vo, nullptr, false, &plan->nu));
+    uint32_t *vtmp = vo == uv0 ? uv1 : uv0;
+    ELP_LAUNCH(c, "large_ties", k_large_ties, dim3(blocks_for(CU, 256)), dim3(256), 0, CU, (const uint64_t *)ko, (const uint32_t *)vo, vtmp, (const uint32_t *)u_read,
+               m_bytes, maxq_p, status, tr, cplan);
+    ELP_LAUNCH(c, "large_scatter", k_large_scatter, dim3(blocks_for(CU, 256)), dim3(256), 0, CU, (const uint32_t *)vtmp, (const uint32_t *)u_pos, (const uint32_t *)u_read,
+               c->perm.p, cplan);
+    uint32_t e[4];
+    ELP_TRY(fetch_err(c, e));
+    if (e[3]) ELP_HIP(c, hipMemsetAsync(status, 0, 4, c->stream));
+    c->tie_had_runs = (e[3] & TPS_RUNS) != 0;
+    if ((e[3] & ~TPS_RUNS) == 0) {
+      c->sorted = true;
+      return 0;
+    }
+  }
   constexpr uint32_t TIE_HEAD = 256;
   std::vector<uint32_t> hb(4 + 2 * (size_t)TIE_HEAD), starts, ends;
   {
@@ -849,6 +1038,8 @@
   const uint32_t nr = hb[0];
   if (nr != hb[1] || nr > bounds_cap) return set_error(c, ELP_ERR_HIP, "coordinate sort: %u starts and %u ends of long runs (internal)", hb[0], hb[1]);
   uint32_t nu = 0;
+  c->tie_learnt = true;
+  c->tie_had_runs = nr > 0;
   if (nr > 0) {
     starts.resize(nr); ends.resize(nr);
     if (nr <= TIE_HEAD) {
@@ -870,19 +1061,25 @@
     }
     first[nr] = (uint32_t)total;
     nu = (uint32_t)total;
+    c->tie_cap_u = std::max<uint64_t>(c->tie_cap_u, (uint64_t)nu + nu / 8 + 1024);
+    c->tie_cap_r = std::max<uint32_t>(c->tie_cap_r, nr + nr / 4 + 16);
+    const uint32_t cu_next = (uint32_t)std::min<uint64_t>(c->tie_cap_u, n), cr_next = std::min<uint32_t>(std::min<uint32_t>(c->tie_cap_r, TP_MAX_RUNS), bounds_cap);
+    const bool plan_next = (uint64_t)cu_next * rw_p <= (512ull << 20);
+    if (plan_next) ELP_TRY(radix_reserve(c, cu_next));
     const uint32_t rw = (c->max_qname_len + 15u + 15u) & ~15u;
     const bool use_rows = (uint64_t)nu * rw <= (512ull << 20);
     const size_t u_words = ((size_t)5 * nu + 2 * (size_t)nr + 64 + 3) & ~(size_t)3;
     uint32_t *u;
-    ELP_TRY(scratch(c, 3, u_words + (use_rows ? ((size_t)nu * rw + 64) / 4 : 0), &u));
+    ELP_TRY(scratch(c, 3, std::max(u_words + (use_rows ? ((size_t)nu * rw + 64) / 4 : 0), plan_next ? tie_plan_words(cu_next, cr_next, rw_p) : (size_t)0), &u));
     uint32_t *u_pos = u, *u_read = u + nu, *u_seg = u + 2 * (size_t)nu, *uv0 = u + 3 * (size_t)nu, *uv1 = u + 4 * (size_t)nu, *d_start = u + 5 * (size_t)nu,
              *d_first = d_start + nr;
     uint64_t *uk;
-    ELP_TRY(scratch(c, 4, (size_t)2 * nu + 16, &uk));
+    ELP_TRY(scratch(c, 4, (size_t)2 * std::max(nu, plan_next ? cu_next : 0u) + 16, &uk));
     uint64_t *uk0 = uk, *uk1 = uk + nu;
     ELP_HIP(c, hipMemcpyAsync(d_start, starts.data(), (size_t)nr * 4, hipMemcpyHostToDevice, c->stream));
     ELP_HIP(c, hipMemcpyAsync(d_first, first.data(), ((size_t)nr + 1) * 4, hipMemcpyHostToDevice, c->stream));
-    ELP_LAUNCH(c, "large_fill", k_large_fill, dim3(blocks_for(nu, 256)), dim3(256), 0, nu, nr, (const uint32_t *)d_start, (const uint32_t *)d_first, sv, u_pos, u_read, u_seg);
+    ELP_LAUNCH(c, "large_fill", k_large_fill, dim3(blocks_for(nu, 256)), dim3(256), 0, nu, nr, (const uint32_t *)d_start, (const uint32_t *)d_first, sv, u_pos, u_read, u_seg,
+               (const TiePlan *)nullptr, (uint32_t *)nullptr);
     ELP_LAUNCH(c, "iota", k_iota, dim3(blocks_for(nu, 256)), dim3(256), 0, uv0, (uint64_t)nu);
     const uint32_t maxq = c->max_qname_len;
     const uint32_t m_bytes = maxq + 15;
@@ -892,12 +1089,12 @@
     if (use_rows) {
       uint8_t *rows = reinterpret_cast<uint8_t *>(u + u_words);
       ELP_LAUNCH(c, "material_rows", k_material_rows, dim3(blocks_for((uint64_t)nu * (rw >> 3), 256)), dim3(256), 0, nu, (const uint32_t *)u_read, maxq, m_bytes, rw,
-                 rows, t);
+                 rows, t, (const TiePlan *)nullptr);
       t.rows = rows;
       t.rw = rw;
     }
     ELP_LAUNCH(c, "material_live", k_material_live, dim3(blocks_for(nu, 256)), dim3(256), 0, nu, (const uint32_t *)u_read, maxq, m_bytes,
-               c->tie_live.p, t);
+               c->tie_live.p, t, (const TiePlan *)nullptr);
     uint32_t live[elp_ctx::TIE_LIVE_WORDS];
     ELP_HIP(c, hipMemcpyAsync(live, c->tie_live.p, sizeof live, hipMemcpyDeviceToHost, c->stream));
     ELP_HIP(c, elp::stream_wait(c->stream));
@@ -914,7 +1111,8 @@
       ELP_TRY(scratch(c, 5, (size_t)TIE_MAX_PACKED * 8 + (size_t)TIE_MAX_PACKED * 64 + 64, &d_vals));
       uint8_t *d_lut = reinterpret_cast<uint8_t *>(d_vals + TIE_MAX_PACKED * 8);
       ELP_HIP(c, hipMemsetAsync(d_vals, 0, (size_t)pl.n * 8 * 4, c->stream));
-      ELP_LAUNCH(c, "material_values", k_material_values, dim3(std::min(blocks_for(nu, 256), 1024u)), dim3(256), 0, nu, (const uint32_t *)u_read, pl, maxq, d_vals, t);
+      ELP_LAUNCH(c, "material_values", k_material_values, dim3(std::min(blocks_for(nu, 256), 1024u)), dim3(256), 0, nu, (const uint32_t *)u_read, pl, maxq, d_vals, t,
+                 (const TiePlan *)nullptr);
       std::vector<uint32_t> hv((size_t)pl.n * 8);
       ELP_HIP(c, hipMemcpyAsync(hv.data(), d_vals, hv.size() * 4, hipMemcpyDeviceToHost, c->stream));
       ELP_HIP(c, elp::stream_wait(c->stream));
@@ -943,7 +1141,7 @@
           sel.n++;
         }
         ELP_LAUNCH(c, "material_keys", k_material_keys_packed, dim3(blocks_for(nu, 256)), dim3(256), 0, nu, (const uint32_t *)vcur, (const uint32_t *)u_read,
-                   sel, (const uint8_t *)d_lut, maxq, uk0, t, (const uint32_t *)(nr > 1 ? u_seg : nullptr), (uint32_t)total);
+                   sel, (const uint8_t *)d_lut, maxq, uk0, t, (const uint32_t *)(nr > 1 ? u_seg : nullptr), (uint32_t)total, (const TiePlan *)nullptr);
         uint64_t *ko;
         uint32_t *vo;
         ELP_TRY(radix_sort_pairs_low(c, uk0, vcur, uk1, vtmp, nu, (segbits + total + 7) / 8, &ko, &vo));
@@ -952,10 +1150,10 @@
         if (!settled) {
           uint32_t *over = c->err_flag.p + 3;
           ELP_LAUNCH(c, "large_ties", k_large_ties, dim3(blocks_for(nu, 256)), dim3(256), 0, nu, (const uint64_t *)ko, (const uint32_t *)vcur, vtmp,
-                     (const uint32_t *)u_read, m_bytes, maxq, over, t);
+                     (const uint32_t *)u_read, m_bytes, maxq, over, t, (const TiePlan *)nullptr);
           std::swap(vcur, vtmp);
           ELP_LAUNCH(c, "large_scatter", k_large_scatter, dim3(blocks_for(nu, 256)), dim3(256), 0, nu, (const uint32_t *)vcur, (const uint32_t *)u_pos,
-                     (const uint32_t *)u_read, c->perm.p);
+                     (const uint32_t *)u_read, c->perm.p, (const TiePlan *)nullptr);
           uint32_t h_over = 0;
           ELP_HIP(c, hipMemcpyAsync(&h_over, over, 4, hipMemcpyDeviceToHost, c->stream));
           ELP_HIP(c, elp::stream_wait(c->stream));
@@ -967,7 +1165,7 @@
           }
         } else {
           ELP_LAUNCH(c, "large_scatter", k_large_scatter, dim3(blocks_for(nu, 256)), dim3(256), 0, nu, (const uint32_t *)vcur, (const uint32_t *)u_pos,
-                     (const uint32_t *)u_read, c->perm.p);
+                     (const uint32_t *)u_read, c->perm.p, (const TiePlan *)nullptr);
         }
         if (settled) {
           c->radix_check_pending = true;
@@ -987,7 +1185,7 @@
           sel.n++;
         }
         ELP_LAUNCH(c, "material_keys", k_material_keys_packed, dim3(blocks_for(nu, 256)), dim3(256), 0, nu, (const uint32_t *)vcur, (const uint32_t *)u_read,
-                   sel, (const uint8_t *)d_lut, maxq, uk0, t, (const uint32_t *)nullptr, 0u);
+                   sel, (const uint8_t *)d_lut, maxq, uk0, t, (const uint32_t *)nullptr, 0u, (const TiePlan *)nullptr);
         uint64_t *ko;
         uint32_t *vo;
         ELP_TRY(radix_sort_pairs_low(c, uk0, vcur, uk1, vtmp, nu, (total + 7) / 8, &ko, &vo));
@@ -1017,7 +1215,7 @@
       if (vo != vcur) { vtmp = vcur; vcur = vo; }
     }
     ELP_LAUNCH(c, "large_scatter", k_large_scatter, dim3(blocks_for(nu, 256)), dim3(256), 0, nu, (const uint32_t *)vcur, (const uint32_t *)u_pos,
-               (const uint32_t *)u_read, c->perm.p);
+               (const uint32_t *)u_read, c->perm.p, (const TiePlan *)nullptr);
   }
   c->radix_check_pending = true;
   c->sorted = true;
```

Result: no change. 2347, median of 2 (-0.2%).
